# aws/sagemaker-xgboost-container

Measured on NVIDIA H100. Metric: boosting rounds/sec, higher is better.
Workload: dtype int64

## Files before the change

include/b200xgb.h:

```cpp
#ifndef B200XGB_H_
#define B200XGB_H_
#include <stddef.h>
#include <stdint.h>

#ifdef __cplusplus
extern "C" {
#endif

#if defined(__GNUC__)
#define XGB_DLL __attribute__((visibility("default")))
#else
#define XGB_DLL
#endif

typedef void* DMatrixHandle;
typedef void* BoosterHandle;
typedef uint64_t bst_ulong;

XGB_DLL const char* XGBGetLastError(void);
XGB_DLL void XGBoostVersion(int* major, int* minor, int* patch);
XGB_DLL int XGBuildInfo(const char** out);

XGB_DLL int XGDMatrixCreateFromDense(const char* data, const char* config, DMatrixHandle* out);
XGB_DLL int XGDMatrixSetInfoFromInterface(DMatrixHandle handle, const char* field, const char* data);
// ... 33 lines not shown
XGB_DLL int XGBoosterTrainOneIter(BoosterHandle handle, DMatrixHandle dtrain, int iter, const char* grad, const char* hess);
XGB_DLL int XGBoosterBoostOneIter(BoosterHandle handle, DMatrixHandle dtrain, float* grad, float* hess, bst_ulong len);
XGB_DLL int XGBoosterEvalOneIter(BoosterHandle handle, int iter, DMatrixHandle dmats[], const char* evnames[], bst_ulong len,
                         const char** out_result);
XGB_DLL int XGBoosterPredictFromDMatrix(BoosterHandle handle, DMatrixHandle dmat, const char* config,
                                bst_ulong const** out_shape, bst_ulong* out_dim, float const** out_result);
XGB_DLL int XGBoosterPredictFromDense(BoosterHandle handle, const char* values, const char* config, DMatrixHandle m,
                                      bst_ulong const** out_shape, bst_ulong* out_dim, const float** out_result);
XGB_DLL int XGBoosterPredictFromCSR(BoosterHandle handle, const char* indptr, const char* indices, const char* values, bst_ulong ncol,
                                    const char* config, DMatrixHandle m, bst_ulong const** out_shape, bst_ulong* out_dim,
                                    const float** out_result);
XGB_DLL int XGBoosterPredictFromCudaArray(BoosterHandle handle, const char* values, const char* config, DMatrixHandle proxy,
                                          bst_ulong const** out_shape, bst_ulong* out_dim, const float** out_result);
XGB_DLL int XGBoosterSaveModel(BoosterHandle handle, const char* fname);
XGB_DLL int XGBoosterLoadModel(BoosterHandle handle, const char* fname);
XGB_DLL int XGBoosterSaveModelToBuffer(BoosterHandle handle, const char* config, bst_ulong* out_len, const char** out_dptr);
XGB_DLL int XGBoosterLoadModelFromBuffer(BoosterHandle handle, const void* buf, bst_ulong len);
XGB_DLL int XGBoosterSerializeToBuffer(BoosterHandle handle, bst_ulong* out_len, const char** out_dptr);
XGB_DLL int XGBoosterUnserializeFromBuffer(BoosterHandle handle, const void* buf, bst_ulong len);
XGB_DLL int XGBoosterSaveJsonConfig(BoosterHandle handle, bst_ulong* out_len, const char** out_str);
XGB_DLL int XGBoosterLoadJsonConfig(BoosterHandle handle, const char* config);
XGB_DLL int XGBoosterGetNumFeature(BoosterHandle handle, bst_ulong* out);
XGB_DLL int XGBoosterBoostedRounds(BoosterHandle handle, int* out);
XGB_DLL int XGBoosterSlice(BoosterHandle handle, int begin_layer, int end_layer, int step, BoosterHandle* out);
XGB_DLL int XGBoosterGetAttr(BoosterHandle handle, const char* key, const char** out, int* success);
XGB_DLL int XGBoosterSetAttr(BoosterHandle handle, const char* key, const char* value);
XGB_DLL int XGBoosterGetAttrNames(BoosterHandle handle, bst_ulong* out_len, const char*** out);
XGB_DLL int XGBoosterSetStrFeatureInfo(BoosterHandle handle, const char* field, const char** features, bst_ulong size);
XGB_DLL int XGBoosterGetStrFeatureInfo(BoosterHandle handle, const char* field, bst_ulong* len, const char*** out_features);

XGB_DLL int XGCommunicatorInit(const char* config);
XGB_DLL int XGCommunicatorBroadcast(void* send_receive_buffer, size_t size, int root);
XGB_DLL int XGCommunicatorFinalize(void);
XGB_DLL int XGCommunicatorGetRank(void);
XGB_DLL int XGCommunicatorGetWorldSize(void);
XGB_DLL int XGCommunicatorGetUniqueId(const char** out_hex);

XGB_DLL int XGB200DMatrixGetCuts(DMatrixHandle handle, int max_bin, bst_ulong* n_ptrs, const int** ptrs, bst_ulong* n_vals,
                         const float** vals, const float** mins, int* has_missing);
XGB_DLL int XGB200DMatrixSetCuts(DMatrixHandle handle, const int* ptrs, bst_ulong n_ptrs, const float* vals, const float* mins);
XGB_DLL int XGB200DMatrixCreateFromCSV(const char* text, bst_ulong len, char delimiter, int* status, DMatrixHandle* out);
XGB_DLL int XGB200DMatrixCreateFromCSVEx(const char* text, bst_ulong len, char delimiter, int label_column, int weight_column,
                             int* status, DMatrixHandle* out);
XGB_DLL int XGB200DMatrixCreateFromLibsvmText(const char* text, bst_ulong len, int whitespace_mode, float absent, int* status, DMatrixHandle* out);
XGB_DLL int XGB200DMatrixCreateFromRecordIO(const char* buf, bst_ulong len, int* status, DMatrixHandle* out);
XGB_DLL int XGB200CommPeerReduceActive(void);
XGB_DLL int XGB200DMatrixCreateFromColumns(const void* const* cols, const int* col_types, int ncols, bst_ulong nrow, int label_column,
                                   int weight_column, DMatrixHandle* out);
XGB_DLL int XGB200DMatrixGetRaw(DMatrixHandle handle, float* out_row_major);
XGB_DLL int XGB200DeviceMemory(bst_ulong* live, bst_ulong* peak, int reset_peak);
XGB_DLL int XGB200DMatrixGetBins(DMatrixHandle handle, int max_bin, uint8_t* out_row_major);
XGB_DLL int XGB200DMatrixGetBinCopies(DMatrixHandle handle, int max_bin, int* out_aligned_stride, uint8_t* out_aligned, uint8_t* out_col);
XGB_DLL int XGB200DMatrixRankCuts(DMatrixHandle handle, int max_bin, const int64_t* row_bounds, int n_ranges, int* out_ptrs,
                          float* out_vals, float* out_mins);
XGB_DLL int XGB200SegmentedQuantile(const float* values, const int32_t* segments, const float* weights, bst_ulong n, int n_segments,
                                    float alpha, float* out);
XGB_DLL int XGB200GradientBasedSample(const float* gpair, bst_ulong n, float subsample, unsigned seed, uint64_t stream,
                                      float* out_threshold, float* out_gpair);
XGB_DLL int XGB200BoosterModelShape(BoosterHandle handle, bst_ulong* num_trees, bst_ulong* num_nodes, float* base_score, int* num_class);
XGB_DLL int XGB200BoosterExportModel(BoosterHandle handle, int64_t* tree_offset, int32_t* tree_info, int32_t* left, int32_t* right,
                             int32_t* parent, int32_t* split_index, int32_t* split_bin, uint8_t* default_left,
                             float* split_cond, float* base_weight, float* loss_chg, float* sum_hess);
XGB_DLL int XGB200BuildRootHistogram(BoosterHandle handle, DMatrixHandle dmat, const float* gpair, int repeats,
                             int64_t* out_hist, float* scales, float* out_ms);
XGB_DLL int XGB200BuildHistogramEx(BoosterHandle handle, DMatrixHandle dmat, const float* gpair, int repeats, int mode,
                             const unsigned* row_ids, bst_ulong n_ids, int64_t* out_hist, float* scales, float* out_ms,
                             const char** out_kernel);
XGB_DLL int XGB200BoosterEvalRootSplit(BoosterHandle handle, DMatrixHandle dmat, const int64_t* hist, int64_t G, int64_t H, float max_g,
                               float max_h, float lower, float upper, const uint8_t* feat_mask, const char** out_json);
XGB_DLL int XGB200BoosterInplaceDebug(BoosterHandle handle, int64_t chunk_rows, bst_ulong* staged_bytes, bst_ulong* staging_capacity);
XGB_DLL int XGB200BoosterPredictKernelMs(BoosterHandle handle, DMatrixHandle dmat, int repeats, float* out_ms);
XGB_DLL int XGB200BoosterPredictPlan(BoosterHandle handle, DMatrixHandle dmat, int iter_begin, int iter_end, const char** out_json);
XGB_DLL int XGB200BoosterEvalContainerMetrics(BoosterHandle handle, DMatrixHandle dmat, const char** names, bst_ulong len, int output_margin,
                                              long long* out);
XGB_DLL int XGB200BoosterGetCachedMargin(BoosterHandle handle, DMatrixHandle dmat, float* out);
XGB_DLL int XGB200BoosterGetTrainingMargin(BoosterHandle handle, DMatrixHandle dtrain, bst_ulong* out_rows, bst_ulong* out_cols, const float** out);
XGB_DLL int XGB200BoosterGetTreeWeights(BoosterHandle handle, bst_ulong* len, float* out);
XGB_DLL int XGB200BoosterGetRefreshSums(BoosterHandle handle, bst_ulong* len, long long* out);
XGB_DLL int XGB200BoosterComputeGradient(BoosterHandle handle, DMatrixHandle dmat, const float* margin, int round, float* out_gpair);
XGB_DLL int XGB200TimerStart(void);
XGB_DLL int XGB200TimerStop(float* out_ms);
XGB_DLL int XGB200BoosterSetProfile(BoosterHandle handle, int enable);
XGB_DLL int XGB200BoosterGetProfile(BoosterHandle handle, const char** out_json);
XGB_DLL int XGB200LaunchCount(long long* out);
XGB_DLL int XGB200Synchronize(void);
XGB_DLL int XGB200LegacyModelToUBJ(const void* buf, bst_ulong len, bst_ulong* out_len, const char** out);

#ifdef __cplusplus
}
#endif
#endif
```

sagemaker-xgboost-container_b200/backend.py:

```python
import ctypes as C
import json
import os

import numpy as np

_HERE = os.path.dirname(os.path.abspath(__file__))
LIB_PATH = os.path.join(_HERE, "lib", "libb200xgb.so")

c_bst_ulong = C.c_uint64


class XGBoostError(ValueError):
    """Error raised by the native library (same name and base class as xgboost.core.XGBoostError)."""


def _cstr(s):
    return C.c_char_p(s.encode("utf-8"))


def _from_cstr_array(ptr, n):
    return [ptr[i].decode("utf-8") for i in range(n)]


_utf8_and_size = C.pythonapi.PyUnicode_AsUTF8AndSize
# ... 543 lines not shown
    def booster_predict_kernel_ms(self, bh, dh, repeats=5):
        ms = C.c_float()
        self._check(self.lib.XGB200BoosterPredictKernelMs(bh, dh, C.c_int(repeats), C.byref(ms)))
        return float(ms.value)

    def booster_predict_plan(self, bh, dh, iteration_range=(0, 0)):
        out = C.c_char_p()
        self._check(self.lib.XGB200BoosterPredictPlan(bh, dh, C.c_int(iteration_range[0]), C.c_int(iteration_range[1]), C.byref(out)))
        return json.loads(out.value.decode())

    def booster_eval_container_metrics(self, bh, dh, names, output_margin):
        arr = (C.c_char_p * len(names))(*[n.encode("utf-8") for n in names])
        out = np.zeros(8 + 64 * 64, np.int64)
        self._check(self.lib.XGB200BoosterEvalContainerMetrics(bh, dh, arr, c_bst_ulong(len(names)), C.c_int(1 if output_margin else 0),
                                                               out.ctypes.data_as(C.POINTER(C.c_longlong))))
        return out

    @staticmethod
    def _gradient_iface(a):
        if isinstance(a, np.ndarray):
            return {"data": [int(a.ctypes.data), True], "shape": [int(d) for d in a.shape], "typestr": a.dtype.str, "strides": None, "version": 3}
        iface = a.__cuda_array_interface__
        out = {"data": [int(iface["data"][0]), False], "shape": [int(d) for d in iface["shape"]], "typestr": iface["typestr"],
               "strides": [int(d) for d in iface["strides"]], "version": 3}
        if "stream" in iface:
            out["stream"] = None if iface["stream"] is None else int(iface["stream"])
        return out

    def booster_boost(self, bh, dh, it, grad, hess):
        self._check(self.lib.XGBoosterTrainOneIter(bh, dh, C.c_int(it), _cstr(json.dumps(self._gradient_iface(grad))),
                                                   _cstr(json.dumps(self._gradient_iface(hess)))))

    def booster_training_margin(self, bh, dh):
        rows, cols, ptr = c_bst_ulong(), c_bst_ulong(), C.POINTER(C.c_float)()
        self._check(self.lib.XGB200BoosterGetTrainingMargin(bh, dh, C.byref(rows), C.byref(cols), C.byref(ptr)))
        if rows.value * cols.value == 0:
            return np.zeros((rows.value, cols.value), np.float32)
        return np.ctypeslib.as_array(ptr, shape=(rows.value, cols.value)).copy()

    def booster_cached_margin(self, bh, dh, K):
        n = self.dmatrix_num_row(dh)
        out = np.zeros((n, K), np.float32)
        self._check(self.lib.XGB200BoosterGetCachedMargin(bh, dh, out.ctypes.data_as(C.POINTER(C.c_float))))
        return out

    def booster_compute_gradient(self, bh, dh, margin, round=0):
        n = self.dmatrix_num_row(dh)
        margin = np.ascontiguousarray(margin, np.float32).reshape(n, -1)
        out = np.zeros((n, margin.shape[1], 2), np.float32)
        self._check(self.lib.XGB200BoosterComputeGradient(bh, dh, margin.ctypes.data_as(C.POINTER(C.c_float)), C.c_int(int(round)),
                                                          out.ctypes.data_as(C.POINTER(C.c_float))))
        return out

    def booster_tree_weights(self, bh):
        n = c_bst_ulong()
        self._check(self.lib.XGB200BoosterGetTreeWeights(bh, C.byref(n), None))
        out = np.zeros(n.value, np.float32)
        self._check(self.lib.XGB200BoosterGetTreeWeights(bh, C.byref(n), out.ctypes.data_as(C.POINTER(C.c_float))))
        return out

    def booster_refresh_sums(self, bh):
        n = c_bst_ulong()
        self._check(self.lib.XGB200BoosterGetRefreshSums(bh, C.byref(n), None))
        out = np.zeros(n.value, np.int64)
        self._check(self.lib.XGB200BoosterGetRefreshSums(bh, C.byref(n), out.ctypes.data_as(C.POINTER(C.c_longlong))))
        return out.reshape(-1, 2)

    def timer_start(self):
        self._check(self.lib.XGB200TimerStart())

    def timer_stop(self):
        ms = C.c_float()
        self._check(self.lib.XGB200TimerStop(C.byref(ms)))
        return float(ms.value)

    def booster_set_profile(self, bh, enable):
        self._check(self.lib.XGB200BoosterSetProfile(bh, C.c_int(1 if enable else 0)))

    def booster_get_profile(self, bh):
        out = C.c_char_p()
        self._check(self.lib.XGB200BoosterGetProfile(bh, C.byref(out)))
        return json.loads(out.value.decode())

    def launch_count(self):
        out = C.c_longlong()
        self._check(self.lib.XGB200LaunchCount(C.byref(out)))
        return int(out.value)

    def synchronize(self):
        self._check(self.lib.XGB200Synchronize())


_BACKEND = None


def get_backend():
    global _BACKEND
    if _BACKEND is None:
        _BACKEND = CudaBackend()
    return _BACKEND
```

sagemaker-xgboost-container_b200/csrc/booster.cu:

```cuda
#include "booster.h"
#include <algorithm>
#include <atomic>
#include <cctype>
#include <climits>
#include <cmath>
#include <cstring>
#include "comm.h"
#include "multi_target.h"
#include "rng.h"

namespace b200 {

long long g_kernel_launches = 0;

namespace {
struct DeviceCtx {
  cudaStream_t stream = nullptr; int num_sms = 0; bool ok = false; std::string why;
  DeviceCtx() {
    int count = 0;
    cudaError_t e = cudaGetDeviceCount(&count);
    if (e != cudaSuccess || count == 0) { why = std::string("no CUDA device available (") + cudaGetErrorString(e) + ")"; cudaGetLastError(); return; }
    int dev = 0;
    if (const char* lr = getenv("LOCAL_RANK")) { dev = atoi(lr) % count; }
    if (const char* d = getenv("B200XGB_DEVICE")) { dev = atoi(d) % count; }
// ... 2067 lines not shown
    CUDA_OK(cudaMemcpyAsync(d_info.p, info.data(), sizeof(int) * info.size(), cudaMemcpyHostToDevice, s));
  }
  CUDA_OK(cudaMemsetAsync(d_out.p, 0, sizeof(float) * std::max<size_t>(total, 1), s));
  ShapArgs sa{}; sa.X = dm->X.p; sa.n = n; sa.F = F; sa.nodes = d_sn.p; sa.tree_offset = d_off.p; sa.tree_info = d_info.p; sa.tree_begin = tb; sa.tree_end = te; sa.K = K;
  sa.out = d_out.p; sa.base_margin = base_margin(); sa.tree_weight = d_w.p;
  if (!dm->base_margin.empty()) { B200_CHECK(dm->base_margin.size() == (size_t)n * K, "base_margin size does not match rows x groups"); sa.base_margin_rows = dm->d_base_margin.p; }
  launch_shap(sa, max_depth, s);
  out->resize(total);
  if (total) CUDA_OK(cudaMemcpyAsync(out->data(), d_out.p, sizeof(float) * total, cudaMemcpyDeviceToHost, s));
  Comm::get().sync_stream(s);
  if (K > 1) shape->assign({(uint64_t)n, (uint64_t)K, (uint64_t)(F + 1)}); else shape->assign({(uint64_t)n, (uint64_t)(F + 1)});
}

PredictArgs Booster::predict_args(DMatrix* dm, int tree_begin, int tree_end) {
  PredictArgs pa{}; if (dm) { pa.X = dm->X.p; pa.n = dm->n; pa.F = dm->F; pa.has_nan = dm->has_missing ? 1 : 0; }
  pa.nodes = d_nodes.p; pa.tree_offset = d_tree_offset.p; pa.tree_info = d_tree_info.p;
  pa.tree_begin = tree_begin; pa.tree_end = tree_end; pa.K = param_.num_outputs(); pa.margin = nullptr; pa.leaf = nullptr;
  pa.h_tree_offset = h_tree_offset.data(); pa.children_adjacent = children_adjacent_ ? 1 : 0;
  pa.model_F = num_feature_;
  return pa;
}

void Booster::run_predict(DMatrix* dm, PredictArgs pa, cudaStream_t s) {
  if (!dm->quantile) { launch_predict(pa, s); return; }
  if (pa.tree_end <= pa.tree_begin) return;
  int64_t lo = h_tree_offset[pa.tree_begin], hi = h_tree_offset[pa.tree_begin + 1];
  for (int t = pa.tree_begin + 1; t < pa.tree_end; ++t) { lo = std::min(lo, h_tree_offset[t]); hi = std::max(hi, h_tree_offset[t + 1]); }
  bin_nodes_.ensure(std::max<size_t>(d_nodes.n, 1));
  launch_bin_thresholds(d_nodes.p + lo, (size_t)(hi - lo), dm->d_cut_ptrs.p, dm->d_cut_vals.p, dm->d_min_vals.p, dm->F, bin_nodes_.p + lo, s);
  pa.nodes = bin_nodes_.p;
  launch_predict_bins(pa, dm->binned_view(), s);
}

std::string Booster::debug_predict_plan(DMatrix* dm, int iter_begin, int iter_end) {
  configure();
  upload_model();
  if (iter_end == 0) iter_end = layers();
  B200_CHECK(iter_begin >= 0 && iter_begin <= iter_end && iter_end <= layers(), "debug_predict_plan: invalid iteration range");
  const PredictArgs pa = predict_args(dm, iteration_indptr_[iter_begin], iteration_indptr_[iter_end]);
  return predict_plan_json(dm->quantile ? plan_for_bins(pa, dm->binned_view()) : plan_for(pa), pa.tree_begin, pa.tree_end, pa.has_nan != 0);
}

float Booster::debug_predict_kernel_ms(DMatrix* dm, int repeats) {
  configure();
  cudaStream_t s = engine_stream();
  upload_model();
  const int K = param_.num_outputs();
  pred_margin_.ensure((size_t)dm->n * K);
  PredictArgs pa = predict_args(dm, 0, (int)trees_.size());
  pa.margin = pred_margin_.p;
  cudaEvent_t e0, e1; CUDA_OK(cudaEventCreate(&e0)); CUDA_OK(cudaEventCreate(&e1));
  float total = 0.f;
  for (int r = 0; r < std::max(1, repeats); ++r) {
    launch_fill(pred_margin_.p, dm->n * K, base_margin(), s);
    CUDA_OK(cudaEventRecord(e0, s));
    run_predict(dm, pa, s);
    CUDA_OK(cudaEventRecord(e1, s));
    CUDA_OK(cudaEventSynchronize(e1));
    float ms = 0; CUDA_OK(cudaEventElapsedTime(&ms, e0, e1)); total += ms;
  }
  cudaEventDestroy(e0); cudaEventDestroy(e1);
  return total / std::max(1, repeats);
}

int Booster::training_margin(DMatrix* dtrain, std::vector<float>* out) {
  configure();
  if (layers() == 0 && !update_mode_) check_targets(dtrain, true);
  cached_margin(dtrain, out);
  return param_.num_outputs();
}

void Booster::cached_margin(DMatrix* dm, std::vector<float>* out) {
  configure();
  cudaStream_t s = engine_stream();
  PredCache& c = cache_for(dm);
  bring_cache_up_to_date(dm, c);
  out->resize((size_t)dm->n * param_.num_outputs());
  if (!out->empty()) CUDA_OK(cudaMemcpyAsync(out->data(), c.margin.p, sizeof(float) * out->size(), cudaMemcpyDeviceToHost, s));
  Comm::get().sync_stream(s);
}

void Booster::set_profile(bool on) { builder_->set_profile(on); }
std::string Booster::get_profile() { return builder_->profile_json(); }

}
```

sagemaker-xgboost-container_b200/csrc/booster.h:

```cpp
#pragma once
#include <functional>
#include <map>
#include <memory>
#include <string>
#include <vector>
#include "container_metrics.h"
#include "curve.h"
#include "custom_grad.h"
#include "engine.h"
#include "grow.h"
#include "json.h"
#include "misc.h"
#include "rank.h"
#include "refresh.h"
#include "sampling.h"
#include "survival.h"
#include "tree.h"

namespace b200 {

struct ProxyBatch {
  enum Kind { kNone, kHostDense, kDevice, kCSR } kind = kNone;
  int64_t n = 0; int F = 0;
  const float* data = nullptr;
// ... 61 lines not shown
};

void csr_to_dense_device(const unsigned long long* d_ptr, const unsigned* d_idx, const float* d_val, int64_t nrow, int F, float* X, cudaStream_t s);

struct HostTree {
  std::vector<int> left, right, parent, split_index, split_bin;
  std::vector<uint8_t> default_left;
  std::vector<float> split_cond, base_weight, loss_chg, sum_hess;
  int num_nodes() const { return (int)left.size(); }
};

struct UpdateState {
  bool started = false;
  std::vector<HostTree> trees; std::vector<int> tree_info;
  std::vector<int> indptr{0};
  std::vector<int> node_off;
  std::vector<int64_t> block_off;
  DevBuf<unsigned char> in_block;
  DevBuf<DevNode> nodes; DevBuf<int> d_node_off, d_class; DevBuf<int64_t> d_block_off;
  DevBuf<GH64> sums; DevBuf<int> scratch; DevBuf<unsigned char> out_blocks;
  DevBuf<float2> gpair; DevBuf<unsigned> absmax; DevBuf<float> scales;
  int64_t global_n = 0; uint64_t global_n_uid = 0;
  int layers() const { return (int)indptr.size() - 1; }
};

struct PredCache {
  DevBuf<float> margin; int trees_applied = 0; int64_t n = 0; uint64_t model_version = 0;
  std::vector<float> weights;
};

struct DartParam { bool on = false; float rate_drop = 0.0f, skip_drop = 0.0f; int one_drop = 0, sample_type = 0, normalize_type = 0; };

bool looks_like_legacy_binary(const char* buf, size_t len);
JPtr legacy_binary_to_doc(const char* buf, size_t len);
std::pair<const char*, size_t> legacy_serialized_model_section(const char* buf, size_t len);

struct GradInput {
  static constexpr uint64_t kNoStream = ~0ull;
  const void* ptr = nullptr; int64_t n = 0, m = 1, s0 = 0, s1 = 0; bool f64 = false; uint64_t stream = kNoStream;
};

class Booster {
 public:
  Booster();
  ~Booster();
  void set_param(const std::string& k, const std::string& v);
  std::string save_config();
  void load_config(const std::string& json);
  void update_one_iter(int iter, DMatrix* dtrain);
  void boost_one_iter(DMatrix* dtrain, const GradInput& grad, const GradInput& hess);
  std::string eval_one_iter(int iter, const std::vector<DMatrix*>& dms, const std::vector<std::string>& names);
  void eval_container_metrics(DMatrix* dm, const std::vector<std::string>& names, bool output_margin, long long* out);
  void predict(DMatrix* dm, int type, bool training, int iter_begin, int iter_end, bool strict_shape,
               std::vector<float>* out, std::vector<uint64_t>* shape);
  void predict_contribs(DMatrix* dm, int tree_begin, int tree_end, std::vector<float>* out, std::vector<uint64_t>* shape);
  void inplace_predict(const InputDesc& in, bool on_device, uint64_t stream, int type, int iter_begin, int iter_end, bool strict_shape,
                       const std::vector<float>& base_margin_rows, std::vector<float>* out, std::vector<uint64_t>* shape, const float** dev_out);
  void inplace_debug(int64_t chunk_rows, uint64_t* staged_bytes, uint64_t* staging_capacity);
  std::string save_model_buffer(const std::string& format);
  void load_model_buffer(const char* buf, size_t len);
  std::string serialize();
  void unserialize(const char* buf, size_t len);
  std::unique_ptr<Booster> slice(int begin, int end, int step);
  int boosted_rounds();
  int num_features() const { return num_feature_; }
  std::map<std::string, std::string> attrs;
  std::vector<std::string> feature_names, feature_types;

  void sync_model();
  void cached_margin(DMatrix* dm, std::vector<float>* out);
  int training_margin(DMatrix* dtrain, std::vector<float>* out);
  float debug_predict_kernel_ms(DMatrix* dm, int repeats);
  std::string debug_predict_plan(DMatrix* dm, int iter_begin, int iter_end);
  const std::vector<HostTree>& trees() { sync_model(); return trees_; }
  const std::vector<int>& tree_info() const { return tree_info_; }
  const std::vector<float>& tree_weights() const { return weight_drop_; }
  float base_score() const { return base_score_; }
  int num_class() const { return param_.num_class; }
  const TrainParam& param() { configure(); return param_; }
  void set_profile(bool on);
  void debug_gradient(DMatrix* dm, const float* margin, int round, float* out);
  void debug_refresh_sums(std::vector<long long>* out);
  std::string get_profile();
  void debug_build_root_hist(DMatrix* dm, const float* gpair_host, std::vector<long long>* hist_out, float* scales_out,
                             int repeats, float* ms_out, int mode = 0, const unsigned* row_ids = nullptr, int64_t n_ids = 0);
  std::string debug_eval_root(DMatrix* dm, const long long* hist_fm, long long G, long long H, float max_g, float max_h,
                              float lower, float upper, const unsigned char* feat_mask);

 private:
  PredictArgs predict_args(DMatrix* dm, int tree_begin, int tree_end);
  void run_predict(DMatrix* dm, PredictArgs pa, cudaStream_t s);
  void predict_margin(DMatrix* dm, int tb, int te);
  void finish_predict(int64_t n, int type, bool strict_shape, std::vector<float>* out, std::vector<uint64_t>* shape, const float** dev_out);
  struct InplaceState {
    unsigned char* pinned = nullptr;
    DevBuf<unsigned char> stage;
    DevBuf<float> scratch;
    cudaStream_t copy = nullptr; cudaEvent_t copied[2] = {}, consumed[2] = {};
    int64_t debug_chunk_rows = 0; uint64_t staged_bytes = 0;
  } inplace_;
  DevBuf<DevNode> bin_nodes_;
  std::map<std::string, std::string> raw_params_;
  std::vector<std::string> eval_metrics_;
  std::vector<int> monotone_;
  std::vector<std::vector<int>> interaction_;
  bool configured_ = false;
  TrainParam param_;
  std::string objective_name_ = "reg:squarederror";
  bool base_score_set_ = false; float base_score_ = 0.5f; bool base_score_estimated_ = false;
  int num_feature_ = 0;
  int num_target_ = 1;
  std::vector<HostTree> trees_; std::vector<int> tree_info_;
  std::vector<int> iteration_indptr_{0};
  DevBuf<float2> forest_gpair_;
  GbsScratch gbs_;
  std::vector<float> weight_drop_;
  DartParam dart_;
  float dart_new_weight_ = 1.0f;
  DevBuf<float> dart_drop_margin_;
  DevBuf<int> dart_ids_; DevBuf<float> dart_coef_;
  std::vector<PendingTree> pending_;
  std::vector<char> on_device_;
  uint64_t model_version_ = 0;
  DevBuf<DevNode> d_nodes; std::vector<int64_t> h_tree_offset; DevBuf<int64_t> d_tree_offset; DevBuf<int> d_tree_info;
  size_t d_nodes_used = 0; int d_trees_uploaded = 0;
  std::map<uint64_t, PredCache> caches_;
  std::unique_ptr<TreeBuilder> builder_ = std::make_unique<TreeBuilder>();
  DevBuf<double> dsum_;
  CoxScratch cox_scratch_;
  RankScratch rank_scratch_;
  CurveScratch curve_scratch_;
  ContainerScratch container_scratch_;
  bool labels_checked_ = false;
  DevBuf<float> pred_margin_, pred_cls_; DevBuf<int> pred_leaf_;
  bool children_adjacent_ = true;
  bool update_mode_ = false; std::vector<int> update_ops_; std::string update_ops_str_; int refresh_leaf_ = 1;
  std::unique_ptr<UpdateState> update_ = std::make_unique<UpdateState>();
  DevBuf<float> quantile_alpha_dev_; std::vector<float> quantile_alpha_host_;
  DevBuf<unsigned> target_absmax_;
  const CustomGradArgs* custom_ = nullptr;
  DevBuf<unsigned char> custom_staging_; DevBuf<unsigned long long> custom_bad_; DevBuf<unsigned> custom_bad_flag_;
  void train_round(DMatrix* dtrain, const CustomGradArgs* custom);
  GradArray custom_array(const GradInput& in, bool device, size_t staging_offset);
  void launch_custom_gradient_checked(int round, float2* gpair, int64_t gp_stride, unsigned* absmax, float subsample, bool per_target_absmax);

  void configure();
  void check_label_ranges(const DMatrix* dtrain);
  void check_targets(const DMatrix* dm, bool training);
  const RankGroups& rank_groups(DMatrix* dm, const char* what);
  void begin_update();
  void refresh_one_iter(DMatrix* dtrain);
  int layers() const { return (int)iteration_indptr_.size() - 1; }
  float base_margin() const;
  void estimate_base_score(DMatrix* dtrain);
  void upload_model();
  PredCache& cache_for(DMatrix* dm);
  void bring_cache_up_to_date(DMatrix* dm, PredCache& c);
  void append_device_tree(int class_id, size_t device_offset, int max_nodes, PendingTree pt, float weight);
  std::vector<int> dart_drop_set(int round) const;
  float* dart_begin_round(DMatrix* dtrain, PredCache& c, int round);
  DartArgs dart_args(const std::vector<int>& ids, const std::vector<float>& coef_full, const std::vector<float>& coef_drop);
  void dart_margin(DMatrix* dm, const std::vector<int>& ids, const std::vector<float>& coef_full, const std::vector<float>& coef_drop,
                   float* m_full, float* m_drop);
  void reserve_nodes(size_t count, size_t slack);
  TreeBuilder& builder_for(DMatrix* dm);
  TreeInputs tree_inputs(const DMatrix& dm, const std::string& mask, int tree_index, float* margin, int k);
// ... 22 lines not shown
```

sagemaker-xgboost-container_b200/csrc/capi.cc:

```cpp
#include "../../include/b200xgb.h"
#include <cmath>
#include <cstdio>
#include <cstring>
#include <algorithm>
#include <dirent.h>
#include <fstream>
#include <map>
#include <memory>
#include <sstream>
#include <sys/stat.h>
#include <string>
#include <vector>
#include "booster.h"
#include "comm.h"

using namespace b200;

namespace {
thread_local std::string g_last_error;
struct DMatrixBox {
  std::unique_ptr<DMatrix> dm;
  std::unique_ptr<ProxyBatch> proxy;
  std::vector<const char*> str_ptrs; std::vector<std::string> strs;
  std::vector<uint8_t> scratch_u8;
// ... 808 lines not shown
  std::vector<long long> h; float sc[4];
  BST(handle)->debug_build_root_hist(dm, gpair, &h, sc, repeats, out_ms, mode, row_ids, (int64_t)n_ids);
  hist_to_feature_major(dm, h, out_hist);
  if (scales) memcpy(scales, sc, sizeof sc);
  if (out_kernel) *out_kernel = hist_last_kernel();
  API_END();
}
int XGB200BoosterEvalRootSplit(BoosterHandle handle, DMatrixHandle dmat, const int64_t* hist, int64_t G, int64_t H, float max_g, float max_h,
                               float lower, float upper, const uint8_t* feat_mask, const char** out_json) {
  API_BEGIN(); BoosterBox* box = static_cast<BoosterBox*>(handle);
  box->ret_str = BST(handle)->debug_eval_root(DM(dmat), reinterpret_cast<const long long*>(hist), G, H, max_g, max_h, lower, upper, feat_mask);
  *out_json = box->ret_str.c_str(); API_END();
}
int XGB200BoosterPredictKernelMs(BoosterHandle handle, DMatrixHandle dmat, int repeats, float* out_ms) {
  API_BEGIN();
  *out_ms = BST(handle)->debug_predict_kernel_ms(DM(dmat), repeats);
  API_END();
}
int XGB200BoosterPredictPlan(BoosterHandle handle, DMatrixHandle dmat, int iter_begin, int iter_end, const char** out_json) {
  API_BEGIN(); BoosterBox* box = static_cast<BoosterBox*>(handle); box->ret_str = BST(handle)->debug_predict_plan(DM(dmat), iter_begin, iter_end);
  *out_json = box->ret_str.c_str(); API_END();
}
int XGB200BoosterGetTreeWeights(BoosterHandle handle, bst_ulong* len, float* out) {
  API_BEGIN();
  const std::vector<float>& w = BST(handle)->tree_weights();
  if (len) *len = w.size();
  if (out) memcpy(out, w.data(), sizeof(float) * w.size());
  API_END();
}
int XGB200BoosterGetRefreshSums(BoosterHandle handle, bst_ulong* len, long long* out) {
  API_BEGIN();
  std::vector<long long> v;
  BST(handle)->debug_refresh_sums(&v);
  if (len) *len = v.size();
  if (out) memcpy(out, v.data(), sizeof(long long) * v.size());
  API_END();
}
int XGB200BoosterComputeGradient(BoosterHandle handle, DMatrixHandle dmat, const float* margin, int round, float* out_gpair) {
  API_BEGIN();
  B200_CHECK(round >= 0, "XGB200BoosterComputeGradient: round must be >= 0");
  BST(handle)->debug_gradient(DM(dmat), margin, round, out_gpair);
  API_END();
}
int XGB200BoosterEvalContainerMetrics(BoosterHandle handle, DMatrixHandle dmat, const char** names, bst_ulong len, int output_margin,
                                      long long* out) {
  API_BEGIN();
  std::vector<std::string> v;
  for (bst_ulong i = 0; i < len; ++i) v.emplace_back(names[i]);
  BST(handle)->eval_container_metrics(DM(dmat), v, output_margin != 0, out);
  API_END();
}
int XGB200BoosterGetTrainingMargin(BoosterHandle handle, DMatrixHandle dtrain, bst_ulong* out_rows, bst_ulong* out_cols, const float** out) {
  API_BEGIN();
  BoosterBox* box = static_cast<BoosterBox*>(handle);
  const int K = BST(handle)->training_margin(DM(dtrain), &box->ret_vec);
  *out_rows = (bst_ulong)DM(dtrain)->n; *out_cols = (bst_ulong)K; *out = box->ret_vec.data();
  API_END();
}
int XGB200BoosterGetCachedMargin(BoosterHandle handle, DMatrixHandle dmat, float* out) {
  API_BEGIN();
  std::vector<float> v;
  BST(handle)->cached_margin(DM(dmat), &v);
  memcpy(out, v.data(), sizeof(float) * v.size());
  API_END();
}
static cudaEvent_t g_t0 = nullptr, g_t1 = nullptr;
int XGB200TimerStart(void) {
  API_BEGIN();
  if (!g_t0) { CUDA_OK(cudaEventCreate(&g_t0)); CUDA_OK(cudaEventCreate(&g_t1)); }
  CUDA_OK(cudaEventRecord(g_t0, engine_stream()));
  API_END();
}
int XGB200TimerStop(float* out_ms) {
  API_BEGIN();
  if (!g_t0) throw Error("XGB200TimerStop without XGB200TimerStart");
  CUDA_OK(cudaEventRecord(g_t1, engine_stream())); CUDA_OK(cudaEventSynchronize(g_t1));
  CUDA_OK(cudaEventElapsedTime(out_ms, g_t0, g_t1));
  API_END();
}
int XGB200BoosterSetProfile(BoosterHandle handle, int enable) { API_BEGIN(); BST(handle)->set_profile(enable != 0); API_END(); }
int XGB200BoosterGetProfile(BoosterHandle handle, const char** out_json) {
  API_BEGIN(); BoosterBox* box = static_cast<BoosterBox*>(handle); box->ret_str = BST(handle)->get_profile(); *out_json = box->ret_str.c_str(); API_END();
}
int XGB200LaunchCount(long long* out) { API_BEGIN(); *out = g_kernel_launches; API_END(); }
int XGB200Synchronize(void) { API_BEGIN(); CUDA_OK(cudaStreamSynchronize(engine_stream())); API_END(); }
int XGB200DMatrixCreateFromColumns(const void* const* cols, const int* col_types, int ncols, bst_ulong nrow, int label_column, int weight_column, DMatrixHandle* out) {
  API_BEGIN();
  B200_CHECK(out != nullptr && (ncols == 0 || (cols != nullptr && col_types != nullptr)), "XGB200DMatrixCreateFromColumns: NULL argument");
  auto box = new DMatrixBox(); std::unique_ptr<DMatrixBox> guard(box);
  box->dm = DMatrix::from_columns(cols, col_types, ncols, (int64_t)nrow, label_column, weight_column);
  *out = guard.release();
  API_END();
}
int XGB200LegacyModelToUBJ(const void* buf, bst_ulong len, bst_ulong* out_len, const char** out) {
  API_BEGIN();
  B200_CHECK(buf != nullptr && out_len != nullptr && out != nullptr, "XGB200LegacyModelToUBJ: NULL argument");
  const char* p = (const char*)buf; size_t n = (size_t)len;
  auto sect = legacy_serialized_model_section(p, n);
  if (sect.first != nullptr) { p = sect.first; n = sect.second; }
  B200_CHECK(looks_like_legacy_binary(p, n), "XGB200LegacyModelToUBJ: the buffer is not a legacy binary model");
  g_ret_str.clear(); ubj_write(*legacy_binary_to_doc(p, n), &g_ret_str);
  *out_len = g_ret_str.size(); *out = g_ret_str.data();
  API_END();
}

}
```

sagemaker-xgboost-container_b200/csrc/engine.h:

```cpp
#pragma once
#include <cuda_runtime.h>
#include <cstdint>
#include <cstdio>
#include <stdexcept>
#include <string>
#include <vector>

namespace b200 {

struct Error : std::runtime_error { using std::runtime_error::runtime_error; };
#define B200_CHECK(cond, msg) do { if (!(cond)) throw ::b200::Error(std::string(msg)); } while (0)
#define CUDA_OK(expr) do { cudaError_t e_ = (expr); if (e_ != cudaSuccess) throw ::b200::Error( \
    std::string("CUDA error: ") + cudaGetErrorString(e_) + " at " + __FILE__ + ":" + std::to_string(__LINE__)); } while (0)

extern long long g_kernel_launches;

cudaStream_t engine_stream();
int engine_num_sms();

void devmem_note(int64_t delta);
void devmem_query(uint64_t* live, uint64_t* peak, bool reset_peak);

template <typename T> struct DevBuf {
  T* p = nullptr; size_t n = 0;
  DevBuf() = default;
  DevBuf(const DevBuf&) = delete; DevBuf& operator=(const DevBuf&) = delete;
  ~DevBuf() { release(); }
  void release() { if (p) { cudaFree(p); devmem_note(-(int64_t)(n * sizeof(T))); } p = nullptr; n = 0; }
  void alloc(size_t count) { if (count == n && p) return; release();
    if (count) { CUDA_OK(cudaMalloc(&p, count * sizeof(T))); devmem_note((int64_t)(count * sizeof(T))); } n = count; }
  void ensure(size_t count) { if (count > n) alloc(count); }
  void zero(cudaStream_t s) { if (n) CUDA_OK(cudaMemsetAsync(p, 0, n * sizeof(T), s)); }
};

constexpr int kSlots = 32;
constexpr int kBins = 256;
constexpr int kGroupEntries = kBins * kSlots;
constexpr int kMissingBin = 255;
constexpr int kGradBits = 18, kWindowRows = 8064;
constexpr int kGradBitsSmall = 21, kWindowRowsSmall = 1008;
constexpr int64_t kSmallMatrixRows = 1 << 20;
inline int grad_bits_for(int64_t n) { return n <= kSmallMatrixRows ? kGradBitsSmall : kGradBits; }
inline int window_rows_for(int64_t n) { return n <= kSmallMatrixRows ? kWindowRowsSmall : kWindowRows; }
constexpr int kMaxDepth = 16;
constexpr int kMaxTrainFeatures = 65534 * 32;
static_assert(kMaxTrainFeatures < (1 << 23), "cand_key holds 23 bits of feature id");

struct GH64 { long long g, h; };

struct BinnedMatrix {
  const uint8_t* bins = nullptr;
  const uint8_t* bins_tail = nullptr;
  const uint8_t* bins_col = nullptr;
  const uint8_t* bins_gather = nullptr;
  int gather_stride = 0;
  int tail_in_gather = 0;
  int64_t n = 0;
  int F = 0, ngroups = 0, tw = 0, ntail = 0;
  int has_missing = 0;
  int unused = 0;
};

inline void feature_layout(int F, int* ngroups, int* tw, int* ntail) {
  const int a = F / 32, L = F % 32;
  if (a >= 1 && L >= 1 && L <= 8) { *ngroups = a; *ntail = L; *tw = L <= 4 ? 4 : 8; }
  else { *ngroups = a + (L > 0 ? 1 : 0); if (*ngroups == 0) *ngroups = 1; *ntail = 0; *tw = 0; }
}
inline size_t hist_slot_entries(int ngroups, int tw) { return (size_t)ngroups * 256 * 32 + (size_t)256 * tw; }

enum Objective : int { kSquaredError = 0, kBinaryLogistic = 1, kRegLogistic = 2, kLogitRaw = 3, kSoftprob = 4, kSoftmax = 5,
                       kSquaredLogError = 6, kPseudoHuber = 7, kPoisson = 8, kGamma = 9, kTweedie = 10, kHinge = 11,
                       kAft = 12, kCox = 13,
                       kAbsoluteError = 14,
                       kQuantileError = 15,
                       kRankPairwise = 16, kRankNdcg = 17, kRankMap = 18 };
enum Transform : int { kTransformNone = 0, kTransformSigmoid = 1, kTransformExp = 2, kTransformHinge = 3 };
inline bool objective_is_logistic(int o) { return o == kBinaryLogistic || o == kRegLogistic || o == kLogitRaw; }
inline bool objective_is_log_link(int o) { return o == kPoisson || o == kGamma || o == kTweedie; }
inline bool objective_is_survival(int o) { return o == kAft || o == kCox; }
inline bool objective_is_adaptive(int o) { return o == kAbsoluteError || o == kQuantileError; }
inline bool objective_is_rank(int o) { return o == kRankPairwise || o == kRankNdcg || o == kRankMap; }
inline int objective_transform(int o) {
  if (o == kBinaryLogistic || o == kRegLogistic) return kTransformSigmoid;
  if (objective_is_log_link(o) || objective_is_survival(o)) return kTransformExp;
  return o == kHinge ? kTransformHinge : kTransformNone;
}

struct TrainParam {
  int objective = kSquaredError;
  int num_class = 1;
  int max_depth = 6, max_leaves = 0, max_bin = 256;
  int lossguide = 0;
  float eta = 0.3f, lambda = 1.0f, alpha = 0.0f, gamma = 0.0f, min_child_weight = 1.0f, max_delta_step = 0.0f;
  float scale_pos_weight = 1.0f, subsample = 1.0f, colsample_bytree = 1.0f, colsample_bylevel = 1.0f, colsample_bynode = 1.0f;
  unsigned seed = 0;
  int num_parallel_tree = 1;
  int gradient_based = 0;
  float huber_slope = 1.0f, tweedie_variance_power = 1.5f, poisson_max_delta_step = 0.7f;
  int aft_dist = 0; float aft_sigma = 1.0f;
  std::vector<float> quantile_alpha;
  int rank_mean = 0, rank_unbiased = 0, rank_k = 32, rank_exp_gain = 1, rank_normalization = 1, rank_score_normalization = 1; float rank_bias_norm = 2.0f;
// ... 39 lines not shown
```

sagemaker-xgboost-container_b200/csrc/grow.cu:

```cuda
#include "grow.h"
#include <algorithm>
#include <cmath>
#include <cstdlib>
#include <cstring>
#include "comm.h"

namespace b200 {

__global__ void pack_tree_kernel(TreeArrays t, const int* n_nodes, DevNode* out, int cap) {
  const int nn = *n_nodes;
  for (int i = blockIdx.x * blockDim.x + threadIdx.x; i < cap; i += gridDim.x * blockDim.x) {
    DevNode d;
    if (i < nn) { d.cond = t.split_cond[i]; d.left = t.left[i]; d.right = t.right[i]; d.fidx_dl = (unsigned)t.split_index[i] | ((unsigned)t.default_left[i] << 31); }
    else { d.cond = 0.f; d.left = -1; d.right = -1; d.fidx_dl = 0; }
    out[i] = d;
  }
}
__global__ void snapshot_h_kernel(const GH64* slot, long long* cache, size_t entries) {
  for (size_t e = (size_t)blockIdx.x * blockDim.x + threadIdx.x; e < entries; e += (size_t)gridDim.x * blockDim.x) cache[e] = slot[e].h;
}
__global__ void slot_from_cache_kernel(GH64* slot, const long long* cache, size_t entries) {
  for (size_t e = (size_t)blockIdx.x * blockDim.x + threadIdx.x; e < entries; e += (size_t)gridDim.x * blockDim.x) { GH64 v; v.g = 0; v.h = cache[e]; slot[e] = v; }
}
__global__ void gather_u32_kernel(const unsigned* src, const unsigned* idx, unsigned* dst, int64_t n) {
  const int64_t i = (int64_t)blockIdx.x * blockDim.x + threadIdx.x;
  if (i < n) dst[i] = src[idx[i]];
}

void* PinnedPool::take(size_t bytes) {
  bytes = (bytes + 255) & ~(size_t)255;
  while (cur < chunks.size() && off + bytes > chunks[cur].second) { ++cur; off = 0; }
  if (cur >= chunks.size()) { size_t sz = std::max<size_t>(bytes, 4u << 20); char* p = nullptr; CUDA_OK(cudaMallocHost(&p, sz)); chunks.emplace_back(p, sz); off = 0; }
  void* r = chunks[cur].first + off; off += bytes; return r;
}
static bool tail_by_position(const BinnedMatrix& bm) { return bm.tw == 4 && !bm.tail_in_gather; }

size_t TreeBuilder::carve(GrowState& gs, uintptr_t base) const {
  const size_t N = cap_nodes, L = max_level_nodes, nblocks = ngroups + (tw > 0 ? 1 : 0);
  size_t off = 0;
  auto take = [&](auto*& p, size_t bytes) { p = reinterpret_cast<std::remove_reference_t<decltype(p)>>(base + off); off += (bytes + 255) & ~(size_t)255; };
  take(gs.seg_begin, 4 * N); take(gs.seg_count, 4 * N); take(gs.hist_slot, 4 * N); take(gs.node_sum, 16 * N); take(gs.root_gain, 4 * N); take(gs.weight, 4 * N);
  take(gs.best, sizeof(SplitCand) * N); take(gs.best_group, sizeof(SplitCand) * N * nblocks);
  take(gs.level_nodes, 4 * (size_t)(kMaxDepth + 1) * L); take(gs.level_count, 4 * (kMaxDepth + 2));
  take(gs.build_nid, 4 * L); take(gs.build_sub_nid, 4 * L); take(gs.build_parent_slot, 4 * L); take(gs.build_count, 4); take(gs.build_prefix, 4 * (L + 1));
  take(gs.part_action, 4 * L); take(gs.tile_prefix, 4 * (L + 1));
  take(gs.tile_desc, 8 * ((size_t)max_tiles + 1)); gs.part_ctl = (unsigned*)(gs.tile_desc + max_tiles);
  take(gs.n_leaves, 4); take(gs.scales, 16); take(gs.absmax, 8);
  take(gs.depth, 4 * N); take(gs.open, N); take(gs.n_slots, 4); take(gs.lg_done, 4); take(gs.lower, 4 * N); take(gs.upper, 4 * N);
  return off;
}

void TreeBuilder::ensure(const BinnedMatrix& bm, int max_depth_, int K, int lg_iters_, int n_ic_) {
  const bool tail_pos_ = tail_by_position(bm);
  const int64_t stride_ = (bm.n + 63) & ~(int64_t)63;
  if (n == bm.n && F == bm.F && ngroups == bm.ngroups && tw == bm.tw && tail_pos == tail_pos_ && max_depth == max_depth_ && lg_iters == lg_iters_ &&
      n_ic == n_ic_ && gpair.n >= (size_t)stride_ * K + 512) return;
  if (lg_iters_ == 0) B200_CHECK(max_depth_ >= 1 && max_depth_ <= kMaxDepth, "max_depth must be in [1, 16] for the B200 depth-wise hist builder");
  n = bm.n; F = bm.F; ngroups = bm.ngroups; tw = bm.tw; tail_pos = tail_pos_; max_depth = max_depth_; lg_iters = lg_iters_; n_ic = n_ic_;
  gp_stride = stride_; root_h_valid = false;
  cudaStream_t s = engine_stream();
  if (peer_reduce_active()) {
    peer_reduce_close();
    DevBuf<unsigned> bar; bar.alloc(1); bar.zero(s);
    Comm::get().allreduce_max_u32(bar.p, 1, s);
    Comm::get().sync_stream(s);
  }
  for (auto& tg : graphs) tg.destroy();
  size_t pool_slots; int max_nodes;
  if (lg_iters > 0) {
    max_nodes = 2 * lg_iters + 1; max_level_nodes = 2; region = 0;
    pool_slots = (size_t)lg_iters + kLgFirstFreeSlot;
  } else {
    max_nodes = (1 << (max_depth + 1)) - 1; max_level_nodes = 1 << (max_depth - 1); region = max_level_nodes;
    pool_slots = 2 * (size_t)region;
  }
  cap_nodes = (max_nodes + 15) & ~15;
  slot_stride = hist_slot_entries(ngroups, tw);
  const size_t partial_entries = hist_partial_entries(ngroups, tw, engine_num_sms(), max_level_nodes);
  const size_t pool_bytes = pool_slots * slot_stride * sizeof(GH64) + partial_entries * sizeof(int2);
  size_t free_b = 0, total_b = 0; cudaMemGetInfo(&free_b, &total_b);
  B200_CHECK(pool_bytes < free_b / 2 + hist_pool.n * sizeof(GH64) + hist_partials.n * sizeof(int2),
             "histogram pool for this max_depth / max_leaves / feature count does not fit in device memory");
  hist_pool.alloc(pool_slots * slot_stride);
  hist_partials.alloc(partial_entries);
  gpair.alloc((size_t)gp_stride * K + 512); gpair.zero(s); err.alloc(1); tree_index_dev.alloc(1);
  if (!leaf_scale.p) { leaf_scale.alloc(1); set_leaf_scale(1.0f); }
  root_h_cache.alloc(slot_stride);
  const bool routed = routes(lg_iters, max_depth);
  for (int i = 0; i < 2; ++i) { const size_t m = i == 0 || !routed ? (size_t)n : 0; ridx[i].alloc(m); gp[i].alloc(m); tl[i].alloc(tail_pos ? m : 0); }
  route_tiles = routed ? (unsigned)((n + kRouteTile - 1) / kRouteTile) : 0u;
  node_of_row.alloc(routed ? (size_t)n : 0);
  route_counts.alloc(routed && max_depth >= 2 ? ((size_t)1 << (max_depth - 2)) * route_tiles : 0);
  max_tiles = (unsigned)((n + kPartTile - 1) / kPartTile) + max_level_nodes + 1;
  scratch.alloc(3 * (size_t)max_level_nodes + 8);
  state_block.alloc(carve(gs, 0)); state_block.zero(s);
  carve(gs, (uintptr_t)state_block.p);
  tree_block.alloc(tree_block_bytes(cap_nodes));
  const TreeBlock tb = tree_block_layout(tree_block.p, cap_nodes);
  gs.n_nodes = tb.n_nodes; ta = tb.t; packed.alloc(cap_nodes);
  ic_path.alloc(n_ic ? (size_t)cap_nodes * F : 0); ic_allowed.alloc(n_ic ? (size_t)cap_nodes * F : 0);
  ic_sets.alloc((size_t)n_ic * F); ic_sets_host.clear();
  hist_configure();
  global_n = n;
  if (Comm::get().distributed()) {
    peer_reduce_setup({{hist_pool.p, hist_pool.n * sizeof(GH64)}, {state_block.p, state_block.n}}, s);
// ... 8 lines not shown

float* TreeBuilder::ensure_adaptive(int targets) {
  if (adapt.ensure(n, max_leaves(), cap_nodes, targets)) for (auto& tg : graphs) tg.destroy();
  return adapt.resid.p;
}

void TreeBuilder::set_leaf_scale(float v) {
  cudaStream_t s = engine_stream();
  CUDA_OK(cudaMemcpyAsync(leaf_scale.p, &v, sizeof v, cudaMemcpyHostToDevice, s));
  Comm::get().sync_stream(s);
}

const unsigned char* TreeBuilder::upload_mask(const std::string& mask, int tree_index) {
  cudaStream_t s = engine_stream(); feat_mask.ensure(mask.size());
  CUDA_OK(cudaMemcpyAsync(feat_mask.p, mask.data(), mask.size(), cudaMemcpyHostToDevice, s));
  CUDA_OK(cudaMemcpyAsync(tree_index_dev.p, &tree_index, sizeof(int), cudaMemcpyHostToDevice, s));
  Comm::get().sync_stream(s); return feat_mask.p;
}
template <typename T> static T* upload_changed(DevBuf<T>& d, std::vector<T>& host, const std::vector<T>& v) {
  if (v == host && d.n >= v.size()) return d.p;
  cudaStream_t s = engine_stream(); d.ensure(v.size());
  CUDA_OK(cudaMemcpyAsync(d.p, v.data(), sizeof(T) * v.size(), cudaMemcpyHostToDevice, s));
  Comm::get().sync_stream(s); host = v; return d.p;
}

const int* TreeBuilder::upload_monotone(const std::vector<int>& mono, int F_) {
  if (mono.empty()) return nullptr;
  B200_CHECK((int)mono.size() <= F_, "monotone_constraints has more entries than the data has features");
  std::vector<int> mh(mono); mh.resize((size_t)F_, 0);
  return upload_changed(monotone_dev, monotone_host, mh);
}
void TreeBuilder::upload_interaction(const std::vector<std::vector<int>>& ic, int F_) {
  if (ic.empty()) return;
  std::vector<unsigned char> sets(ic.size() * (size_t)F_, 0);
  for (size_t si = 0; si < ic.size(); ++si)
    for (int f : ic[si]) { B200_CHECK(f < F_, "interaction_constraints names feature " + std::to_string(f) + " but the data has " + std::to_string(F_) + " features"); sets[si * F_ + f] = 1; }
  upload_changed(ic_sets, ic_sets_host, sets);
}
HistArgs TreeBuilder::hist_args(const BinnedMatrix& bm, int k) const {
  HistArgs ha{}; ha.bins = bm.bins; ha.bins_tail = bm.bins_tail; ha.n = bm.n; ha.row_stride = bm.ngroups * kSlots; ha.tw = bm.tw;
  ha.bins_gather = bm.bins_gather; ha.gather_stride = bm.gather_stride;
  ha.tail_in_gather = bm.tail_in_gather;
  ha.gpair = gpair.p + (size_t)k * gp_stride;
  ha.build_count = gs.build_count; ha.build_nid = gs.build_nid; ha.build_prefix = gs.build_prefix; ha.seg_begin = gs.seg_begin;
  ha.hist_slot = gs.hist_slot; ha.scales = gs.scales; ha.hist_pool = hist_pool.p; ha.node_sum = gs.node_sum; ha.ngroups = bm.ngroups;
  ha.partials = hist_partials.p; ha.accumulate_sum = 1; ha.window_rows = window_rows_for(global_n);
  return ha;
}

EvalArgs TreeBuilder::eval_args(const TreeInputs& in, int level, const unsigned char* feat_mask) const {
  const BinnedMatrix& bm = in.bm;
  EvalArgs ea{}; ea.hist_pool = hist_pool.p; ea.gs = gs; ea.cut_ptrs = in.cut_ptrs; ea.feat_mask = feat_mask; ea.p = in.p; ea.F = bm.F;
  ea.ngroups = bm.ngroups; ea.tw = bm.tw; ea.ntail = bm.ntail; ea.has_missing = bm.has_missing; ea.level = level; ea.max_level_nodes = max_level_nodes;
  ea.colsample_bynode = in.mask ? in.colsample_bynode : 1.0f; ea.seed = in.seed; ea.tree_index = tree_index_dev.p; ea.monotone = in.monotone;
  ea.node_allowed = in.n_ic > 0 ? ic_allowed.p : nullptr;
  return ea;
}
ApplyArgs TreeBuilder::apply_args(const TreeInputs& in, int level, int next_base, int next_half) const {
  const BinnedMatrix& bm = in.bm;
  ApplyArgs aa{}; aa.gs = gs; aa.tree = ta; aa.cut_ptrs = in.cut_ptrs; aa.cut_vals = in.cut_vals; aa.min_vals = in.min_vals;
  aa.p = in.p; aa.scratch = scratch.p; aa.nblocks = bm.ngroups + (bm.tw > 0 ? 1 : 0); aa.level = level; aa.max_level_nodes = max_level_nodes;
  aa.next_base = next_base; aa.next_half = next_half; aa.monotone = in.monotone;
  if (in.n_ic > 0) { aa.node_path = ic_path.p; aa.node_allowed = ic_allowed.p; aa.ic_sets = ic_sets.p; aa.n_ic_sets = in.n_ic; aa.F = bm.F; }
  return aa;
}
template <class Launch> void TreeBuilder::timed(ProfKind kind, Launch launch) {
  if (!profile) { launch(); return; }
  ProfEvent e; e.kind = kind; e.launches = g_kernel_launches;
  CUDA_OK(cudaEventCreate(&e.a)); CUDA_OK(cudaEventCreate(&e.b));
  CUDA_OK(cudaEventRecord(e.a, engine_stream()));
  launch();
  e.launches = g_kernel_launches - e.launches;
  CUDA_OK(cudaEventRecord(e.b, engine_stream()));
  prof_events.push_back(e);
}

constexpr int kRootRows = -1;
void TreeBuilder::enqueue(const TreeInputs& in) {
  cudaStream_t s = engine_stream();
  const BinnedMatrix& bm = in.bm;
  const int k = in.k, D = in.p.max_depth;
  const bool dist = in.world > 1;
  const int num_sms = engine_num_sms();
  launch_init_tree(gs, ta, (unsigned)bm.n, s);
  if (in.root_mode == 2) { slot_from_cache_kernel<<<num_sms, 256, 0, s>>>(hist_pool.p, root_h_cache.p, slot_stride); ++g_kernel_launches; CUDA_OK(cudaGetLastError()); }
  else CUDA_OK(cudaMemsetAsync(hist_pool.p, 0, slot_stride * sizeof(GH64), s));
  const bool g_only = in.root_mode != 0;
  const int pay = g_only ? 4 : 8;
  const bool carry_tail = tail_by_position(bm);
  const bool routed = routes(in.lg_iters, D);
  if (profile && routed) {
    prof_part_row_bytes[0] = 3;
    prof_part_row_bytes[1] = 4;
    prof_part_row_bytes[2] = pay + 4 + pay + (carry_tail ? 8 : 0);
  } else if (profile) {
    prof_part_row_bytes[0] = pay + (carry_tail ? 4 : 0) + 1;
    prof_part_row_bytes[2] = 4 + pay + (carry_tail ? 4 : 0);
    prof_part_row_bytes[1] = prof_part_row_bytes[2] + 1;
  }
  HistArgs root = hist_args(bm, k);
  if (g_only) { root.gpair = nullptr; root.gpos = g_dense(); }
  root.g_only = in.root_mode == 2 ? 1 : 0; root.rows_counter = profile ? prof_rows.p : nullptr;
  timed(kProfRootHist, [&] { launch_hist_build(root, num_sms, s); });
  if (in.root_mode == 1) { snapshot_h_kernel<<<num_sms, 256, 0, s>>>(hist_pool.p, root_h_cache.p, slot_stride); ++g_kernel_launches; CUDA_OK(cudaGetLastError()); }
  auto collective = [&](std::function<void()> f) {
    if (!dist) return;
    if (!capturing) { f(); return; }
    end_segment(); capturing->colls.push_back(f);
    CUDA_OK(cudaStreamBeginCapture(s, cudaStreamCaptureModeThreadLocal));
  };
  auto allreduce_hist = [&](GH64* p, size_t cnt) {
    if (!dist) return;
    if (peer_allreduce_i64(reinterpret_cast<long long*>(p), cnt, s)) return;
    collective([p, cnt, s]() { Comm::get().allreduce_sum_i64(p, cnt, s); });
  };
  allreduce_hist(hist_pool.p, slot_stride * 2);
  allreduce_hist(gs.node_sum, 2);
  if (in.n_ic > 0) {
    CUDA_OK(cudaMemsetAsync(ic_path.p, 0, (size_t)bm.F, s));
    CUDA_OK(cudaMemsetAsync(ic_allowed.p, 1, (size_t)bm.F, s));
  }
  auto part_args = [&](int level, int cur, int next) {
    const bool root = cur == kRootRows;
    PartArgs pa{}; pa.gs = gs; pa.tree = ta; pa.bins_col = bm.bins_col; pa.n = bm.n;
    pa.ridx_cur = root ? nullptr : ridx[cur].p; pa.ridx_next = ridx[next].p;
    const void* root_gp = g_only ? static_cast<const void*>(g_dense()) : static_cast<const void*>(gpair.p + (size_t)k * gp_stride);
    pa.gp_cur = root ? root_gp : gp[cur].p; pa.gp_next = gp[next].p; pa.g_only = g_only ? 1 : 0;
    pa.tl_cur = !carry_tail ? nullptr : (root ? reinterpret_cast<const unsigned*>(bm.bins_tail) : tl[cur].p); pa.tl_next = carry_tail ? tl[next].p : nullptr;
    pa.has_missing = bm.has_missing; pa.level = level; pa.max_level_nodes = max_level_nodes; pa.rows_counter = profile ? prof_rows.p + 2 : nullptr;
    return pa;
  };
  auto level_hist_args = [&](int set) {
    HistArgs ha = hist_args(bm, k);
    ha.ridx = ridx[set].p; ha.tail_pos = carry_tail ? tl[set].p : nullptr; ha.accumulate_sum = 0;
    ha.gpair = g_only ? nullptr : gp[set].p; ha.gpos = g_only ? reinterpret_cast<const float*>(gp[set].p) : nullptr;
    ha.rows_counter = profile ? prof_rows.p + 1 : nullptr;
    return ha;
  };
  launch_eval(eval_args(in, 0, in.mask), 1, s);
  for (int it = 0; it < in.lg_iters; ++it) {
    launch_apply_lossguide(apply_args(in, 0, 0, 0), it, s);
    const PartArgs pa = part_args(0, it == 0 ? kRootRows : 0, 1);
    timed(kProfPartition, [&] { launch_partition(pa, max_tiles, s); });
    launch_lg_copy_back(pa, ridx[0].p, gp[0].p, tl[0].p, max_tiles, s);
    launch_zero_build_slots(gs, hist_pool.p, slot_stride, 1, s);
    timed(kProfDeepHist, [&] { launch_hist_build(level_hist_args(0), num_sms, s); });
    if (dist) {
      launch_lg_stage(gs, hist_pool.p, slot_stride, 1, s);
      allreduce_hist(hist_pool.p + (size_t)kLgStageSlot * slot_stride, slot_stride * 2);
      launch_lg_stage(gs, hist_pool.p, slot_stride, 0, s);
    }
    launch_subtract(gs, hist_pool.p, slot_stride, 1, s);
    launch_eval(eval_args(in, 1, nullptr), 2, s);
  }
  for (int L = 0; L < D && in.lg_iters == 0; ++L) {
    const bool final_level = (L == D - 1);
    const int next_base = ((L + 1) & 1) * region, next_half = 1 << L;
    launch_apply(apply_args(in, L, next_base, next_half), s);
    if (final_level) break;
    if (routed) {
      RouteArgs ra{}; ra.gs = gs; ra.tree = ta; ra.bins_col = bm.bins_col; ra.n = bm.n; ra.node_of_row = node_of_row.p;
      ra.tile_counts = route_counts.p; ra.ntiles = route_tiles; ra.has_missing = bm.has_missing; ra.level = L;
      if (g_only) ra.g = g_dense(); else ra.gpair = gpair.p + (size_t)k * gp_stride;
      ra.g_only = g_only ? 1 : 0;
      ra.tail_row = carry_tail ? reinterpret_cast<const unsigned*>(bm.bins_tail) : nullptr;
      ra.ridx = ridx[0].p; ra.gp = gp[0].p; ra.tl = carry_tail ? tl[0].p : nullptr; ra.rows_counter = profile ? prof_rows.p + 2 : nullptr;
      timed(kProfPartition, [&] { launch_route(ra, s); });
    } else {
      PartArgs pa = part_args(L, L == 0 ? kRootRows : (L & 1) ^ 1, L & 1);
      pa.build_only = L == D - 2 ? 1 : 0;
      timed(kProfPartition, [&] { launch_partition(pa, max_tiles, s); });
    }
    CUDA_OK(cudaMemsetAsync(hist_pool.p + (size_t)next_base * slot_stride, 0, (size_t)next_half * slot_stride * sizeof(GH64), s));
    timed(kProfDeepHist, [&] { launch_hist_build(level_hist_args(routed ? 0 : L & 1), num_sms, s); });
    allreduce_hist(hist_pool.p + (size_t)next_base * slot_stride, (size_t)next_half * slot_stride * 2);
    launch_subtract(gs, hist_pool.p, slot_stride, next_half, s);
    launch_eval(eval_args(in, L + 1, in.mask ? in.mask + (size_t)(L + 1) * bm.F : nullptr), 1 << (L + 1), s);
  }
  const uint8_t* start = routed && D >= 2 ? node_of_row.p : nullptr;
  if (in.adaptive) {
    launch_locate_leaves(ta, gs.n_nodes, bm.bins_col, bm.n, bm.has_missing, start, g_only ? nullptr : gpair.p + (size_t)k * gp_stride, &adapt, s);
    SelectArgs sa{}; sa.values = in.resid; sa.seg = adapt.seg.p; sa.h = in.adaptive == 2 ? reinterpret_cast<const float*>(gpair.p + (size_t)k * gp_stride) + 1 : nullptr;
    sa.h_stride = 2; sa.scales = gs.scales; sa.n = bm.n; sa.nseg = max_leaves(); sa.alpha = (double)in.alpha;
    if (in.adaptive == 3) { sa.h = in.weight; sa.h_stride = 1; sa.scales = adapt.scales.p; }
    sa.leaf_nid = adapt.leaf_nid.p; sa.split_cond = ta.split_cond; sa.lr = in.p.eta;
    segmented_select(sa, &adapt, [&](unsigned long long* p, size_t cnt) { collective([p, cnt, s]() { Comm::get().allreduce_sum_i64(p, cnt, s); }); },
                     [&](unsigned* p, size_t cnt) { collective([p, cnt, s]() { Comm::get().allreduce_max_u32(p, cnt, s); }); }, s);
  }
  timed(kProfMargin, [&] { launch_update_margin(ta, gs.n_nodes, bm.bins_col, bm.n, bm.has_missing, start, in.margin, in.K, k, leaf_scale.p, s); });
  if (profile) prof_margin_rows += bm.n;
  pack_tree_kernel<<<(cap_nodes + 255) / 256, 256, 0, s>>>(ta, gs.n_nodes, packed.p, cap_nodes); ++g_kernel_launches;
  CUDA_OK(cudaGetLastError());
}
void TreeBuilder::end_segment() {
  cudaGraph_t graph = nullptr; cudaGraphExec_t exec = nullptr;
  CUDA_OK(cudaStreamEndCapture(engine_stream(), &graph));
  cudaError_t e = cudaGraphInstantiate(&exec, graph, 0);
  cudaGraphDestroy(graph);
  CUDA_OK(e);
  capturing->segs.push_back(exec);
}

void TreeBuilder::grow(const TreeInputs& in) {
  cudaStream_t s = engine_stream();
  static const bool no_graph = getenv("B200XGB_NO_GRAPH") != nullptr;
  if ((int)graphs.size() <= in.k) graphs.resize(in.k + 1);
  TreeGraph& tg = graphs[in.k];
  if (profile || no_graph || (in.world > 1 && !tg.eager_done) || in.root_mode == 1) { tg.eager_done = true; enqueue(in); return; }
  if (tg.segs.empty() || memcmp(&tg.key, &in, sizeof in) != 0) {
    tg.destroy();
    const long long launches_before = g_kernel_launches;
    CUDA_OK(cudaStreamBeginCapture(s, cudaStreamCaptureModeThreadLocal));
    capturing = &tg;
    try { enqueue(in); end_segment(); }
    catch (...) { capturing = nullptr; cudaGraph_t graph = nullptr; cudaStreamEndCapture(s, &graph); if (graph) cudaGraphDestroy(graph); tg.destroy(); throw; }
    capturing = nullptr;
    tg.key = in; tg.launches = g_kernel_launches - launches_before;
    g_kernel_launches = launches_before;
  }
  for (size_t i = 0; i < tg.segs.size(); ++i) {
    CUDA_OK(cudaGraphLaunch(tg.segs[i], s));
    if (i < tg.colls.size()) tg.colls[i]();
  }
  g_kernel_launches += tg.launches;
}
PendingTree TreeBuilder::stage_tree() {
  cudaStream_t s = engine_stream();
  PendingTree pt; pt.cap_nodes = (size_t)cap_nodes; pt.staging = pinned.take(tree_block.n);
  if (!free_events.empty()) { pt.ready = free_events.back(); free_events.pop_back(); }
  else CUDA_OK(cudaEventCreateWithFlags(&pt.ready, cudaEventDisableTiming));
  CUDA_OK(cudaMemcpyAsync(pt.staging, tree_block.p, tree_block.n, cudaMemcpyDeviceToHost, s));
  CUDA_OK(cudaEventRecord(pt.ready, s));
  return pt;
}

void TreeBuilder::debug_build_root_hist(const BinnedMatrix& bm, const float* gpair_host, std::vector<long long>* hist_out, float* scales_out,
                                        int repeats, float* ms_out, int mode, const unsigned* row_ids, int64_t n_ids) {
  cudaStream_t s = engine_stream();
  const int64_t rows = row_ids ? n_ids : bm.n;
  B200_CHECK(rows <= bm.n, "debug_build_root_hist: more row ids than rows");
  CUDA_OK(cudaMemcpyAsync(gpair.p, gpair_host, sizeof(float2) * rows, cudaMemcpyHostToDevice, s));
  if (row_ids) CUDA_OK(cudaMemcpyAsync(ridx[0].p, row_ids, sizeof(unsigned) * rows, cudaMemcpyHostToDevice, s));
  float mg = 0.f, mh = 0.f;
  for (int64_t i = 0; i < rows; ++i) { mg = std::max(mg, std::fabs(gpair_host[2 * i])); mh = std::max(mh, gpair_host[2 * i + 1]); }
  unsigned am[2]; memcpy(&am[0], &mg, 4); memcpy(&am[1], &mh, 4);
  CUDA_OK(cudaMemcpyAsync(gs.absmax, am, 8, cudaMemcpyHostToDevice, s));
  launch_scales(gs, grad_bits_for(global_n), s);
  HistArgs ha = hist_args(bm, 0);
  ha.ridx = row_ids ? ridx[0].p : nullptr;
  ha.force_gather = (mode & 3) == 1 ? 1 : 0; ha.g_only = (mode & 3) == 2 ? 1 : 0;
  if ((mode & 8) || ha.g_only) {
    std::vector<float> gh((size_t)rows);
    for (int64_t i = 0; i < rows; ++i) gh[i] = gpair_host[2 * i];
    float* gpos = row_ids ? reinterpret_cast<float*>(gp[0].p) : g_dense();
    if (rows) CUDA_OK(cudaMemcpyAsync(gpos, gh.data(), sizeof(float) * rows, cudaMemcpyHostToDevice, s));
    Comm::get().sync_stream(s);
    ha.gpos = gpos; ha.gpair = nullptr;
  }
  if ((mode & 4) && row_ids && tail_by_position(bm)) {
    gather_u32_kernel<<<(unsigned)((rows + 255) / 256), 256, 0, s>>>(reinterpret_cast<const unsigned*>(bm.bins_tail), ridx[0].p, tl[0].p, rows); ++g_kernel_launches;
    CUDA_OK(cudaGetLastError());
    ha.tail_pos = tl[0].p;
  }
  root_h_valid = false;
  cudaEvent_t e0, e1; CUDA_OK(cudaEventCreate(&e0)); CUDA_OK(cudaEventCreate(&e1));
  float total = 0.f;
  for (int r = 0; r < std::max(1, repeats); ++r) {
    launch_init_tree(gs, ta, (unsigned)rows, s);
    CUDA_OK(cudaMemsetAsync(hist_pool.p, 0, slot_stride * sizeof(GH64), s));
    CUDA_OK(cudaEventRecord(e0, s));
    launch_hist_build(ha, engine_num_sms(), s);
    CUDA_OK(cudaEventRecord(e1, s));
    CUDA_OK(cudaEventSynchronize(e1));
    float ms = 0; CUDA_OK(cudaEventElapsedTime(&ms, e0, e1)); total += ms;
  }
  if (ms_out) *ms_out = total / std::max(1, repeats);
  hist_out->resize(slot_stride * 2);
  CUDA_OK(cudaMemcpyAsync(hist_out->data(), hist_pool.p, sizeof(GH64) * slot_stride, cudaMemcpyDeviceToHost, s));
  CUDA_OK(cudaMemcpyAsync(scales_out, gs.scales, 4 * sizeof(float), cudaMemcpyDeviceToHost, s));
  Comm::get().sync_stream(s);
  cudaEventDestroy(e0); cudaEventDestroy(e1);
}

std::string TreeBuilder::debug_eval_root(const TreeInputs& in, const long long* hist_fm, long long G, long long H, float max_g, float max_h,
                                         float lower, float upper) {
  cudaStream_t s = engine_stream();
  root_h_valid = false;
  const BinnedMatrix& bm = in.bm;
  const int F_ = bm.F;
  std::vector<GH64> slot(slot_stride, GH64{0, 0});
  const size_t W = (size_t)bm.ngroups * kSlots, tail0 = (size_t)bm.ngroups * kGroupEntries;
  for (int f = 0; f < F_; ++f)
    for (int b = 0; b < kBins; ++b) {
      const size_t e = (size_t)f < W ? ((size_t)(f / kSlots) * kBins + b) * kSlots + f % kSlots : tail0 + (size_t)b * bm.tw + (f - W);
      slot[e].g = hist_fm[((size_t)f * kBins + b) * 2]; slot[e].h = hist_fm[((size_t)f * kBins + b) * 2 + 1];
    }
  launch_init_tree(gs, ta, (unsigned)bm.n, s);
  CUDA_OK(cudaMemcpyAsync(hist_pool.p, slot.data(), sizeof(GH64) * slot_stride, cudaMemcpyHostToDevice, s));
  const GH64 tot{G, H};
  CUDA_OK(cudaMemcpyAsync(gs.node_sum, &tot, sizeof tot, cudaMemcpyHostToDevice, s));
  CUDA_OK(cudaMemcpyAsync(gs.lower, &lower, 4, cudaMemcpyHostToDevice, s));
  CUDA_OK(cudaMemcpyAsync(gs.upper, &upper, 4, cudaMemcpyHostToDevice, s));
  unsigned am[2]; memcpy(&am[0], &max_g, 4); memcpy(&am[1], &max_h, 4);
  CUDA_OK(cudaMemcpyAsync(gs.absmax, am, 8, cudaMemcpyHostToDevice, s));
  launch_scales(gs, grad_bits_for(global_n), s);
  launch_eval(eval_args(in, 0, in.mask), 1, s);
  const ApplyArgs aa = apply_args(in, 0, region, 1);
  if (in.lg_iters > 0) launch_apply_lossguide(aa, 0, s); else launch_apply(aa, s);
  const int nblocks = bm.ngroups + (bm.tw > 0 ? 1 : 0);
  std::vector<unsigned char> sb(state_block.n), tb(tree_block.n);
  CUDA_OK(cudaMemcpyAsync(sb.data(), state_block.p, sb.size(), cudaMemcpyDeviceToHost, s));
  CUDA_OK(cudaMemcpyAsync(tb.data(), tree_block.p, tb.size(), cudaMemcpyDeviceToHost, s));
  Comm::get().sync_stream(s);
  GrowState h; carve(h, (uintptr_t)sb.data());
  auto bits = [](float v) { unsigned u; memcpy(&u, &v, 4); return std::to_string(u); };
  auto cand = [&](const SplitCand& c) {
    return "{\"loss_chg\":" + bits(c.loss_chg) + ",\"feature\":" + std::to_string(c.feature) + ",\"bin\":" + std::to_string(c.bin) + ",\"dleft\":" +
           std::to_string(c.dleft) + ",\"ord\":" + std::to_string(c.ord) + ",\"GL\":" + std::to_string(c.GL) + ",\"HL\":" + std::to_string(c.HL) + "}";
  };
  const TreeBlock t = tree_block_layout(tb.data(), cap_nodes);
  const int nn = *t.n_nodes;
  std::string o = "{\"scales\":[";
  for (int i = 0; i < 4; ++i) o += (i ? "," : "") + bits(h.scales[i]);
  o += "],\"root_gain\":" + bits(h.root_gain[0]) + ",\"weight\":" + bits(h.weight[0]) + ",\"best_group\":[";
  for (int i = 0; i < nblocks; ++i) o += (i ? "," : "") + cand(h.best_group[i]);
  o += "],\"best\":" + cand(h.best[0]) + ",\"n_nodes\":" + std::to_string(nn) + ",\"expanded\":" + (nn == 3 ? "true" : "false") + ",\"tree\":{";
  const char* iname[5] = {"left", "right", "parent", "split_index", "split_bin"};
  const int* iarr[5] = {t.t.left, t.t.right, t.t.parent, t.t.split_index, t.t.split_bin};
  const char* fname[4] = {"split_cond", "base_weight", "loss_chg", "sum_hess"};
  const float* farr[4] = {t.t.split_cond, t.t.base_weight, t.t.loss_chg, t.t.sum_hess};
  for (int a = 0; a < 5; ++a) { o += std::string(a ? "," : "") + "\"" + iname[a] + "\":["; for (int i = 0; i < nn; ++i) o += (i ? "," : "") + std::to_string(iarr[a][i]); o += "]"; }
  for (int a = 0; a < 4; ++a) { o += std::string(",\"") + fname[a] + "\":["; for (int i = 0; i < nn; ++i) o += (i ? "," : "") + bits(farr[a][i]); o += "]"; }
  o += ",\"default_left\":["; for (int i = 0; i < nn; ++i) o += (i ? "," : "") + std::to_string((int)t.t.default_left[i]); o += "]}";
  o += ",\"children\":[";
  for (int c = 1; c < nn && c < 3; ++c)
    o += std::string(c > 1 ? "," : "") + "{\"G\":" + std::to_string(h.node_sum[c].g) + ",\"H\":" + std::to_string(h.node_sum[c].h) + ",\"lower\":" + bits(h.lower[c]) + ",\"upper\":" + bits(h.upper[c]) + "}";
  o += "]}";
  return o;
}

void TreeBuilder::set_profile(bool on) {
  profile = on;
  if (on) { prof_rows.alloc(4); prof_rows.zero(engine_stream()); prof_margin_rows = 0; }
  for (auto& e : prof_events) { cudaEventDestroy(e.a); cudaEventDestroy(e.b); }
  prof_events.clear();
}
std::string TreeBuilder::profile_json() {
  cudaStream_t s = engine_stream();
  Comm::get().sync_stream(s);
  double ms[kProfKinds] = {}; long long launches[kProfKinds] = {};
  for (auto& e : prof_events) { float t = 0; CUDA_OK(cudaEventElapsedTime(&t, e.a, e.b)); ms[e.kind] += t; launches[e.kind] += e.launches; }
  unsigned long long rows[4] = {0, 0, 0, 0};
  if (prof_rows.p) CUDA_OK(cudaMemcpy(rows, prof_rows.p, sizeof rows, cudaMemcpyDeviceToHost));
  char buf[1024];
  snprintf(buf, sizeof buf, "{\"root_hist_ms\":%.6f,\"root_hist_launches\":%lld,\"root_hist_rows\":%llu,\"deep_hist_ms\":%.6f,\"deep_hist_launches\":%lld,\"deep_hist_rows\":%llu,"
           "\"part_ms\":%.6f,\"part_launches\":%lld,\"part_rows\":%llu,\"part_rows_written\":%llu,"
           "\"part_row_bytes_in_root\":%d,\"part_row_bytes_in\":%d,\"part_row_bytes_out\":%d,\"margin_ms\":%.6f,\"margin_launches\":%lld,\"margin_rows\":%lld}",
           ms[kProfRootHist], launches[kProfRootHist], rows[0], ms[kProfDeepHist], launches[kProfDeepHist], rows[1],
           ms[kProfPartition], launches[kProfPartition], rows[2], rows[3], prof_part_row_bytes[0], prof_part_row_bytes[1], prof_part_row_bytes[2],
           ms[kProfMargin], launches[kProfMargin], prof_margin_rows);
  return buf;
}

}
```

sagemaker-xgboost-container_b200/csrc/grow.h:

```cpp
#pragma once
#include <functional>
#include <string>
#include <type_traits>
#include <vector>
#include "adaptive.h"
#include "engine.h"
#include "misc.h"
#include "tree.h"

namespace b200 {

struct TreeInputs {
  BinnedMatrix bm;
  const int* cut_ptrs; const float* cut_vals; const float* min_vals;
  float* margin;
  const unsigned char* mask;
  const int* monotone;
  TrainParamDev p;
  float colsample_bynode; unsigned seed;
  int lg_iters, n_ic;
  int K, k, world;
  int root_mode;
  const float* resid; const float* weight;
  int adaptive;
  float alpha;
};
static_assert(std::is_trivially_copyable<TreeInputs>::value, "TreeInputs is compared as bytes");
static_assert(sizeof(BinnedMatrix) == 4 * sizeof(void*) + sizeof(int64_t) + 8 * sizeof(int), "BinnedMatrix has padding bytes");
static_assert(sizeof(TrainParamDev) == 8 * 4, "TrainParamDev has padding bytes");
static_assert(sizeof(TreeInputs) == sizeof(BinnedMatrix) + 8 * sizeof(void*) + sizeof(TrainParamDev) + 10 * 4, "TreeInputs has padding bytes");

inline size_t tree_block_bytes(size_t cap) { return 64 + 9 * 4 * cap + cap; }
struct TreeBlock { int* n_nodes; TreeArrays t; };
__host__ __device__ inline TreeBlock tree_block_layout(void* base, size_t cap) {
  int* ip = (int*)((unsigned char*)base + 64); float* fp = (float*)(ip + 5 * cap);
  return {(int*)base, {ip, ip + cap, ip + 2 * cap, ip + 3 * cap, ip + 4 * cap, (unsigned char*)(fp + 4 * cap), fp, fp + cap, fp + 2 * cap, fp + 3 * cap}};
}

struct PendingTree {
  void* staging = nullptr; size_t cap_nodes = 0; cudaEvent_t ready = nullptr;
};
struct PinnedPool {
  std::vector<std::pair<char*, size_t>> chunks; size_t cur = 0, off = 0;
  ~PinnedPool() { for (auto& c : chunks) cudaFreeHost(c.first); }
  void* take(size_t bytes);
  void reset() { cur = 0; off = 0; }
};

struct TreeGraph {
  std::vector<cudaGraphExec_t> segs; std::vector<std::function<void()>> colls;
  TreeInputs key{}; long long launches = 0;
  bool eager_done = false;
  TreeGraph() = default; TreeGraph(TreeGraph&&) = default;
  ~TreeGraph() { destroy(); }
  void destroy() { for (auto e : segs) if (e) cudaGraphExecDestroy(e); segs.clear(); colls.clear(); }
};

struct TreeBuilder {
  int64_t n = 0; int F = 0, ngroups = 0, tw = 0, max_depth = 0, cap_nodes = 0, max_level_nodes = 0, region = 0; bool tail_pos = false;
  int lg_iters = 0, n_ic = 0;
  size_t slot_stride = 0;
  int64_t gp_stride = 0;
  unsigned max_tiles = 0;
  int64_t global_n = 0;
  DevBuf<long long> root_h_cache; uint64_t root_h_uid = 0, root_h_version = 0; bool root_h_valid = false;
  GrowState gs{}; TreeArrays ta{};
  DevBuf<unsigned char> state_block;
  DevBuf<unsigned char> tree_block;
  DevBuf<GH64> hist_pool; DevBuf<unsigned> ridx[2], scratch;
  DevBuf<int2> hist_partials;
  DevBuf<float2> gpair, gp[2]; DevBuf<unsigned> tl[2]; DevBuf<int> err, tree_index_dev; DevBuf<unsigned char> ic_path, ic_allowed, ic_sets;
  DevBuf<uint8_t> node_of_row; DevBuf<unsigned> route_counts; unsigned route_tiles = 0;
  DevBuf<DevNode> packed;
  DevBuf<float> leaf_scale;
  DevBuf<unsigned char> feat_mask; DevBuf<int> monotone_dev;
  std::vector<unsigned char> ic_sets_host;
  std::vector<int> monotone_host;
  PinnedPool pinned; std::vector<cudaEvent_t> free_events;
  std::vector<TreeGraph> graphs;
  TreeGraph* capturing = nullptr;
  SelectScratch adapt;
  int max_leaves() const { return lg_iters > 0 ? lg_iters + 1 : 1 << max_depth; }
  float* ensure_adaptive(int targets = 1);
  enum ProfKind { kProfRootHist, kProfDeepHist, kProfPartition, kProfMargin, kProfKinds };
  struct ProfEvent { cudaEvent_t a, b; int kind; long long launches; };
  bool profile = false; std::vector<ProfEvent> prof_events;
  DevBuf<unsigned long long> prof_rows;
  long long prof_margin_rows = 0;
  int prof_part_row_bytes[3] = {0, 0, 0};

  ~TreeBuilder() { for (auto e : free_events) cudaEventDestroy(e); for (auto& e : prof_events) { cudaEventDestroy(e.a); cudaEventDestroy(e.b); } }
  void ensure(const BinnedMatrix& bm, int max_depth, int K, int lg_iters, int n_ic);
  static bool routes(int lg_iters, int max_depth) { return lg_iters == 0 && max_depth <= kRouteMaxDepth; }
  const unsigned char* upload_mask(const std::string& mask, int tree_index);
  const int* upload_monotone(const std::vector<int>& mono, int F);
  void upload_interaction(const std::vector<std::vector<int>>& sets, int F);
  void set_leaf_scale(float v);
  void grow(const TreeInputs& in);
  PendingTree stage_tree();
  void set_profile(bool on); std::string profile_json();
  void debug_build_root_hist(const BinnedMatrix& bm, const float* gpair_host, std::vector<long long>* hist_out, float* scales_out,
                             int repeats, float* ms_out, int mode, const unsigned* row_ids, int64_t n_ids);
  std::string debug_eval_root(const TreeInputs& in, const long long* hist_fm, long long G, long long H, float max_g, float max_h,
                              float lower, float upper);

 private:
  size_t carve(GrowState& g, uintptr_t base) const;
  void enqueue(const TreeInputs& in);
  void end_segment();
  HistArgs hist_args(const BinnedMatrix& bm, int k) const;
  float* g_dense() const { return reinterpret_cast<float*>(gpair.p); }
  EvalArgs eval_args(const TreeInputs& in, int level, const unsigned char* feat_mask) const;
  ApplyArgs apply_args(const TreeInputs& in, int level, int next_base, int next_half) const;
  template <class Launch> void timed(ProfKind kind, Launch launch);
};

}
```

sagemaker-xgboost-container_b200/csrc/hist.cu:

```cuda
#include <cuda.h>
#include <cstdlib>
#include <cstring>
#include <map>
#include <mutex>
#include <tuple>
#include <type_traits>
#include "engine.h"
#include "tree.h"

namespace b200 {

constexpr int kSuperRows = 32;
constexpr int kMinRowsPerCta = 4096;
constexpr int kSpillThresholdG = 1 << 25;
constexpr unsigned kSpillThresholdH = 1u << 26;
constexpr int kPlaneBytes = kGroupEntries * 4;
constexpr int kMaxSmem = 232448;
constexpr int kTeamWarps = 4, kTeams = 6, kRootRows = 16 * kTeamWarps;
constexpr int kRootConsumerWarps = kTeamWarps * kTeams;
constexpr int kRootProducerWarps = 3;
constexpr int kRootThreads = (kRootConsumerWarps + kRootProducerWarps) * 32;

template <int K, int N, typename F> __device__ __forceinline__ void static_for(F&& f) {
  if constexpr (K < N) { f(std::integral_constant<int, K>{}); static_for<K + 1, N>(f); }
// ... 174 lines not shown
    red_shared_u32(addr + kHPlane, hq);
  }
}

__device__ __forceinline__ void flush_node_sum(GH64* dst, int g, unsigned h, int lane) {
  long long G = g, H = h;
#pragma unroll
  for (int o = 16; o > 0; o >>= 1) { G += __shfl_xor_sync(0xffffffffu, G, o); H += __shfl_xor_sync(0xffffffffu, H, o); }
  if (lane == 0 && (G != 0 || H != 0)) { red_global_s64(&dst->g, G); red_global_s64(&dst->h, H); }
}

template <int PL>
__device__ __forceinline__ void spill_main(int* smem, int ng_here, GH64* out, bool last, int tid, int nthr) {
  const int vecs = ng_here * PL * (kGroupEntries / 4);
  const int start = (int)(((long long)blockIdx.x * vecs) / gridDim.x);
  for (int i = tid; i < vecs; i += nthr) {
    int v = i + start; if (v >= vecs) v -= vecs;
    int4 x = reinterpret_cast<int4*>(smem)[v];
    if ((x.x | x.y | x.z | x.w) == 0) continue;
    const int plane = v >> 11;
    const int e0 = (v & 2047) << 2;
    const bool is_h = PL == 2 && (plane & 1);
    GH64* o = out + (size_t)(plane / PL) * kGroupEntries + e0;
    int vals[4] = {x.x, x.y, x.z, x.w};
    bool any = false;
#pragma unroll
    for (int k = 0; k < 4; ++k) {
      const int val = vals[k];
      const bool sp = last ? (val != 0) : (is_h ? ((unsigned)val >= kSpillThresholdH) : (val >= kSpillThresholdG || val <= -kSpillThresholdG));
      if (sp) {
        red_global_s64(is_h ? &o[k].h : &o[k].g, is_h ? (long long)(unsigned)val : (long long)val);
        vals[k] = 0; any = true;
      }
    }
    if (any) reinterpret_cast<int4*>(smem)[v] = make_int4(vals[0], vals[1], vals[2], vals[3]);
  }
}

template <int PL>
__device__ __forceinline__ void spill_tail(int* tsm, int tw, int trep, GH64* out_tail, bool last, int tid, int nthr) {
  const int per_plane = 256 * tw * trep;
  const int per_bin = tw * trep;
  for (int idx = tid; idx < PL * per_plane; idx += nthr) {
    const int val = tsm[idx];
    if (val == 0) continue;
    const bool is_h = idx >= per_plane;
    const int e = is_h ? idx - per_plane : idx;
    const int bin = e / per_bin, slot = e & (tw - 1);
    const bool sp = last ? true : (is_h ? ((unsigned)val >= kSpillThresholdH) : (val >= kSpillThresholdG || val <= -kSpillThresholdG));
    if (sp) {
      GH64* o = out_tail + bin * tw + slot;
      red_global_s64(is_h ? &o->h : &o->g, is_h ? (long long)(unsigned)val : (long long)val);
      tsm[idx] = 0;
    }
  }
}

struct RootCfg {
  int S;
  int trep;
  int box_groups;
  unsigned tail_off;
  unsigned ring_off;
  unsigned stage_bytes;
  unsigned total;
  int flags;
};

template <bool GONLY, int G>
__device__ __forceinline__ void root_unit(const LaneConst& lc, const unsigned (&ldsoff)[4], unsigned rowaddr, int gq, unsigned hq) {
  constexpr int PL = GONLY ? 1 : 2;
  unsigned ww[4];
#pragma unroll
  for (int j = 0; j < 4; ++j) ww[j] = lds_u32(rowaddr + (unsigned)(G * 32) + ldsoff[j]);
  accumulate16<GONLY, G * PL * kPlaneBytes>(lc, ww, gq, hq);
}

template <bool GONLY>
__global__ void __launch_bounds__(kRootThreads, 1)
hist_root_kernel(const __grid_constant__ CUtensorMap tm, HistArgs a, RootCfg c) {
  constexpr int PL = GONLY ? 1 : 2;
  constexpr int NCW = kRootConsumerWarps, R = kRootRows;
  extern __shared__ __align__(128) unsigned char smem_raw[];
  const int nb = *a.build_count;
  if (nb <= 0) return;
  const unsigned T = a.build_prefix[nb];
  if (T == 0) return;
  const int lane = threadIdx.x & 31, warp = threadIdx.x >> 5;
  const int g0 = blockIdx.y * a.ng_chunk;
  const int ng_here = min(a.ng_chunk, a.ngroups - g0);
  const bool has_tail = a.tw > 0 && blockIdx.y == gridDim.y - 1;
  if (a.rows_counter && blockIdx.x == 0 && blockIdx.y == 0 && threadIdx.x == 0) atomicAdd(a.rows_counter, (unsigned long long)T);

  const unsigned smem_base = (unsigned)__cvta_generic_to_shared(smem_raw);
  const unsigned ring = (smem_base + c.ring_off + 127u) & ~127u;
  const unsigned bars = ring + (unsigned)c.S * c.stage_bytes;
  const unsigned row_bytes = 32u * (unsigned)c.box_groups;
  const unsigned main_tile_bytes = (unsigned)R * row_bytes;
  constexpr unsigned kGradBytes = GONLY ? 4u : 8u;
  const unsigned gp_off = main_tile_bytes, tail_tile_off = main_tile_bytes + (unsigned)R * kGradBytes;
  const unsigned ntiles = (T + R - 1) / R;
  const unsigned my_ntiles = ntiles > blockIdx.x ? (ntiles - blockIdx.x + gridDim.x - 1) / gridDim.x : 0u;

  {
    const int main4 = ng_here * PL * kPlaneBytes / 16;
    int4* z = reinterpret_cast<int4*>(smem_raw);
    for (int i = threadIdx.x; i < main4; i += blockDim.x) z[i] = make_int4(0, 0, 0, 0);
    if (has_tail) {
      const int tail4 = PL * 256 * a.tw * c.trep * 4 / 16;
      int4* zt = reinterpret_cast<int4*>(smem_raw + c.tail_off);
      for (int i = threadIdx.x; i < tail4; i += blockDim.x) zt[i] = make_int4(0, 0, 0, 0);
    }
    if (threadIdx.x == 0) {
      for (int s = 0; s < c.S; ++s) { mbar_init(bars + 8u * s, 1); mbar_init(bars + 8u * (c.S + s), kTeamWarps); }
      asm volatile("fence.mbarrier_init.release.cluster;" ::: "memory");
    }
  }
  __syncthreads();

  const int nid = a.build_nid[0];
  const size_t slot_entries = (size_t)a.ngroups * kGroupEntries + (size_t)256 * a.tw;
  GH64* out_slot = a.hist_pool + (size_t)a.hist_slot[nid] * slot_entries;
  GH64* out_main = out_slot + (size_t)g0 * kGroupEntries;
  GH64* out_tail = out_slot + (size_t)a.ngroups * kGroupEntries;

  if (warp >= NCW) {
    if (lane == 0) {
      const unsigned P = (c.flags & 8) ? 1u : (unsigned)kRootProducerWarps, pw = (unsigned)(warp - NCW);
      if (pw < P) {
        const unsigned tx = main_tile_bytes + (unsigned)R * kGradBytes + (has_tail ? (unsigned)R * (unsigned)a.tw : 0u);
        unsigned s = pw % (unsigned)c.S, round = pw / (unsigned)c.S;
        for (unsigned i = pw; i < my_ntiles; i += P) {
          if (round > 0) mbar_wait(bars + 8u * (c.S + s), (round - 1u) & 1u);
          const unsigned full = bars + 8u * s, dst = ring + s * c.stage_bytes;
          const unsigned t = blockIdx.x + i * gridDim.x;
          const unsigned row0 = t * (unsigned)R;
          mbar_expect_tx(full, tx);
          if ((c.flags & 1) && gridDim.y == 1) bulk_load_1d(dst, a.bins + (size_t)row0 * a.row_stride, main_tile_bytes, full);
          else tma_load_2d(dst, &tm, g0 * 32, (int)row0, full);
          if (GONLY) bulk_load_1d(dst + gp_off, a.gpos + row0, (unsigned)R * 4u, full);
          else bulk_load_1d(dst + gp_off, a.gpair + row0, (unsigned)R * 8u, full);
          if (has_tail) bulk_load_1d(dst + tail_tile_off, a.bins_tail + (size_t)row0 * a.tw, (unsigned)R * (unsigned)a.tw, full);
          const unsigned tp = t + 8u * gridDim.x;
          if (tp < ntiles && !(c.flags & 4)) tma_prefetch_2d(&tm, g0 * 32, (int)(tp * (unsigned)R));
          s += P; if (s >= (unsigned)c.S) { s -= (unsigned)c.S; ++round; }
        }
      }
    }
    return;
  }

  const int team = warp / kTeamWarps, wit = warp % kTeamWarps;
  const float sg = a.scales[0], sh = a.scales[1];
  const LaneConst lc = make_lane_const(lane, smem_base);
  unsigned ldsoff[4];
#pragma unroll
  for (int j = 0; j < 4; ++j) { ldsoff[j] = 16u * (unsigned)(lane & 1) + 4u * (unsigned)((j + lc.qw) & 3); asm volatile("" : "+r"(ldsoff[j])); }
  TailConst tc;
  tc.tw = a.tw; tc.base_g = smem_base + c.tail_off; tc.hplane_bytes = 256u * (unsigned)a.tw * (unsigned)c.trep * 4u;
  tc.bin_stride = (unsigned)a.tw * (unsigned)c.trep * 4u;
  tc.rep_off = has_tail ? (unsigned)((lane / a.tw) % c.trep) * (unsigned)a.tw * 4u : 0u;
  const unsigned rowl = (unsigned)(wit << 4) + (unsigned)(lane >> 1);
  const unsigned tiles_per_window = (unsigned)a.window_rows / R;
  const unsigned hq_one = (unsigned)__float2int_rn(1.0f * sh);
  auto quant = [&](unsigned tile, unsigned row, bool valid, int& gq, unsigned& hq) {
    gq = 0; hq = 0;
    if constexpr (GONLY) {
      const float g = __uint_as_float(lds_u32(tile + gp_off + row * 4u));
      if (valid) { gq = __float2int_rn(g * sg); hq = hq_one; }
    } else {
      const uint2 gh = lds_v2(tile + gp_off + row * 8u);
      if (valid) { gq = __float2int_rn(__uint_as_float(gh.x) * sg); hq = (unsigned)__float2int_rn(__uint_as_float(gh.y) * sh); }
    }
  };
  long long accG = 0, accH = 0;
  unsigned i = (unsigned)team, s = (unsigned)team, ph = 0;
  for (unsigned wstart = 0;; wstart += tiles_per_window) {
    const unsigned wend = wstart + tiles_per_window < my_ntiles ? wstart + tiles_per_window : my_ntiles;
    while (i < wend) {
      mbar_wait(bars + 8u * s, ph);
      const unsigned tile = ring + s * c.stage_bytes;
      const unsigned row0 = (blockIdx.x + i * gridDim.x) * (unsigned)R;
      if (!(c.flags & 2)) {
        int gq; unsigned hq;
        quant(tile, rowl, row0 + rowl < T, gq, hq);
        if ((lane & 1) == 0) { accG += gq; accH += hq; }
        const unsigned rowaddr = tile + rowl * row_bytes;
        root_unit<GONLY, 0>(lc, ldsoff, rowaddr, gq, hq);
        if (ng_here > 1) root_unit<GONLY, 1>(lc, ldsoff, rowaddr, gq, hq);
        if (ng_here > 2) root_unit<GONLY, 2>(lc, ldsoff, rowaddr, gq, hq);
        if (has_tail) {
          const unsigned tu = ((unsigned)wit + i) & (unsigned)(kTeamWarps - 1);
          if (tu < (unsigned)(R >> 5)) {
            const unsigned trow = (tu << 5) + (unsigned)lane;
            unsigned w0, w1 = 0;
            if (a.tw == 4) w0 = lds_u32(tile + tail_tile_off + trow * 4u);
            else { const uint2 ww = lds_v2(tile + tail_tile_off + trow * 8u); w0 = ww.x; w1 = ww.y; }
            int gqt; unsigned hqt;
            quant(tile, trow, row0 + trow < T, gqt, hqt);
            if (row0 + trow >= T) { w0 = 0; w1 = 0; }
            tail_accumulate<GONLY>(tc, lane, w0, w1, gqt, hqt);
          }
        }
      }
      __syncwarp();
      if (lane == 0) mbar_arrive(bars + 8u * (c.S + s));
      i += kTeams; s += kTeams;
      if (s >= (unsigned)c.S) { s -= (unsigned)c.S; ph ^= 1u; }
    }
    if (wend == my_ntiles) break;
    named_bar_sync(1, NCW * 32);
    spill_main<PL>(reinterpret_cast<int*>(smem_raw), ng_here, out_main, false, threadIdx.x, NCW * 32);
    if (has_tail) spill_tail<PL>(reinterpret_cast<int*>(smem_raw + c.tail_off), a.tw, c.trep, out_tail, false, threadIdx.x, NCW * 32);
    named_bar_sync(1, NCW * 32);
  }
  named_bar_sync(1, NCW * 32);
  spill_main<PL>(reinterpret_cast<int*>(smem_raw), ng_here, out_main, true, threadIdx.x, NCW * 32);
  if (has_tail) spill_tail<PL>(reinterpret_cast<int*>(smem_raw + c.tail_off), a.tw, c.trep, out_tail, true, threadIdx.x, NCW * 32);
  if (a.accumulate_sum && blockIdx.y == 0) {
#pragma unroll
    for (int o = 16; o > 0; o >>= 1) { accG += __shfl_xor_sync(0xffffffffu, accG, o); accH += __shfl_xor_sync(0xffffffffu, accH, o); }
    if (lane == 0 && (accG != 0 || accH != 0)) { red_global_s64(&a.node_sum[nid].g, accG); red_global_s64(&a.node_sum[nid].h, accH); }
  }
}

template <int TW, bool GPAY> struct Stage { unsigned id; typename std::conditional<GPAY, float, float2>::type gr; unsigned t0; };
template <bool GPAY> struct Stage<8, GPAY> { unsigned id; typename std::conditional<GPAY, float, float2>::type gr; unsigned t0, t1; };

__host__ __device__ constexpr int gather_tail_replicas(int ng) { return ng >= 3 ? 4 : 8; }
__host__ __device__ constexpr int gather_tail_bytes(int ng) { return ng >= 3 ? 32768 : 65536; }
__host__ __device__ constexpr int gather_super_rows(int ng) { return 32 / (2 * ng) * (2 * ng); }

__device__ __forceinline__ void gather_split(unsigned T, unsigned C, unsigned sup, unsigned& ceff, unsigned& chunk) {
  ceff = (T + kMinRowsPerCta - 1) / kMinRowsPerCta;
  ceff = ceff < 1 ? 1 : (ceff > C ? C : ceff);
  chunk = (T + ceff - 1) / ceff;
  chunk = (chunk + sup - 1) / sup * sup;
}

template <int TWC, int TREP>
__device__ __forceinline__ void flush_partials(int* smem, int* tsm, int ng_here, bool has_tail, int2* part_main, int2* part_tail, GH64* out_tail,
                                               int tid, int nthr) {
  constexpr int kHalf = kGroupEntries / 2;
#pragma unroll 1
  for (int i = tid; i < ng_here * kHalf; i += nthr) {
    const int k = i / kHalf, e = (i - k * kHalf) * 2;
    int2* G = reinterpret_cast<int2*>(smem + k * 2 * kGroupEntries + e);
    int2* H = G + kHalf;
    const int2 g = *G, h = *H;
    *reinterpret_cast<int4*>(part_main + (size_t)k * kGroupEntries + e) = make_int4(g.x, h.x, g.y, h.y);
    *G = make_int2(0, 0); *H = make_int2(0, 0);
  }
  if (has_tail) {
    constexpr int kTailPlane = 256 * TWC * TREP;
    for (int e = tid; e < 256 * TWC; e += nthr) {
      const int bin = e / TWC, slot = e - bin * TWC;
      long long g = 0, h = 0;
#pragma unroll
      for (int r = 0; r < TREP; ++r) {
        int* t = tsm + (bin * TREP + r) * TWC + slot;
        g += t[0]; h += (unsigned)t[kTailPlane];
        t[0] = 0; t[kTailPlane] = 0;
      }
      if (g != (long long)(int)g) { red_global_s64(&out_tail[e].g, g); g = 0; }
      if (h != (long long)(unsigned)h) { red_global_s64(&out_tail[e].h, h); h = 0; }
      part_tail[e] = make_int2((int)g, (int)(unsigned)h);
    }
  }
}

template <int NG, int TW, int NTHREADS, bool GPAY>
__global__ void __launch_bounds__(NTHREADS, NG == 1 ? (TW ? 1 : 3) : 1) hist_gather_kernel(HistArgs a) {
  constexpr bool TAIL = TW != 0;
  constexpr int NWARPS = NTHREADS / 32;
  constexpr int LPR = 2 * NG, RPI = 32 / LPR, U = 2 * NG;
  constexpr int SUP = RPI * U;
  static_assert(SUP == gather_super_rows(NG), "hist_reduce_kernel splits the rows with gather_super_rows");
  static_assert(kWindowRowsSmall / (SUP * NWARPS) >= 1, "window too small");
  const unsigned iters_per_window = (unsigned)a.window_rows / (SUP * NWARPS);
  extern __shared__ __align__(16) int smem[];
  const int nb = *a.build_count;
  if (nb <= 0) return;
  const unsigned T = a.build_prefix[nb];
  if (T == 0) return;
  if (a.rows_counter && blockIdx.x == 0 && blockIdx.y == 0 && threadIdx.x == 0) atomicAdd(a.rows_counter, (unsigned long long)T);
  unsigned ceff, chunk;
  gather_split(T, gridDim.x, SUP, ceff, chunk);
  if (blockIdx.x >= ceff) return;
  unsigned long long r0l = (unsigned long long)blockIdx.x * chunk;
  if (r0l >= T) return;
  unsigned r0 = (unsigned)r0l;
  unsigned r1 = (unsigned long long)r0 + chunk > T ? T : r0 + chunk;
  const int g0 = blockIdx.y * a.ng_chunk;
  const int ng_here = min(min(a.ng_chunk, NG), a.ngroups - g0);
  const bool has_tail = TAIL && a.tw > 0 && blockIdx.y == gridDim.y - 1;
  const float sg = a.scales[0], sh = a.scales[1];
  const unsigned smem_g = (unsigned)__cvta_generic_to_shared(smem);
  const bool aligned = a.ridx != nullptr && a.bins_gather != nullptr;
  constexpr bool kLineTail = NG == 3 && TW == 8;
  const bool tail_line = kLineTail && aligned && a.tail_in_gather;
  const int64_t row_stride = aligned ? (int64_t)a.gather_stride : (int64_t)a.row_stride;
  const int lane = threadIdx.x & 31, warp = threadIdx.x >> 5;
  const int q = lane / LPR, c = lane - q * LPR;
  const bool lane_on = q < RPI && (c >> 1) < ng_here;
  const int rot = q < RPI ? NG * q + (c >> 1) : 15;
  const LaneConst lc = make_lane_const_rot(rot, c & 1, smem_g + (unsigned)((q < RPI ? (c >> 1) : 0) * 2 * kPlaneBytes));
  const int rot_qw = rot >> 2, rot_qb8 = (rot & 3) * 8;
  const uint8_t* gbins = (aligned ? a.bins_gather : a.bins) + (int64_t)g0 * kSlots + c * 16;
  constexpr int TWC = TAIL ? TW : 4;
  constexpr int trep = gather_tail_replicas(NG) < gather_tail_bytes(NG) / (2 * 256 * 4 * TWC) ? gather_tail_replicas(NG) : gather_tail_bytes(NG) / (2 * 256 * 4 * TWC);
  const unsigned tail_base_rep = smem_g + (unsigned)(NG * 2 * kPlaneBytes) + (unsigned)((lane / TWC) % trep) * (unsigned)TWC * 4u;

  {
    const int words4 = (NG * 2 * kPlaneBytes + (TAIL ? 2 * 256 * TWC * trep * 4 : 0)) / 16;
    for (int i = threadIdx.x; i < words4; i += NTHREADS) reinterpret_cast<int4*>(smem)[i] = make_int4(0, 0, 0, 0);
  }
  __syncthreads();

  int b = 0;
  { int lo = 0, hi = nb; while (lo < hi) { int mid = (lo + hi) >> 1; if (a.build_prefix[mid + 1] > r0) hi = mid; else lo = mid + 1; } b = lo; }

  const size_t slot_entries = (size_t)a.ngroups * kGroupEntries + (size_t)256 * a.tw;
  typedef Stage<TW, GPAY> StageT;
  const unsigned hq_one = (unsigned)__float2int_rn(1.0f * sh);
  while (r0 < r1) {
    const unsigned nbeg = a.build_prefix[b], nend_node = a.build_prefix[b + 1];
    const unsigned nend = nend_node < r1 ? nend_node : r1;
    const int nid = a.build_nid[b];
    const unsigned seg = a.seg_begin[nid];
    GH64* out_slot = a.hist_pool + (size_t)a.hist_slot[nid] * slot_entries;
    GH64* out_main = out_slot + (size_t)g0 * kGroupEntries;
    GH64* out_tail = out_slot + (size_t)a.ngroups * kGroupEntries;
    int accG = 0; unsigned accH = 0;
    const unsigned pa = seg + (r0 - nbeg), pb = seg + (nend - nbeg);
    const unsigned nsuper = (pb - pa + SUP - 1) / SUP;
    const unsigned iters = (nsuper + NWARPS - 1) / NWARPS;

    auto load_ids = [&](unsigned st) -> StageT {
      StageT s_; s_.id = 0xffffffffu; s_.gr = {}; s_.t0 = 0u;
      if constexpr (TW == 8) s_.t1 = 0u;
      unsigned p = pa + st * SUP + lane;
      if (lane < SUP && st < nsuper && p < pb) {
        s_.id = a.ridx ? __ldg(a.ridx + p) : p;
        if constexpr (GPAY) s_.gr = __uint_as_float(ldg_nc_u32(a.gpos + p)); else s_.gr = ldg_nc_f2(a.gpair + p);
        if (TAIL && has_tail && !tail_line) {
          if constexpr (TW == 8) { const uint2 v = ldg_nc_v2(a.bins_tail + (int64_t)s_.id * 8); s_.t0 = v.x; s_.t1 = v.y; }
          else if (a.tail_pos) s_.t0 = ldg_nc_u32(a.tail_pos + p);
          else s_.t0 = ldg_nc_u32(a.bins_tail + (int64_t)s_.id * 4);
        }
      }
      return s_;
    };
    auto load_unit = [&](unsigned ids, int k) -> uint4 {
      const unsigned rid = __shfl_sync(0xffffffffu, ids, q < RPI ? k * RPI + q : 0);
      return (lane_on && rid != 0xffffffffu) ? ldg_nc_v4(gbins + (int64_t)rid * row_stride) : make_uint4(0, 0, 0, 0);
    };
    auto load_line_tail = [&](StageT& s_) {
      if constexpr (TAIL) {
        if (tail_line && has_tail && s_.id != 0xffffffffu) {
          const uint8_t* t = a.bins_gather + (int64_t)s_.id * row_stride + a.ngroups * kSlots;
          if constexpr (TW == 8) { const uint2 v = ldg_nc_v2(t); s_.t0 = v.x; s_.t1 = v.y; } else s_.t0 = ldg_nc_u32(t);
        }
      }
    };
    StageT cur = load_ids(warp);
    StageT nxt = load_ids(warp + NWARPS);
    uint4 w[U];
#pragma unroll
    for (int k = 0; k < U; ++k) w[k] = load_unit(cur.id, k);
    load_line_tail(cur);
    for (unsigned it = 0; it < iters; ++it) {
      const unsigned s = warp + it * NWARPS;
      StageT nn = load_ids(s + 2 * NWARPS);
      const bool active = s < nsuper;
      int gq_l; unsigned hq_l;
      if constexpr (GPAY) { gq_l = __float2int_rn(cur.gr * sg); hq_l = cur.id != 0xffffffffu ? hq_one : 0u; }
      else { gq_l = __float2int_rn(cur.gr.x * sg); hq_l = (unsigned)__float2int_rn(cur.gr.y * sh); }
      accG += gq_l; accH += hq_l;
#pragma unroll
      for (int k = 0; k < U; ++k) {
        if (active) {
          int gq = __shfl_sync(0xffffffffu, gq_l, q < RPI ? k * RPI + q : 0);
          unsigned hq = __shfl_sync(0xffffffffu, hq_l, q < RPI ? k * RPI + q : 0);
          if (!lane_on) { gq = 0; hq = 0; }
          unsigned ww[4];
          rotate_words_bytes(rot_qw, rot_qb8, w[k], ww);
          accumulate16_pairs_prerotated<0>(lc.A, ww, gq, hq);
        }
        w[k] = load_unit(nxt.id, k);
      }
      if constexpr (TAIL) { if (active && has_tail) { unsigned t1 = 0; if constexpr (TW == 8) t1 = cur.t1; tail_accumulate_ct<TWC, trep>(tail_base_rep, lane, cur.t0, t1, gq_l, hq_l); } }
      load_line_tail(nxt);
      cur = nxt; nxt = nn;
      if ((it + 1) % iters_per_window == 0 && it + 1 < iters) {
        if (a.accumulate_sum && blockIdx.y == 0) { flush_node_sum(a.node_sum + nid, accG, accH, lane); accG = 0; accH = 0; }
        __syncthreads();
        spill_main<2>(smem, ng_here, out_main, false, threadIdx.x, NTHREADS);
        if (has_tail) spill_tail<2>(smem + NG * 2 * kGroupEntries, TWC, trep, out_tail, false, threadIdx.x, NTHREADS);
        __syncthreads();
      }
    }
    __syncthreads();
    if (a.partials) {
      int2* part = a.partials + (size_t)(blockIdx.x + b) * slot_entries;
      flush_partials<TWC, trep>(smem, smem + NG * 2 * kGroupEntries, ng_here, has_tail, part + (size_t)g0 * kGroupEntries,
                                part + (size_t)a.ngroups * kGroupEntries, out_tail, threadIdx.x, NTHREADS);
    } else {
      spill_main<2>(smem, ng_here, out_main, true, threadIdx.x, NTHREADS);
      if (has_tail) spill_tail<2>(smem + NG * 2 * kGroupEntries, TWC, trep, out_tail, true, threadIdx.x, NTHREADS);
    }
    __syncthreads();
    if (a.accumulate_sum && blockIdx.y == 0) flush_node_sum(a.node_sum + nid, accG, accH, lane);
    r0 = nend; ++b;
  }
}

__global__ void __launch_bounds__(256) hist_reduce_kernel(HistArgs a, unsigned C, unsigned sup) {
  const int nb = *a.build_count;
  if (nb <= 0) return;
  const unsigned T = a.build_prefix[nb];
  if (T == 0) return;
  unsigned ceff, chunk;
  gather_split(T, C, sup, ceff, chunk);
  const size_t slot_entries = (size_t)a.ngroups * kGroupEntries + (size_t)256 * a.tw;
  const size_t pairs = slot_entries / 2;
  for (size_t item = (size_t)blockIdx.x * blockDim.x + threadIdx.x; item < (size_t)nb * pairs; item += (size_t)gridDim.x * blockDim.x) {
    const int b = (int)(item / pairs);
    const size_t p = item - (size_t)b * pairs;
    const unsigned nbeg = a.build_prefix[b], nend = a.build_prefix[b + 1];
    if (nbeg == nend) continue;
    const unsigned x_lo = nbeg / chunk, nseg = (nend - 1) / chunk - x_lo + 1;
    const int4* src = reinterpret_cast<const int4*>(a.partials + (size_t)(x_lo + b) * slot_entries) + p;
    long long g0 = 0, h0 = 0, g1 = 0, h1 = 0;
    auto add = [&](const int4& v) { g0 += v.x; h0 += (unsigned)v.y; g1 += v.z; h1 += (unsigned)v.w; };
    unsigned s = 0;
    for (; s + 8 <= nseg; s += 8) {
      int4 v[8];
#pragma unroll
      for (int j = 0; j < 8; ++j) v[j] = __ldcs(src + (size_t)(s + j) * pairs);
#pragma unroll
      for (int j = 0; j < 8; ++j) add(v[j]);
    }
    for (; s < nseg; ++s) add(__ldcs(src + (size_t)s * pairs));
    longlong2* o = reinterpret_cast<longlong2*>(a.hist_pool + (size_t)a.hist_slot[a.build_nid[b]] * slot_entries + 2 * p);
    longlong2 e0 = o[0], e1 = o[1];
    e0.x += g0; e0.y += h0; e1.x += g1; e1.y += h1;
    o[0] = e0; o[1] = e1;
  }
}

static thread_local const char* g_last_kernel = "none";
const char* hist_last_kernel() { return g_last_kernel; }

static int chunks_for(int ngroups) { return (ngroups + 2) / 3; }
static int groups_per_chunk(int ngroups) { const int nc = chunks_for(ngroups); return (ngroups + nc - 1) / nc; }
static int gather_grid_x(int ngroups, int tw, int num_sms) {
  const int nchunks = chunks_for(ngroups);
  const int per_sm = groups_per_chunk(ngroups) > 1 ? 1 : (tw ? 1 : 3);
  return (num_sms * per_sm + nchunks - 1) / nchunks;
}
size_t hist_partial_entries(int ngroups, int tw, int num_sms, int max_build) {
  return ((size_t)gather_grid_x(ngroups, tw, num_sms) + (size_t)max_build) * hist_slot_entries(ngroups, tw);
}

static bool root_plan(int ngc, int tw, bool gonly, RootCfg* c) {
  const int PL = gonly ? 1 : 2;
  const unsigned main_b = (unsigned)ngc * PL * kPlaneBytes;
  const unsigned avail = kMaxSmem - 128  - 2 * 8 * 16 ;
  const unsigned stage = (unsigned)kRootRows * (32u * ngc + (gonly ? 4u : 8u) + tw);
  int trep = tw ? 32 / tw : 0;
  unsigned tail_b = (unsigned)PL * 256u * tw * trep * 4u;
  if (tw && main_b + tail_b + kTeams * stage > avail) { trep = 1; tail_b = (unsigned)PL * 256u * tw * 4u; }
  if (main_b + tail_b + kTeams * stage > avail) return false;
  int S = (int)((avail - main_b - tail_b) / stage);
  int smax = 16;
  if (const char* e = getenv("B200XGB_ROOT_S")) smax = atoi(e);
  if (S > smax) S = smax;
  constexpr int kStageQuantum = kTeams % kRootProducerWarps == 0 ? kTeams : kTeams * kRootProducerWarps;
  S -= S % kStageQuantum;
  if (S < kTeams) return false;
  c->S = S; c->trep = trep; c->box_groups = ngc; c->tail_off = main_b; c->ring_off = main_b + tail_b; c->stage_bytes = stage;
  c->total = main_b + tail_b + 128 + (unsigned)S * stage + 2 * 8 * (unsigned)S;
  c->flags = 0;
  if (const char* f = getenv("B200XGB_ROOT_FLAGS")) c->flags = atoi(f);
  return true;
}

typedef CUresult (*EncodeTiledFn)(CUtensorMap*, CUtensorMapDataType, cuuint32_t, void*, const cuuint64_t*, const cuuint64_t*, const cuuint32_t*,
                                  const cuuint32_t*, CUtensorMapInterleave, CUtensorMapSwizzle, CUtensorMapL2promotion, CUtensorMapFloatOOBfill);
static EncodeTiledFn encode_fn() {
  static EncodeTiledFn fn = [] {
    void* p = nullptr; cudaDriverEntryPointQueryResult q;
    if (cudaGetDriverEntryPoint("cuTensorMapEncodeTiled", &p, cudaEnableDefault, &q) != cudaSuccess || q != cudaDriverEntryPointSuccess) { cudaGetLastError(); p = nullptr; }
    return reinterpret_cast<EncodeTiledFn>(p);
  }();
  return fn;
}

static bool get_tensor_map(const uint8_t* bins, int64_t n, int row_stride, int box_groups, int R, CUtensorMap* out) {
  typedef std::tuple<const void*, int64_t, int, int, int> Key;
  static std::map<Key, CUtensorMap> cache; static std::mutex mu;
  std::lock_guard<std::mutex> lk(mu);
  const Key key(bins, n, row_stride, box_groups, R);
  auto it = cache.find(key);
  if (it != cache.end()) { *out = it->second; return true; }
  EncodeTiledFn fn = encode_fn();
  if (!fn) return false;
  CUtensorMap tm;
  const cuuint64_t dims[2] = {(cuuint64_t)row_stride, (cuuint64_t)n};
  const cuuint64_t strides[1] = {(cuuint64_t)row_stride};
  const cuuint32_t box[2] = {(cuuint32_t)(32 * box_groups), (cuuint32_t)R};
  const cuuint32_t estr[2] = {1, 1};
  CUresult r = fn(&tm, CU_TENSOR_MAP_DATA_TYPE_UINT8, 2, const_cast<uint8_t*>(bins), dims, strides, box, estr, CU_TENSOR_MAP_INTERLEAVE_NONE,
                  CU_TENSOR_MAP_SWIZZLE_NONE, CU_TENSOR_MAP_L2_PROMOTION_L2_128B, CU_TENSOR_MAP_FLOAT_OOB_FILL_NONE);
  if (r != CUDA_SUCCESS) return false;
  if (cache.size() > 64) cache.clear();
  cache[key] = tm; *out = tm;
  return true;
}

template <int NG, int TW, int NT> static void set_gather_attr() {
  const int smem = NG * 2 * kPlaneBytes + (TW ? gather_tail_bytes(NG) : 0);
  CUDA_OK(cudaFuncSetAttribute(hist_gather_kernel<NG, TW, NT, false>, cudaFuncAttributeMaxDynamicSharedMemorySize, smem));
  CUDA_OK(cudaFuncSetAttribute(hist_gather_kernel<NG, TW, NT, true>, cudaFuncAttributeMaxDynamicSharedMemorySize, smem));
}

void hist_configure() {
  static bool configured = false;
  if (configured) return;
  set_gather_attr<1, 0, 256>(); set_gather_attr<1, 4, 256>(); set_gather_attr<1, 8, 256>();
  set_gather_attr<2, 0, 768>(); set_gather_attr<2, 4, 768>(); set_gather_attr<2, 8, 768>();
  set_gather_attr<3, 0, 768>(); set_gather_attr<3, 4, 768>(); set_gather_attr<3, 8, 768>();
  CUDA_OK(cudaFuncSetAttribute(hist_root_kernel<false>, cudaFuncAttributeMaxDynamicSharedMemorySize, kMaxSmem));
  CUDA_OK(cudaFuncSetAttribute(hist_root_kernel<true>, cudaFuncAttributeMaxDynamicSharedMemorySize, kMaxSmem));
  configured = true;
}

template <int NG, int NT, bool GPAY>
static void launch_gather_tw(const HistArgs& a, int gx, int nchunks, cudaStream_t stream) {
  const int smem = NG * 2 * kPlaneBytes + (a.tw ? gather_tail_bytes(NG) : 0);
  if (a.tw == 0) hist_gather_kernel<NG, 0, NT, GPAY><<<dim3(gx, nchunks), NT, smem, stream>>>(a);
  else if (a.tw == 4) hist_gather_kernel<NG, 4, NT, GPAY><<<dim3(gx, nchunks), NT, smem, stream>>>(a);
  else hist_gather_kernel<NG, 8, NT, GPAY><<<dim3(gx, nchunks), NT, smem, stream>>>(a);
}
template <int NG, int NT>
static void launch_gather(const HistArgs& a, int gx, int nchunks, cudaStream_t stream) {
  if (a.gpos) launch_gather_tw<NG, NT, true>(a, gx, nchunks, stream); else launch_gather_tw<NG, NT, false>(a, gx, nchunks, stream);
}

void launch_hist_build(const HistArgs& a_in, int num_sms, cudaStream_t stream) {
  HistArgs a = a_in;
  const int nchunks = chunks_for(a.ngroups);
  a.ng_chunk = groups_per_chunk(a.ngroups);
  static const bool no_tma = getenv("B200XGB_NO_TMA") != nullptr;
  const bool gonly = a.g_only != 0;
  B200_CHECK(!gonly || a.gpos != nullptr, "hist: the G-only root pass reads the dense g (gpos)");
  if (a.ridx == nullptr && !no_tma && !a.force_gather && (a.gpos == nullptr || gonly)) {
    RootCfg c; CUtensorMap tm;
    if (root_plan(a.ng_chunk, a.tw, gonly, &c) && get_tensor_map(a.bins, a.n, a.row_stride, c.box_groups, kRootRows, &tm)) {
      const int gx = num_sms / nchunks > 0 ? num_sms / nchunks : 1;
      if (gonly) hist_root_kernel<true><<<dim3(gx, nchunks), kRootThreads, c.total, stream>>>(tm, a, c);
      else hist_root_kernel<false><<<dim3(gx, nchunks), kRootThreads, c.total, stream>>>(tm, a, c);
      g_last_kernel = gonly ? "hist_root_kernel<GONLY>" : "hist_root_kernel<GH>";
      ++g_kernel_launches;
      CUDA_OK(cudaGetLastError());
      return;
    }
  }
  B200_CHECK(!a.g_only || a.ridx == nullptr, "hist: G-only accumulation is a root-pass mode");
  B200_CHECK(!a.g_only, "hist: the G-only root pass needs the TMA kernel (tensor-map creation failed or B200XGB_NO_TMA is set)");
  static const bool red_flush = getenv("B200XGB_HIST_RED_FLUSH") != nullptr;
  if (red_flush) a.partials = nullptr;
  else B200_CHECK(a.partials != nullptr, "hist: the gathered passes need the builder's partial histograms");
  const int ng = a.ng_chunk;
  const int gx = gather_grid_x(a.ngroups, a.tw, num_sms);
  if (ng == 1) launch_gather<1, 256>(a, gx, nchunks, stream);
  else if (ng == 2) launch_gather<2, 768>(a, gx, nchunks, stream);
  else launch_gather<3, 768>(a, gx, nchunks, stream);
  g_last_kernel = "hist_gather_kernel";
  ++g_kernel_launches;
  CUDA_OK(cudaGetLastError());
  if (a.partials) {
    hist_reduce_kernel<<<num_sms * 8, 256, 0, stream>>>(a, (unsigned)gx, (unsigned)gather_super_rows(ng));
    ++g_kernel_launches;
    CUDA_OK(cudaGetLastError());
  }
}

}
```

sagemaker-xgboost-container_b200/csrc/tree.cu:

```cuda
#include <algorithm>
#include <type_traits>
#include "engine.h"
#include "rng.h"
#include "split_math.h"
#include "tree.h"

namespace b200 {


__device__ __forceinline__ void interaction_children(const ApplyArgs& a, int nid, int f, int Lc, int Rc) {
  if (a.node_allowed == nullptr) return;
  const size_t F = (size_t)a.F;
  unsigned char* pl = a.node_path + (size_t)Lc * F; unsigned char* pr = a.node_path + (size_t)Rc * F;
  unsigned char* al = a.node_allowed + (size_t)Lc * F; unsigned char* ar = a.node_allowed + (size_t)Rc * F;
  const unsigned char* pp = a.node_path + (size_t)nid * F;
  for (int j = 0; j < a.F; ++j) { const unsigned char v = (pp[j] || j == f) ? 1 : 0; pl[j] = v; pr[j] = v; al[j] = v; ar[j] = v; }
  for (int s = 0; s < a.n_ic_sets; ++s) {
    const unsigned char* set = a.ic_sets + (size_t)s * F;
    bool relevant = true;
    for (int j = 0; j < a.F && relevant; ++j) if (pl[j] && !set[j]) relevant = false;
    if (relevant) for (int j = 0; j < a.F; ++j) if (set[j]) { al[j] = 1; ar[j] = 1; }
  }
}

__device__ __forceinline__ float clamp_weight(float w, float lo, float hi) { return w < lo ? lo : (w > hi ? hi : w); }
__device__ __forceinline__ float gain_at_weight(const TrainParamDev& p, double G, double H, float w) {
  if (H <= 0.0) return 0.0f;
  return gain_at_weight_f((float)G, (float)H, p.lambda, w);
}
__device__ __forceinline__ bool constrained_split_gain(const TrainParamDev& p, double GL, double HL, double GR, double HR, float lo, float hi, int c, float* gain) {
  const float wl = clamp_weight(calc_weight(p, GL, HL), lo, hi), wr = clamp_weight(calc_weight(p, GR, HR), lo, hi);
  *gain = gain_at_weight(p, GL, HL, wl) + gain_at_weight(p, GR, HR, wr);
  return c == 0 || (c > 0 ? wl <= wr : wl >= wr);
}

__device__ __forceinline__ unsigned long long cand_key(float loss, int f, int ord) {
  if (!(loss > 0.0f) || isinf(loss)) return 0ull;
  return ((unsigned long long)__float_as_uint(loss) << 32) | ((unsigned long long)(0x7FFFFFu - (unsigned)f) << 9) |
         (unsigned long long)(0x1FFu - (unsigned)ord);
}

__global__ void init_tree_kernel(GrowState gs, TreeArrays t, unsigned n) {
  if (threadIdx.x != 0 || blockIdx.x != 0) return;
  *gs.n_nodes = 1; *gs.n_leaves = 1;
  *gs.n_slots = kLgFirstFreeSlot; *gs.lg_done = 0; gs.depth[0] = 0; gs.open[0] = 0;
  gs.lower[0] = -INFINITY; gs.upper[0] = INFINITY;
  for (int d = 0; d < kMaxDepth + 2; ++d) gs.level_count[d] = 0;
  gs.level_count[0] = 1; gs.level_nodes[0] = 0;
  gs.seg_begin[0] = 0; gs.seg_count[0] = n; gs.hist_slot[0] = kLgRootSlot;
  gs.node_sum[0].g = 0; gs.node_sum[0].h = 0;
  *gs.build_count = 1; gs.build_nid[0] = 0; gs.build_sub_nid[0] = -1; gs.build_parent_slot[0] = -1;
  gs.build_prefix[0] = 0; gs.build_prefix[1] = n;
  t.left[0] = -1; t.right[0] = -1; t.parent[0] = 2147483647; t.split_index[0] = 0; t.split_bin[0] = -1;
  t.default_left[0] = 0; t.split_cond[0] = 0.f; t.base_weight[0] = 0.f; t.loss_chg[0] = 0.f; t.sum_hess[0] = 0.f;
}

__global__ void scales_kernel(GrowState gs, int grad_bits) {
  if (threadIdx.x != 0 || blockIdx.x != 0) return;
  float mg = __uint_as_float(gs.absmax[0]), mh = __uint_as_float(gs.absmax[1]);
  int eg = 0, eh = 0;
  if (mg > 0.f && isfinite(mg)) frexpf(mg, &eg);
  if (mh > 0.f && isfinite(mh)) frexpf(mh, &eh);
  float sg = ldexpf(1.0f, grad_bits - eg), sh = ldexpf(1.0f, grad_bits + 1 - eh);
  gs.scales[0] = sg; gs.scales[1] = sh; gs.scales[2] = 1.0f / sg; gs.scales[3] = 1.0f / sh;
}

constexpr int kEvalSegs = 32, kEvalBinsPerSeg = kBins / kEvalSegs;
__global__ void __launch_bounds__(32 * kEvalSegs) eval_kernel(EvalArgs a) {
  const int li = blockIdx.x;
  if (li >= a.gs.level_count[a.level]) return;
  const int nid = a.gs.level_nodes[(size_t)a.level * a.max_level_nodes + li];
  const int group = blockIdx.y;
  const bool is_tail = group == a.ngroups;
  const int nblocks = a.ngroups + (a.tw > 0 ? 1 : 0);
  const int64_t slot_entries = (int64_t)a.ngroups * kGroupEntries + 256 * a.tw;
  const GH64* hist = a.hist_pool + (int64_t)a.gs.hist_slot[nid] * slot_entries + (int64_t)group * kGroupEntries;
  const int stride = is_tail ? a.tw : kSlots;
  const int slot = threadIdx.x & 31, seg = threadIdx.x >> 5;
  const int f = group * kSlots + slot;
  bool active = slot < stride && f < a.F && (a.feat_mask == nullptr || a.feat_mask[f] != 0);
  if (active && a.node_allowed != nullptr) active = a.node_allowed[(size_t)nid * a.F + f] != 0;
  if (a.feat_mask != nullptr && a.colsample_bynode < 1.0f) {
    __shared__ int s_rank[32], s_cnt;
    if (threadIdx.x < 32) s_rank[threadIdx.x] = 0;
    if (threadIdx.x == 0) s_cnt = 0;
    __syncthreads();
    const unsigned long long stream = 0x80000000ull + ((unsigned long long)(unsigned)*a.tree_index << 20) + (unsigned long long)nid;
    const float uf = rng_uniform(a.seed, stream, (unsigned long long)f);
    int rank = 0, cnt = 0;
    for (int g = seg; g < a.F; g += kEvalSegs) {
      if (a.feat_mask[g]) { ++cnt; const float ug = rng_uniform(a.seed, stream, (unsigned long long)g); rank += (ug < uf || (ug == uf && g < f)) ? 1 : 0; }
    }
    if (rank) atomicAdd(&s_rank[slot], rank);
    if (slot == 0 && cnt) atomicAdd(&s_cnt, cnt);
    __syncthreads();
    const int keep = max(1, (int)floorf(a.colsample_bynode * (float)s_cnt));
    active = active && s_rank[slot] < keep;
  }
  const int nbf = active ? a.cut_ptrs[f + 1] - a.cut_ptrs[f] : 0;
  const double isg = (double)a.gs.scales[2], ish = (double)a.gs.scales[3];
  const GH64 tot = a.gs.node_sum[nid];
  const double G = (double)tot.g * isg, H = (double)tot.h * ish;
  const bool mono = a.monotone != nullptr;
  const float w_lo = mono ? a.gs.lower[nid] : 0.f, w_hi = mono ? a.gs.upper[nid] : 0.f;
  const int mono_c = (mono && active) ? a.monotone[f] : 0;
  const float node_w = mono ? clamp_weight(calc_weight(a.p, G, H), w_lo, w_hi) : calc_weight(a.p, G, H);
  const float root_gain = mono ? gain_at_weight(a.p, G, H, node_w) : calc_gain(a.p, G, H);
  if (threadIdx.x == 0 && group == 0) { a.gs.root_gain[nid] = root_gain; a.gs.weight[nid] = node_w; }

  __shared__ long long segG[kEvalSegs][32], segH[kEvalSegs][32];
  __shared__ unsigned long long wkey[kEvalSegs];
  const int b0 = seg * kEvalBinsPerSeg;
  GH64 vals[kEvalBinsPerSeg];
  long long sG = 0, sH = 0;
#pragma unroll
  for (int i = 0; i < kEvalBinsPerSeg; ++i) { int b = b0 + i; GH64 v; v.g = 0; v.h = 0; if (b < nbf) v = hist[b * stride + slot]; vals[i] = v; sG += v.g; sH += v.h; }
  segG[seg][slot] = sG; segH[seg][slot] = sH;
  __syncthreads();
  long long pG = 0, pH = 0, tG = 0, tH = 0;
#pragma unroll 8
  for (int s = 0; s < kEvalSegs; ++s) { long long x = segG[s][slot], y = segH[s][slot]; if (s < seg) { pG += x; pH += y; } tG += x; tH += y; }
  const bool fmiss = a.has_missing && (tG != tot.g || tH != tot.h);

  SplitCand best; best.loss_chg = 0.f; best.feature = 0; best.bin = -1; best.dleft = 0; best.ord = 0; best.GL = 0; best.HL = 0;
  unsigned long long bkey = 0ull;
  const double mcw = (double)a.p.min_child_weight;
  long long cG = pG, cH = pH;
#pragma unroll
  for (int i = 0; i < kEvalBinsPerSeg; ++i) {
    int b = b0 + i;
    if (b < nbf) {
      GH64 v = vals[i]; cG += v.g; cH += v.h;
      double GL = (double)cG * isg, HL = (double)cH * ish;
      double GR = (double)(tot.g - cG) * isg, HR = (double)(tot.h - cH) * ish;
      if (HL >= mcw && HR >= mcw) {
        float lc;
        if (mono) { float gsum; lc = constrained_split_gain(a.p, GL, HL, GR, HR, w_lo, w_hi, mono_c, &gsum) ? gsum - root_gain : 0.0f; }
        else lc = calc_split_gain(a.p, GL, HL, GR, HR) - root_gain;
        unsigned long long k = cand_key(lc, f, b);
        if (k > bkey) { bkey = k; best.loss_chg = lc; best.feature = f; best.bin = b; best.dleft = 0; best.ord = b; best.GL = cG; best.HL = cH; }
      }
    }
  }
  if (fmiss) {
    long long rG = tG - pG, rH = tH - pH;
#pragma unroll
    for (int i = 0; i < kEvalBinsPerSeg; ++i) {
      int b = b0 + i;
      if (b < nbf) {
        long long lG = tot.g - rG, lH = tot.h - rH;
        double GL = (double)lG * isg, HL = (double)lH * ish, GR = (double)rG * isg, HR = (double)rH * ish;
// ... 30 lines not shown
    unsigned v = i < n ? in[i] : 0u, x = v;
#pragma unroll
    for (int o = 1; o < 32; o <<= 1) { unsigned y = __shfl_up_sync(0xffffffffu, x, o); if (lane >= o) x += y; }
    if (lane == 31) s_tmp[warp] = x;
    __syncthreads();
    if (warp == 0) {
      unsigned w = lane < nw ? s_tmp[lane] : 0u, z = w;
#pragma unroll
      for (int o = 1; o < 32; o <<= 1) { unsigned y = __shfl_up_sync(0xffffffffu, z, o); if (lane >= o) z += y; }
      s_tmp[lane] = z - w;
      if (lane == 31) s_tmp[32] = z;
    }
    __syncthreads();
    if (i < n) out[i] = carry + s_tmp[warp] + x - v;
    carry += s_tmp[32];
    __syncthreads();
  }
  return carry;
}

__device__ __forceinline__ SplitCand best_of_blocks(const ApplyArgs& a, int nid) {
  SplitCand best = a.gs.best_group[(size_t)nid * a.nblocks];
  unsigned long long bk = cand_key(best.loss_chg, best.feature, best.ord);
  for (int g = 1; g < a.nblocks; ++g) {
    SplitCand c = a.gs.best_group[(size_t)nid * a.nblocks + g];
    unsigned long long k = cand_key(c.loss_chg, c.feature, c.ord);
    if (k > bk) { bk = k; best = c; }
  }
  a.gs.best[nid] = best;
  return best;
}

__device__ __forceinline__ bool split_is_valid(const TrainParamDev& p, const SplitCand& best, const GH64& tot, int depth) {
  bool ok = best.loss_chg > 1e-6f;
  if (ok && (best.HL == 0 || tot.h - best.HL == 0)) ok = false;
  if (ok && best.loss_chg < p.gamma) ok = false;
  if (ok && p.max_depth > 0 && depth >= p.max_depth) ok = false;
  return ok;
}

__device__ __forceinline__ void finish_root(const ApplyArgs& a, double ish) {
  const GrowState& gs = a.gs; const TreeArrays& t = a.tree;
  t.base_weight[0] = gs.weight[0]; t.sum_hess[0] = (float)((double)gs.node_sum[0].h * ish); t.split_cond[0] = a.p.eta * gs.weight[0];
}

__device__ __forceinline__ void expand_node(const ApplyArgs& a, int nid, const SplitCand& best, const GH64& tot, int Lc, int Rc, double isg, double ish) {
  const GrowState& gs = a.gs; const TreeArrays& t = a.tree;
  const long long GLq = best.GL, HLq = best.HL, GRq = tot.g - best.GL, HRq = tot.h - best.HL;
  const double GL = (double)GLq * isg, HL = (double)HLq * ish, GR = (double)GRq * isg, HR = (double)HRq * ish;
  float wl = calc_weight(a.p, GL, HL), wr = calc_weight(a.p, GR, HR);
  if (a.monotone) {
    const float lo = gs.lower[nid], hi = gs.upper[nid];
    wl = clamp_weight(wl, lo, hi); wr = clamp_weight(wr, lo, hi);
    const float mid = (wl + wr) / 2.0f; const int mc = a.monotone[best.feature];
    gs.lower[Lc] = lo; gs.upper[Lc] = hi; gs.lower[Rc] = lo; gs.upper[Rc] = hi;
    if (mc < 0) { gs.lower[Lc] = mid; gs.upper[Rc] = mid; } else if (mc > 0) { gs.upper[Lc] = mid; gs.lower[Rc] = mid; }
  }
  interaction_children(a, nid, best.feature, Lc, Rc);
  const int cb = a.cut_ptrs[best.feature];
  const float thr = best.dleft ? (best.bin < 0 ? a.min_vals[best.feature] : a.cut_vals[cb + best.bin]) : a.cut_vals[cb + best.bin];
  t.left[nid] = Lc; t.right[nid] = Rc; t.split_index[nid] = best.feature; t.split_cond[nid] = thr;
  t.split_bin[nid] = best.bin; t.default_left[nid] = (unsigned char)best.dleft;
  t.base_weight[nid] = gs.weight[nid]; t.loss_chg[nid] = best.loss_chg; t.sum_hess[nid] = (float)((double)tot.h * ish);
  const int ch[2] = {Lc, Rc}; const float cw[2] = {wl, wr}; const double chh[2] = {HL, HR};
  for (int s = 0; s < 2; ++s) {
    const int c = ch[s];
    t.left[c] = -1; t.right[c] = -1; t.parent[c] = nid; t.split_index[c] = 0; t.split_bin[c] = -1; t.default_left[c] = 0;
    t.split_cond[c] = a.p.eta * cw[s]; t.base_weight[c] = a.p.eta * cw[s]; t.loss_chg[c] = 0.f; t.sum_hess[c] = (float)chh[s];
  }
  gs.node_sum[Lc].g = GLq; gs.node_sum[Lc].h = HLq; gs.node_sum[Rc].g = GRq; gs.node_sum[Rc].h = HRq;
  gs.seg_begin[Lc] = 0; gs.seg_count[Lc] = 0; gs.seg_begin[Rc] = 0; gs.seg_count[Rc] = 0;
}

__device__ __forceinline__ void plan_child_hists(const GrowState& gs, int r, int nid, const SplitCand& best, const GH64& tot, int Lc, int Rc,
                                                 int bld_slot, int sub_slot) {
  const bool fewer_right = tot.h - best.HL < best.HL;
  const int bld = fewer_right ? Rc : Lc, sub = fewer_right ? Lc : Rc;
  gs.hist_slot[bld] = bld_slot; gs.hist_slot[sub] = sub_slot;
  gs.build_nid[r] = bld; gs.build_sub_nid[r] = sub; gs.build_parent_slot[r] = gs.hist_slot[nid];
}

__global__ void __launch_bounds__(256) apply_kernel(ApplyArgs a) {
  __shared__ unsigned s_tmp[33];
  GrowState& gs = a.gs;
  const int L = a.level;
  const int cnt = gs.level_count[L];
  const int* nodes = gs.level_nodes + (size_t)L * a.max_level_nodes;
  unsigned* valid = a.scratch;
  unsigned* rank = a.scratch + a.max_level_nodes;
  unsigned* tiles = a.scratch + 2 * (size_t)a.max_level_nodes;
  const double isg = (double)gs.scales[2], ish = (double)gs.scales[3];
  if (L == 0 && threadIdx.x == 0 && cnt > 0) finish_root(a, ish);
  for (int i = threadIdx.x; i < cnt; i += blockDim.x) {
    const int nid = nodes[i];
    const SplitCand best = best_of_blocks(a, nid);
    valid[i] = split_is_valid(a.p, best, gs.node_sum[nid], L) ? 1u : 0u;
  }
  __syncthreads();
  if (a.p.max_leaves > 0 && threadIdx.x == 0) {
    int leaves = *gs.n_leaves;
    for (int i = 0; i < cnt; ++i) { if (valid[i]) { if (leaves >= a.p.max_leaves) valid[i] = 0; else ++leaves; } }
  }
  __syncthreads();
  const unsigned nvalid = block_exclusive_scan(valid, rank, cnt, s_tmp);
  const int n0 = *gs.n_nodes;
  const bool children_evaluated = (L + 1 < a.p.max_depth) || a.p.max_depth == 0;
  for (int i = threadIdx.x; i < cnt; i += blockDim.x) {
    const int nid = nodes[i];
    tiles[i] = (gs.seg_count[nid] + kPartTile - 1) / kPartTile;
    gs.part_action[i] = (int)valid[i];
    if (!valid[i]) continue;
    const SplitCand best = gs.best[nid];
    const GH64 tot = gs.node_sum[nid];
    const int r = (int)rank[i];
    const int Lc = n0 + 2 * r, Rc = Lc + 1;
    expand_node(a, nid, best, tot, Lc, Rc, isg, ish);
    if (children_evaluated) {
      int* nxt = gs.level_nodes + (size_t)(L + 1) * a.max_level_nodes;
      nxt[2 * r] = Lc; nxt[2 * r + 1] = Rc;
      plan_child_hists(gs, r, nid, best, tot, Lc, Rc, a.next_base + r, a.next_base + a.next_half + r);
    }
  }
  __syncthreads();
  const unsigned total_tiles = block_exclusive_scan(tiles, gs.tile_prefix, cnt, s_tmp);
  if (threadIdx.x == 0) {
    gs.tile_prefix[cnt] = total_tiles;
    *gs.n_nodes = n0 + 2 * (int)nvalid;
    *gs.n_leaves += (int)nvalid;
    gs.level_count[L + 1] = children_evaluated ? 2 * (int)nvalid : 0;
    *gs.build_count = children_evaluated ? (int)nvalid : 0;
  }
}

__global__ void __launch_bounds__(256) apply_lossguide_kernel(ApplyArgs a, int iter) {
  __shared__ unsigned long long s_key[8];
  GrowState& gs = a.gs;
  const double isg = (double)gs.scales[2], ish = (double)gs.scales[3];
  const int src = iter == 0 ? 0 : 1;
  const int cnt = gs.level_count[src];
  const int* nodes = gs.level_nodes + (size_t)src * a.max_level_nodes;
  if (iter == 0 && threadIdx.x == 0 && cnt > 0) finish_root(a, ish);
  for (int i = threadIdx.x; i < cnt; i += blockDim.x) {
    const int nid = nodes[i];
    gs.open[nid] = best_of_blocks(a, nid).loss_chg > 1e-6f ? 1 : 0;
  }
  __syncthreads();
  const int n0 = *gs.n_nodes;
  unsigned long long key = 0ull;
  for (int nid = threadIdx.x; nid < n0; nid += blockDim.x)
    if (gs.open[nid]) { unsigned long long k = ((unsigned long long)__float_as_uint(gs.best[nid].loss_chg) << 32) | (unsigned long long)(0xffffffffu - (unsigned)nid); key = k > key ? k : key; }
#pragma unroll
  for (int o = 16; o > 0; o >>= 1) { unsigned long long x = __shfl_xor_sync(0xffffffffu, key, o); key = x > key ? x : key; }
  if ((threadIdx.x & 31) == 0) s_key[threadIdx.x >> 5] = key;
  __syncthreads();
  if (threadIdx.x != 0) return;
  for (int w = 1; w < 8; ++w) key = s_key[w] > key ? s_key[w] : key;
  bool stop = *gs.lg_done != 0 || key == 0ull;
  int nid = 0; SplitCand best{}; GH64 tot{};
  if (!stop) {
    nid = (int)(0xffffffffu - (unsigned)(key & 0xffffffffull));
    best = gs.best[nid]; tot = gs.node_sum[nid];
    stop = !split_is_valid(a.p, best, tot, gs.depth[nid]) || (a.p.max_leaves > 0 && *gs.n_leaves == a.p.max_leaves);
  }
  if (stop) {
    *gs.lg_done = 1;
    gs.level_count[0] = 0; gs.level_count[1] = 0; *gs.build_count = 0; gs.part_action[0] = 0; gs.tile_prefix[0] = 0; gs.tile_prefix[1] = 0;
// ... 131 lines not shown
    }
    const int lane = threadIdx.x & 31, warp = threadIdx.x >> 5;
    unsigned x = mine;
#pragma unroll
    for (int o = 1; o < 32; o <<= 1) { unsigned y = __shfl_up_sync(0xffffffffu, x, o); if (lane >= o) x += y; }
    if (lane == 31) s_w[warp] = x;
    __syncthreads();
    unsigned woff = 0, tile_left = 0;
    for (int w = 0; w < 8; ++w) { if (w < warp) woff += s_w[w]; tile_left += s_w[w]; }
    unsigned long long* desc = gs.tile_desc + t0;
    if (threadIdx.x == 0) st_relaxed_u64(desc + lt, (lt == 0 ? kDescPrefix : kDescAggregate) | tile_left);
    unsigned lbefore = woff + x - mine;
#pragma unroll
    for (int j = 0; j < 8; ++j) {
      if (fl[j] == 2) continue;
      const unsigned jj = threadIdx.x * 8 + j;
      const unsigned slot = fl[j] ? lbefore++ : tile_left + (jj - lbefore);
      s_rid[slot] = rows[j]; s_gp[slot] = gp[j]; if constexpr (TL) s_tl[slot] = tl[j];
    }
    unsigned lefts_before = 0;
    if (warp == 0 && lt > 0) {
      lefts_before = lookback_lefts(desc, lt);
      if (lane == 0) st_relaxed_u64(desc + lt, kDescPrefix | (lefts_before + tile_left));
    }
    __syncthreads();
    if (threadIdx.x == 0) s_w[0] = lefts_before;
    __syncthreads();
    lefts_before = s_w[0];
    const unsigned rights_before = lt * kPartTile - lefts_before;
    const int Lc = a.tree.left[nid], Rc = a.tree.right[nid];
    bool write_left = true, write_right = true;
    if (a.build_only) { const bool build_right = gs.node_sum[Rc].h < gs.node_sum[Lc].h; write_left = !build_right; write_right = build_right; }
    const unsigned k0 = write_left ? 0u : tile_left, k1 = write_right ? nrows : tile_left;
    const unsigned dl0 = b + lefts_before, dr0 = b + c - 1 - rights_before + tile_left;
    for (unsigned k = k0 + threadIdx.x; k < k1; k += blockDim.x) {
      const unsigned dest = k < tile_left ? dl0 + k : dr0 - k;
      a.ridx_next[dest] = s_rid[k];
      gp_next[dest] = s_gp[k];
      if constexpr (TL) a.tl_next[dest] = s_tl[k];
    }
    if (threadIdx.x == 0) {
      if (lt == gs.tile_prefix[i + 1] - t0 - 1) {
        const unsigned nl = lefts_before + tile_left;
        gs.seg_begin[Lc] = b; gs.seg_count[Lc] = nl; gs.seg_begin[Rc] = b + nl; gs.seg_count[Rc] = c - nl;
      }
      if (a.rows_counter) { atomicAdd(a.rows_counter, (unsigned long long)nrows); atomicAdd(a.rows_counter + 1, (unsigned long long)(k1 - k0)); }
    }
  }
  __syncthreads();
  if (threadIdx.x == 0) { __threadfence(); s_w[0] = atomicAdd(gs.part_ctl + 1, 1u) == gridDim.x - 1 ? 1u : 0u; }
  __syncthreads();
  if (!s_w[0]) return;
  __threadfence();
  const int nb = *gs.build_count;
  for (int r = threadIdx.x; r < nb; r += blockDim.x) gs.build_prefix[r] = __ldcg(gs.seg_count + gs.build_nid[r]);
  __syncthreads();
  const unsigned tot = nb > 0 ? block_exclusive_scan(gs.build_prefix, gs.build_prefix, nb, s_rid ) : 0u;
  if (threadIdx.x == 0) gs.build_prefix[nb > 0 ? nb : 0] = tot;
}

struct PackedNode { unsigned feat; unsigned short bin_dl; unsigned short left; };
constexpr int kPackedNodesSmem = 2048;
static_assert(sizeof(PackedNode) == 8, "PackedNode is 8 B");
__device__ __forceinline__ PackedNode pack_node(const TreeArrays& t, int i) {
  PackedNode p; p.feat = (unsigned)t.split_index[i]; p.bin_dl = (unsigned short)((t.split_bin[i] + 1) | (t.default_left[i] ? 0x8000 : 0));
  const int l = t.left[i]; p.left = l < 0 ? 0xffff : (unsigned short)l;
  return p;
}
__device__ __forceinline__ bool goes_left(const PackedNode& p, int byte, int has_missing) {
  return (has_missing && byte == kMissingBin) ? ((p.bin_dl & 0x8000) != 0) : (byte < (int)(p.bin_dl & 0x7fff));
}

__device__ __forceinline__ void stage_route_tables(const RouteArgs& a, PackedNode* s_node, unsigned char* s_bidx, int nb) {
  const int nn = *a.gs.n_nodes;
  for (int i = threadIdx.x; i < kRouteMaxNodes; i += blockDim.x) {
    if (s_node) { PackedNode p{0u, 0, 0xffff}; if (i < nn) p = pack_node(a.tree, i); s_node[i] = p; }
    s_bidx[i] = 0xff;
  }
  __syncthreads();
  for (int r = threadIdx.x; r < nb; r += blockDim.x) s_bidx[a.gs.build_nid[r]] = (unsigned char)r;
  __syncthreads();
}

constexpr int kRuns = kRouteTile / 1024;
__global__ void __launch_bounds__(256) route_kernel(RouteArgs a) {
  __shared__ PackedNode s_node[kRouteMaxNodes];
  __shared__ unsigned char s_bidx[kRouteMaxNodes];
  __shared__ unsigned s_cnt[kRouteMaxBuild];
  const int nb = *a.gs.build_count;
  if (a.level > 0 && nb == 0) return;
  const int64_t r0 = (int64_t)blockIdx.x * kRouteTile + threadIdx.x * 4;
  const int lane = threadIdx.x & 31;
  unsigned ids[kRuns], out[kRuns];
#pragma unroll
  for (int j = 0; j < kRuns; ++j) {
    const int64_t r = r0 + j * 1024;
    ids[j] = 0u; out[j] = 0u;
    if (a.level > 0) {
      if (r + 4 <= a.n) ids[j] = *reinterpret_cast<const unsigned*>(a.node_of_row + r);
      else for (int e = 0; e < 4; ++e) if (r + e < a.n) ids[j] |= (unsigned)a.node_of_row[r + e] << (8 * e);
    }
  }
  if (threadIdx.x < kRouteMaxBuild) s_cnt[threadIdx.x] = 0;
  stage_route_tables(a, s_node, s_bidx, nb);
  int byte[4 * kRuns];
#pragma unroll
  for (int q = 0; q < 4 * kRuns; ++q) {
    const int64_t r = r0 + (q >> 2) * 1024 + (q & 3);
    const PackedNode p = s_node[(ids[q >> 2] >> (8 * (q & 3))) & 0xffu];
    byte[q] = (r < a.n && p.left != 0xffff) ? a.bins_col[(int64_t)p.feat * a.n + r] : 0;
  }
#pragma unroll
  for (int q = 0; q < 4 * kRuns; ++q) {
    const int64_t r = r0 + (q >> 2) * 1024 + (q & 3);
    const unsigned id = (ids[q >> 2] >> (8 * (q & 3))) & 0xffu;
    const PackedNode p = s_node[id];
    const unsigned child = p.left == 0xffff ? id : (goes_left(p, byte[q], a.has_missing) ? p.left : p.left + 1u);
    out[q >> 2] |= child << (8 * (q & 3));
    const unsigned c = r < a.n ? s_bidx[child] : 0xffu;
    const unsigned m = __match_any_sync(0xffffffffu, c);
    if (c != 0xffu && lane == __ffs(m) - 1) atomicAdd(&s_cnt[c], (unsigned)__popc(m));
  }
#pragma unroll
  for (int j = 0; j < kRuns; ++j) {
    const int64_t r = r0 + j * 1024;
    if (a.level > 0 && out[j] == ids[j]) continue;
    if (r + 4 <= a.n) *reinterpret_cast<unsigned*>(a.node_of_row + r) = out[j];
    else for (int e = 0; e < 4; ++e) if (r + e < a.n) a.node_of_row[r + e] = (uint8_t)(out[j] >> (8 * e));
  }
  __syncthreads();
  for (int c = threadIdx.x; c < nb; c += blockDim.x) a.tile_counts[(size_t)c * a.ntiles + blockIdx.x] = s_cnt[c];
  if (a.rows_counter && threadIdx.x == 0) {
    const int64_t t0 = (int64_t)blockIdx.x * kRouteTile;
    atomicAdd(a.rows_counter, (unsigned long long)(a.n - t0 < (int64_t)kRouteTile ? a.n - t0 : (int64_t)kRouteTile));
  }
}

__global__ void __launch_bounds__(1024) route_scan_kernel(RouteArgs a) {
  __shared__ unsigned s_run[1024], s_tmp[33];
  const int c = blockIdx.x;
  if (c >= *a.gs.build_count) return;
  unsigned* cnt = a.tile_counts + (size_t)c * a.ntiles;
  const unsigned per = (a.ntiles + blockDim.x - 1) / blockDim.x, t0 = threadIdx.x * per, t1 = min(t0 + per, a.ntiles);
  unsigned sum = 0;
#pragma unroll 8
  for (unsigned t = t0; t < t1; ++t) sum += cnt[t];
  s_run[threadIdx.x] = sum;
  __syncthreads();
  const unsigned tot = block_exclusive_scan(s_run, s_run, (int)blockDim.x, s_tmp);
  unsigned run = s_run[threadIdx.x];
#pragma unroll 8
  for (unsigned t = t0; t < t1; ++t) { const unsigned v = cnt[t]; cnt[t] = run; run += v; }
  if (threadIdx.x == 0) a.gs.seg_count[a.gs.build_nid[c]] = tot;
}

constexpr int kWarpRows = kRouteTile / 8, kWarpSteps = kWarpRows / 32;
template <bool GONLY, bool TL>
__global__ void __launch_bounds__(256, 4) scatter_kernel(RouteArgs a) {
  typedef typename std::conditional<GONLY, float, float2>::type Pay;
  __shared__ unsigned char s_bidx[kRouteMaxNodes];
  __shared__ unsigned s_start[kRouteMaxBuild];
  __shared__ unsigned s_local[kRouteMaxBuild + 1];
  __shared__ unsigned s_dst[kRouteMaxBuild];
  __shared__ unsigned s_wofs[8][kRouteMaxBuild];
  __shared__ unsigned s_rid[kRouteTile];
  __shared__ Pay s_gp[kRouteTile];
  __shared__ unsigned s_tl[TL ? kRouteTile : 1];
  __shared__ unsigned char s_ch[kRouteTile];
  const GrowState& gs = a.gs;
  const int nb = *gs.build_count;
  if (nb == 0) { if (blockIdx.x == 0 && threadIdx.x == 0) gs.build_prefix[0] = 0; return; }
  stage_route_tables(a, nullptr, s_bidx, nb);
  if (threadIdx.x < nb) s_start[threadIdx.x] = gs.seg_count[gs.build_nid[threadIdx.x]];
  __syncthreads();
  if (threadIdx.x == 0) {
    unsigned run = 0;
    for (int c = 0; c < nb; ++c) {
      const unsigned t = s_start[c]; s_start[c] = run;
      if (blockIdx.x == 0) { gs.build_prefix[c] = run; gs.seg_begin[gs.build_nid[c]] = run; }
      run += t;
    }
    if (blockIdx.x == 0) gs.build_prefix[nb] = run;
  }
  const int lane = threadIdx.x & 31, warp = threadIdx.x >> 5;
  const unsigned lanes_below = (1u << lane) - 1u;
  for (unsigned tile = blockIdx.x; tile < a.ntiles; tile += gridDim.x) {
    const int64_t rw = (int64_t)tile * kRouteTile + warp * kWarpRows + lane;
    unsigned ck[kWarpSteps];
#pragma unroll
    for (int it = 0; it < kWarpSteps; ++it) { const int64_t r = rw + it * 32; ck[it] = r < a.n ? a.node_of_row[r] : kRouteMaxNodes - 1; }
    const unsigned toff = threadIdx.x < nb ? a.tile_counts[(size_t)threadIdx.x * a.ntiles + tile] : 0u;
    __syncthreads();
    for (int i = threadIdx.x; i < 8 * kRouteMaxBuild; i += blockDim.x) s_wofs[i / kRouteMaxBuild][i % kRouteMaxBuild] = 0;
    __syncthreads();
#pragma unroll
    for (int it = 0; it < kWarpSteps; ++it) {
      const unsigned c = s_bidx[ck[it]];
      const unsigned m = __match_any_sync(0xffffffffu, c);
      const unsigned before = c != 0xffu ? s_wofs[warp][c] : 0u;
      __syncwarp();
      if (c != 0xffu && lane == __ffs(m) - 1) s_wofs[warp][c] = before + __popc(m);
      __syncwarp();
      ck[it] = c << 16 | (before + __popc(m & lanes_below));
    }
    __syncthreads();
    if (threadIdx.x < nb) {
      unsigned t = 0;
      for (int w = 0; w < 8; ++w) t += s_wofs[w][threadIdx.x];
      s_local[threadIdx.x + 1] = t;
    }
    __syncthreads();
    if (threadIdx.x == 0) { s_local[0] = 0; for (int c = 0; c < nb; ++c) s_local[c + 1] += s_local[c]; }
    __syncthreads();
    if (threadIdx.x < nb) {
      const unsigned c = threadIdx.x;
      unsigned run = s_local[c];
      s_dst[c] = s_start[c] + toff - run;
      for (int w = 0; w < 8; ++w) { const unsigned t = s_wofs[w][c]; s_wofs[w][c] = run; run += t; }
    }
    __syncthreads();
#pragma unroll
    for (int h = 0; h < kWarpSteps; h += 8) {
      Pay pv[8]; unsigned tv[8];
#pragma unroll
      for (int j = 0; j < 8; ++j) {
        const unsigned r = (unsigned)(rw + (h + j) * 32);
        pv[j] = Pay{}; tv[j] = 0u;
        if ((ck[h + j] >> 16) != 0xffu) {
          if constexpr (GONLY) pv[j] = __ldg(a.g + r); else pv[j] = __ldg(a.gpair + r);
          if constexpr (TL) tv[j] = __ldg(a.tail_row + r);
        }
      }
#pragma unroll
      for (int j = 0; j < 8; ++j) {
        const unsigned c = ck[h + j] >> 16;
        if (c == 0xffu) continue;
        const unsigned k = s_wofs[warp][c] + (ck[h + j] & 0xffffu);
        s_rid[k] = (unsigned)(rw + (h + j) * 32); s_gp[k] = pv[j]; s_ch[k] = (unsigned char)c;
        if constexpr (TL) s_tl[k] = tv[j];
      }
    }
    __syncthreads();
    const unsigned built = s_local[nb];
    for (unsigned k = threadIdx.x; k < built; k += blockDim.x) {
      const unsigned pos = s_dst[s_ch[k]] + k;
      a.ridx[pos] = s_rid[k]; static_cast<Pay*>(a.gp)[pos] = s_gp[k];
      if constexpr (TL) a.tl[pos] = s_tl[k];
    }
    if (a.rows_counter && threadIdx.x == 0) atomicAdd(a.rows_counter + 1, (unsigned long long)built);
  }
}

__global__ void __launch_bounds__(256) update_margin_kernel(TreeArrays t, const int* n_nodes, const uint8_t* bins_col, int64_t n, int has_missing,
                                                            const uint8_t* node_of_row, float* margin, int K, int k, const float* leaf_scale) {
  __shared__ PackedNode s_nodes[kPackedNodesSmem];
  __shared__ float s_leaf[kPackedNodesSmem];
  const int nn = *n_nodes;
  const bool packed = nn <= kPackedNodesSmem && nn < 0xffff;
  if (packed) {
    for (int i = threadIdx.x; i < nn; i += blockDim.x) { s_nodes[i] = pack_node(t, i); s_leaf[i] = t.split_cond[i]; }
    __syncthreads();
  }
  const int64_t base = (int64_t)blockIdx.x * 1024 + threadIdx.x;
  int nid[4]; bool done[4];
#pragma unroll
  for (int j = 0; j < 4; ++j) {
    const int64_t r = base + j * 256;
    nid[j] = (node_of_row != nullptr && r < n) ? (int)node_of_row[r] : 0;
    done[j] = r >= n || (packed ? (s_nodes[nid[j]].left == 0xffff) : (t.left[nid[j]] == -1));
  }
  bool any = !(done[0] && done[1] && done[2] && done[3]);
  while (any) {
    int byte[4];
#pragma unroll
    for (int j = 0; j < 4; ++j) {
      const int f = packed ? (int)s_nodes[nid[j]].feat : t.split_index[nid[j]];
      byte[j] = done[j] ? 0 : bins_col[(int64_t)f * n + base + j * 256];
    }
    any = false;
#pragma unroll
    for (int j = 0; j < 4; ++j) {
      if (done[j]) continue;
      const int nd = nid[j];
      if (packed) {
        const PackedNode p = s_nodes[nd];
        nid[j] = goes_left(p, byte[j], has_missing) ? p.left : p.left + 1;
        done[j] = s_nodes[nid[j]].left == 0xffff;
      } else {
        const bool left = (has_missing && byte[j] == kMissingBin) ? (t.default_left[nd] != 0) : (byte[j] <= t.split_bin[nd]);
        nid[j] = left ? t.left[nd] : t.right[nd];
        done[j] = t.left[nid[j]] == -1;
      }
      any |= !done[j];
    }
  }
  const float sc = *leaf_scale;
#pragma unroll
  for (int j = 0; j < 4; ++j) { const int64_t r = base + j * 256; if (r < n) margin[r * K + k] = __fadd_rn(margin[r * K + k], __fmul_rn(sc, packed ? s_leaf[nid[j]] : t.split_cond[nid[j]])); }
}

__global__ void __launch_bounds__(256) subtract_kernel(GrowState gs, GH64* pool, size_t stride) {
  const int r = blockIdx.x;
  if (r >= *gs.build_count) return;
  const int bld = gs.build_nid[r], sub = gs.build_sub_nid[r];
  const GH64* hb = pool + (size_t)gs.hist_slot[bld] * stride;
  const GH64* hp = pool + (size_t)gs.build_parent_slot[r] * stride;
  GH64* hs = pool + (size_t)gs.hist_slot[sub] * stride;
  for (size_t e = (size_t)blockIdx.y * blockDim.x + threadIdx.x; e < stride; e += (size_t)gridDim.y * blockDim.x) {
    GH64 p = hp[e], b = hb[e]; GH64 o; o.g = p.g - b.g; o.h = p.h - b.h; hs[e] = o;
  }
}

void launch_init_tree(const GrowState& gs, const TreeArrays& t, unsigned n, cudaStream_t s) {
  init_tree_kernel<<<1, 32, 0, s>>>(gs, t, n); ++g_kernel_launches; CUDA_OK(cudaGetLastError());
}
void launch_scales(const GrowState& gs, int grad_bits, cudaStream_t s) { scales_kernel<<<1, 32, 0, s>>>(gs, grad_bits); ++g_kernel_launches; CUDA_OK(cudaGetLastError()); }
void launch_eval(const EvalArgs& a, int max_nodes_level, cudaStream_t s) {
  dim3 grid(max_nodes_level, a.ngroups + (a.tw > 0 ? 1 : 0)); eval_kernel<<<grid, 32 * kEvalSegs, 0, s>>>(a); ++g_kernel_launches; CUDA_OK(cudaGetLastError());
}
void launch_apply_lossguide(const ApplyArgs& a, int iter, cudaStream_t s) { apply_lossguide_kernel<<<1, 256, 0, s>>>(a, iter); ++g_kernel_launches; CUDA_OK(cudaGetLastError()); }
void launch_lg_copy_back(const PartArgs& a, unsigned* ridx_dst, void* gp_dst, unsigned* tl_dst, unsigned max_tiles, cudaStream_t s) {
  const unsigned grid = max_tiles < 1184u ? max_tiles : 1184u;
  if (a.g_only) lg_copy_back_kernel<float><<<grid, 256, 0, s>>>(a, ridx_dst, static_cast<float*>(gp_dst), tl_dst);
  else lg_copy_back_kernel<float2><<<grid, 256, 0, s>>>(a, ridx_dst, static_cast<float2*>(gp_dst), tl_dst);
  ++g_kernel_launches; CUDA_OK(cudaGetLastError());
}
void launch_zero_build_slots(const GrowState& gs, GH64* pool, size_t slot_entries, int max_build, cudaStream_t s) {
  dim3 grid(max_build, (unsigned)((slot_entries + 1023) / 1024)); zero_build_slots_kernel<<<grid, 256, 0, s>>>(gs, pool, slot_entries); ++g_kernel_launches; CUDA_OK(cudaGetLastError());
}
void launch_lg_stage(const GrowState& gs, GH64* pool, size_t slot_entries, int to_stage, cudaStream_t s) {
  lg_stage_kernel<<<(unsigned)((slot_entries + 1023) / 1024), 256, 0, s>>>(gs, pool, slot_entries, to_stage); ++g_kernel_launches; CUDA_OK(cudaGetLastError());
}
void launch_apply(const ApplyArgs& a, cudaStream_t s) { apply_kernel<<<1, 256, 0, s>>>(a); ++g_kernel_launches; CUDA_OK(cudaGetLastError()); }
void launch_partition(const PartArgs& a, unsigned max_tiles, cudaStream_t s) {
  CUDA_OK(cudaMemsetAsync(a.gs.tile_desc, 0, sizeof(unsigned long long) * ((size_t)max_tiles + 1), s));
  const bool tl = a.tl_cur != nullptr;
  if (a.g_only) { if (tl) part_kernel<true, true><<<max_tiles, 256, 0, s>>>(a); else part_kernel<true, false><<<max_tiles, 256, 0, s>>>(a); }
  else { if (tl) part_kernel<false, true><<<max_tiles, 256, 0, s>>>(a); else part_kernel<false, false><<<max_tiles, 256, 0, s>>>(a); }
  ++g_kernel_launches; CUDA_OK(cudaGetLastError());
}
void launch_route(const RouteArgs& a, cudaStream_t s) {
  if (a.ntiles == 0) return;
  route_kernel<<<a.ntiles, 256, 0, s>>>(a); ++g_kernel_launches; CUDA_OK(cudaGetLastError());
  route_scan_kernel<<<1u << a.level, 1024, 0, s>>>(a); ++g_kernel_launches; CUDA_OK(cudaGetLastError());
  const bool tl = a.tail_row != nullptr;
  const unsigned grid = std::min(a.ntiles, 4u * (unsigned)engine_num_sms());
  if (a.g_only) { if (tl) scatter_kernel<true, true><<<grid, 256, 0, s>>>(a); else scatter_kernel<true, false><<<grid, 256, 0, s>>>(a); }
  else { if (tl) scatter_kernel<false, true><<<grid, 256, 0, s>>>(a); else scatter_kernel<false, false><<<grid, 256, 0, s>>>(a); }
  ++g_kernel_launches; CUDA_OK(cudaGetLastError());
}
void launch_update_margin(const TreeArrays& t, const int* n_nodes, const uint8_t* bins_col, int64_t n, int has_missing, const uint8_t* node_of_row,
                          float* margin, int K, int k, const float* leaf_scale, cudaStream_t s) {
  if (n == 0) return;
  update_margin_kernel<<<(unsigned)((n + 1023) / 1024), 256, 0, s>>>(t, n_nodes, bins_col, n, has_missing, node_of_row, margin, K, k, leaf_scale);
  ++g_kernel_launches; CUDA_OK(cudaGetLastError());
}
void launch_subtract(const GrowState& gs, GH64* pool, size_t slot_entries, int max_build, cudaStream_t s) {
  dim3 grid(max_build, (unsigned)((slot_entries + 1023) / 1024)); subtract_kernel<<<grid, 256, 0, s>>>(gs, pool, slot_entries); ++g_kernel_launches; CUDA_OK(cudaGetLastError());
}

}
```

sagemaker-xgboost-container_b200/csrc/tree.h:

```cpp
#pragma once
#include "engine.h"

namespace b200 {

constexpr unsigned kPartTile = 2048;

struct TrainParamDev {
  float eta, lambda, alpha, gamma, min_child_weight, max_delta_step;
  int max_depth, max_leaves;
};

struct EvalArgs {
  const GH64* hist_pool; GrowState gs; const int* cut_ptrs; const unsigned char* feat_mask;
  TrainParamDev p; int F, ngroups, tw, ntail, has_missing, level, max_level_nodes;
  const int* monotone;
  const unsigned char* node_allowed;
  float colsample_bynode; unsigned seed; const int* tree_index;
};

struct ApplyArgs {
  GrowState gs; TreeArrays tree; const int* cut_ptrs; const float* cut_vals; const float* min_vals;
  TrainParamDev p; unsigned* scratch; int nblocks , level, max_level_nodes, next_base, next_half;
  const int* monotone;
  unsigned char* node_path; unsigned char* node_allowed; const unsigned char* ic_sets; int n_ic_sets, F;
};

struct PartArgs {
  GrowState gs; TreeArrays tree; const uint8_t* bins_col; int64_t n; const unsigned* ridx_cur; unsigned* ridx_next;
  const void* gp_cur; void* gp_next; int g_only;
  const unsigned* tl_cur; unsigned* tl_next;
  int has_missing, level, max_level_nodes;
  int build_only;
  unsigned long long* rows_counter;
};

constexpr int kRouteMaxDepth = 7;
constexpr unsigned kRouteTile = 2048;
constexpr int kRouteMaxNodes = 256;
constexpr int kRouteMaxBuild = 1 << (kRouteMaxDepth - 2);
struct RouteArgs {
  GrowState gs; TreeArrays tree; const uint8_t* bins_col; int64_t n;
  uint8_t* node_of_row;
  unsigned* tile_counts;
  unsigned ntiles; int has_missing, level;
  const float* g; const float2* gpair; int g_only; const unsigned* tail_row;
  unsigned* ridx; void* gp; unsigned* tl;
  unsigned long long* rows_counter;
};

struct HistArgs {
  const uint8_t* bins;
  const uint8_t* bins_tail;
  const unsigned* tail_pos;
  int64_t n;
  int row_stride;
  const uint8_t* bins_gather;
  int gather_stride;
  int tail_in_gather;
  int tw;
  const float2* gpair;
  const float* gpos;
  const unsigned* ridx;
  const int* build_count;
  const int* build_nid;
  const unsigned* build_prefix;
  const unsigned* seg_begin;
  const int* hist_slot;
  const float* scales;
  GH64* hist_pool;
  GH64* node_sum;
  int2* partials;
  int ngroups;
  int ng_chunk;
  int accumulate_sum;
  int g_only;
  int window_rows;
  int force_gather;
  unsigned long long* rows_counter;
};

constexpr int kLgRootSlot = 0, kLgStageSlot = 1, kLgFirstFreeSlot = 2;
void launch_apply_lossguide(const ApplyArgs& a, int iter, cudaStream_t s);
void launch_lg_copy_back(const PartArgs& a, unsigned* ridx_dst, void* gp_dst, unsigned* tl_dst, unsigned max_tiles, cudaStream_t s);
void launch_zero_build_slots(const GrowState& gs, GH64* pool, size_t slot_entries, int max_build, cudaStream_t s);
void launch_lg_stage(const GrowState& gs, GH64* pool, size_t slot_entries, int to_stage, cudaStream_t s);
void launch_hist_build(const HistArgs& a, int num_sms, cudaStream_t stream);
size_t hist_partial_entries(int ngroups, int tw, int num_sms, int max_build);
void hist_configure();
const char* hist_last_kernel();
void launch_init_tree(const GrowState& gs, const TreeArrays& t, unsigned n, cudaStream_t s);
void launch_scales(const GrowState& gs, int grad_bits, cudaStream_t s);
void launch_eval(const EvalArgs& a, int max_nodes_level, cudaStream_t s);
void launch_apply(const ApplyArgs& a, cudaStream_t s);
void launch_partition(const PartArgs& a, unsigned max_tiles, cudaStream_t s);
void launch_route(const RouteArgs& a, cudaStream_t s);
void launch_update_margin(const TreeArrays& t, const int* n_nodes, const uint8_t* bins_col, int64_t n, int has_missing, const uint8_t* node_of_row,
                          float* margin, int K, int k, const float* leaf_scale, cudaStream_t s);
void launch_subtract(const GrowState& gs, GH64* pool, size_t slot_entries, int max_build, cudaStream_t s);

}
```

Measured before the change: 109.0.

## Chain tree-growth kernels with programmatic dependent launch and fold memsets into kernels

Per-round tree-growth kernels now launch through cudaLaunchKernelEx with programmatic stream serialization, and each kernel calls griddepcontrol.wait, so a kernel's launch can overlap the tail of the one before it in the captured graph. Separate memsets (root slot zeroing, interaction-constraint buffers, next-level histogram zeroing on the routed path) are folded into existing kernels to cut node count. The route scan kernel is rewritten to use warp-shuffle scans. The intent is to shrink launch gaps between the many small kernels in each round, at the cost of more complex dependency semantics. Some of the new pieces are only partly visible.

```diff
diff --git a/include/b200xgb.h b/include/b200xgb.h
--- a/include/b200xgb.h
+++ b/include/b200xgb.h
@@ -139,6 +139,7 @@
 XGB_DLL int XGB200TimerStop(float* out_ms);
 XGB_DLL int XGB200BoosterSetProfile(BoosterHandle handle, int enable);
 XGB_DLL int XGB200BoosterGetProfile(BoosterHandle handle, const char** out_json);
+XGB_DLL int XGB200BoosterGraphInfo(BoosterHandle handle, const char** out_json);
 XGB_DLL int XGB200LaunchCount(long long* out);
 XGB_DLL int XGB200Synchronize(void);
 XGB_DLL int XGB200LegacyModelToUBJ(const void* buf, bst_ulong len, bst_ulong* out_len, const char** out);
diff --git a/microbench/tree_timeline.py b/microbench/tree_timeline.py
--- /dev/null
+++ b/microbench/tree_timeline.py
@@ -0,0 +1,150 @@
+#!/usr/bin/env python
+import argparse
+import json
+import os
+import re
+import statistics
+import sys
+import tempfile
+
+HERE = os.path.dirname(os.path.dirname(os.path.abspath(__file__)))
+BIG = ("hist_root_kernel", "hist_gather_kernel", "route_kernel", "scatter_kernel", "update_margin_kernel", "gradient_kernel")
+
+
+def family(name):
+    if not name.startswith("void ") and "(" not in name:
+        return name
+    base = name[5:] if name.startswith("void ") else name
+    base = re.sub(r"\(.*$", "", base)
+    depth, out = 0, []
+    for ch in base:
+        if ch == "<":
+            depth += 1
+        elif ch == ">":
+            depth -= 1
+        elif depth == 0:
+            out.append(ch)
+    return "".join(out).split("::")[-1].strip()
+
+
+def device_events(trace_path):
+    ev = json.load(open(trace_path))["traceEvents"]
+    keep = []
+    for e in ev:
+        if e.get("ph") != "X" or e.get("cat") not in ("kernel", "gpu_memcpy", "gpu_memset"):
+            continue
+        keep.append({"name": e["name"], "family": family(e["name"]), "ts": float(e["ts"]), "dur": float(e["dur"])})
+    keep.sort(key=lambda x: x["ts"])
+    return keep
+
+
+def split_rounds(events):
+    starts = [i for i, e in enumerate(events) if e["family"] == "init_tree_kernel"]
+    return [events[a:b] for a, b in zip(starts, starts[1:])]
+
+
+def analyse(rnd, next_start):
+    rows, gaps, overlap = [], 0.0, 0.0
+    fam = {}
+    level, levels = "root", {}
+    prev_end = None
+    for e in rnd:
+        gap = 0.0 if prev_end is None else e["ts"] - prev_end
+        if e["family"] == "apply_kernel":
+            level = "L%d" % sum(1 for k in levels if k.startswith("L"))
+        lv = levels.setdefault(level, {"small_kernel_us": 0.0, "small_launches": 0, "gap_us": 0.0})
+        if gap > 0:
+            gaps += gap; lv["gap_us"] += gap
+        else:
+            overlap -= gap
+        if e["family"] not in BIG:
+            lv["small_kernel_us"] += e["dur"]; lv["small_launches"] += 1
+        f = fam.setdefault(e["family"], {"count": 0, "us": 0.0})
+        f["count"] += 1; f["us"] += e["dur"]
+        rows.append({"name": e["family"], "start_us": e["ts"] - rnd[0]["ts"], "dur_us": e["dur"], "gap_us": gap})
+        prev_end = e["ts"] + e["dur"] if prev_end is None else max(prev_end, e["ts"] + e["dur"])
+    small = sum(v["us"] for k, v in fam.items() if k not in BIG)
+    return {"span_us": next_start - rnd[0]["ts"], "activities": len(rnd), "gap_sum_us": gaps, "overlap_sum_us": overlap,
+            "small_kernel_us": small, "ceiling_us": gaps + small, "families": fam, "levels": levels, "timeline": rows}
+
+
+def card():
+    try:
+        import pynvml
+        pynvml.nvmlInit()
+        h = pynvml.nvmlDeviceGetHandleByIndex(0)
+        name = pynvml.nvmlDeviceGetName(h)
+        return (name.decode() if isinstance(name, bytes) else name), pynvml.nvmlDeviceGetPowerManagementLimit(h) / 1000.0
+    except Exception:
+        return None, None
+
+
+def main():
+    ap = argparse.ArgumentParser()
+    ap.add_argument("--rows", type=int, default=50_000_000)
+    ap.add_argument("--cols", type=int, default=100)
+    ap.add_argument("--max-depth", type=int, default=6)
+    ap.add_argument("--objective", default="reg:squarederror")
+    ap.add_argument("--warmup", type=int, default=5)
+    ap.add_argument("--timed", type=int, default=20, help="graph-replayed rounds timed with CUDA events, profiler off")
+    ap.add_argument("--rounds", type=int, default=5, help="rounds recorded by the profiler")
+    ap.add_argument("--tree", default=HERE, help="checkout whose package and bench.py are measured")
+    ap.add_argument("--label", default="")
+    ap.add_argument("--out-dir", required=True)
+    a = ap.parse_args()
+    tree = os.path.abspath(a.tree)
+    sys.path.insert(0, tree)
+    import torch
+    import bench
+    import sagemaker_xgboost_container_b200 as xgb
+    assert os.path.dirname(os.path.abspath(bench.__file__)) == tree, bench.__file__
+    if not torch.cuda.is_available():
+        raise SystemExit("tree_timeline: no CUDA device")
+    be = xgb.get_backend()
+    dev = torch.device("cuda", 0)
+    ba = argparse.Namespace(rows=a.rows, cols=a.cols, seed=43, objective=a.objective, num_class=0)
+    X, y = bench.gen_shard(ba, 0, a.rows, dev)
+    d = xgb.DMatrix(X, label=y.cpu().numpy())
+    del X
+    torch.cuda.empty_cache()
+    params = bench.params_of(argparse.Namespace(objective=a.objective, max_depth=a.max_depth, max_bin=256, num_class=0))
+    b = xgb.Booster(params, [d])
+    it = 0
+    for _ in range(a.warmup):
+        b.update(d, it); it += 1
+    be.synchronize()
+    be.timer_start()
+    for _ in range(a.timed):
+        b.update(d, it); it += 1
+    round_ms = be.timer_stop() / a.timed
+    from torch.profiler import ProfilerActivity, profile
+    with profile(activities=[ProfilerActivity.CUDA]) as prof:
+        for _ in range(a.rounds + 1):
+            b.update(d, it); it += 1
+        be.synchronize()
+    os.makedirs(a.out_dir, exist_ok=True)
+    with tempfile.TemporaryDirectory() as td:
+        tp = os.path.join(td, "trace.json")
+        prof.export_chrome_trace(tp)
+        events = device_events(tp)
+    starts = [e["ts"] for e in events if e["family"] == "init_tree_kernel"]
+    rounds = [analyse(r, s) for r, s in zip(split_rounds(events), starts[1:])]
+    if not rounds:
+        raise SystemExit("tree_timeline: the trace holds no complete round (%d device activities)" % len(events))
+    med = sorted(rounds, key=lambda r: r["span_us"])[len(rounds) // 2]
+    name, power = card()
+    label = a.label or os.path.basename(tree.rstrip("/"))
+    out = {"label": label, "tree": tree, "gpu": name, "power_limit_w": power, "rows": a.rows, "cols": a.cols, "objective": a.objective,
+           "max_depth": a.max_depth, "round_ms_event_timed": round_ms, "profiled_rounds": len(rounds),
+           "per_round": [{k: r[k] for k in ("span_us", "activities", "gap_sum_us", "overlap_sum_us", "small_kernel_us", "ceiling_us")} for r in rounds],
+           "median": {k: statistics.median(r[k] for r in rounds) for k in ("span_us", "gap_sum_us", "overlap_sum_us", "small_kernel_us", "ceiling_us")},
+           "median_round": med}
+    path = os.path.join(a.out_dir, "timeline_%s.json" % label)
+    json.dump(out, open(path, "w"), indent=1)
+    summary = {"label": label, "gpu": name, "power_limit_w": power, "round_ms": round_ms, "median": out["median"],
+               "levels": med["levels"], "families": {k: round(v["us"], 2) for k, v in med["families"].items()}}
+    print(json.dumps(summary), flush=True)
+
+
+if __name__ == "__main__":
+    main()
diff --git a/sagemaker-xgboost-container_b200/backend.py b/sagemaker-xgboost-container_b200/backend.py
--- a/sagemaker-xgboost-container_b200/backend.py
+++ b/sagemaker-xgboost-container_b200/backend.py
@@ -649,6 +649,11 @@
         self._check(self.lib.XGB200BoosterGetProfile(bh, C.byref(out)))
         return json.loads(out.value.decode())
 
+    def booster_graph_info(self, bh):
+        out = C.c_char_p()
+        self._check(self.lib.XGB200BoosterGraphInfo(bh, C.byref(out)))
+        return json.loads(out.value.decode())
+
     def launch_count(self):
         out = C.c_longlong()
         self._check(self.lib.XGB200LaunchCount(C.byref(out)))
diff --git a/sagemaker-xgboost-container_b200/csrc/booster.cu b/sagemaker-xgboost-container_b200/csrc/booster.cu
--- a/sagemaker-xgboost-container_b200/csrc/booster.cu
+++ b/sagemaker-xgboost-container_b200/csrc/booster.cu
@@ -2173,5 +2173,6 @@
 
 void Booster::set_profile(bool on) { builder_->set_profile(on); }
 std::string Booster::get_profile() { return builder_->profile_json(); }
-
-}
+std::string Booster::graph_info() const { return builder_->graph_json(); }
+
+}
diff --git a/sagemaker-xgboost-container_b200/csrc/booster.h b/sagemaker-xgboost-container_b200/csrc/booster.h
--- a/sagemaker-xgboost-container_b200/csrc/booster.h
+++ b/sagemaker-xgboost-container_b200/csrc/booster.h
@@ -167,6 +167,7 @@
   void debug_gradient(DMatrix* dm, const float* margin, int round, float* out);
   void debug_refresh_sums(std::vector<long long>* out);
   std::string get_profile();
+  std::string graph_info() const;
   void debug_build_root_hist(DMatrix* dm, const float* gpair_host, std::vector<long long>* hist_out, float* scales_out,
                              int repeats, float* ms_out, int mode = 0, const unsigned* row_ids = nullptr, int64_t n_ids = 0);
   std::string debug_eval_root(DMatrix* dm, const long long* hist_fm, long long G, long long H, float max_g, float max_h,
diff --git a/sagemaker-xgboost-container_b200/csrc/capi.cc b/sagemaker-xgboost-container_b200/csrc/capi.cc
--- a/sagemaker-xgboost-container_b200/csrc/capi.cc
+++ b/sagemaker-xgboost-container_b200/csrc/capi.cc
@@ -914,6 +914,9 @@
 int XGB200BoosterGetProfile(BoosterHandle handle, const char** out_json) {
   API_BEGIN(); BoosterBox* box = static_cast<BoosterBox*>(handle); box->ret_str = BST(handle)->get_profile(); *out_json = box->ret_str.c_str(); API_END();
 }
+int XGB200BoosterGraphInfo(BoosterHandle handle, const char** out_json) {
+  API_BEGIN(); BoosterBox* box = static_cast<BoosterBox*>(handle); box->ret_str = BST(handle)->graph_info(); *out_json = box->ret_str.c_str(); API_END();
+}
 int XGB200LaunchCount(long long* out) { API_BEGIN(); *out = g_kernel_launches; API_END(); }
 int XGB200Synchronize(void) { API_BEGIN(); CUDA_OK(cudaStreamSynchronize(engine_stream())); API_END(); }
 int XGB200DMatrixCreateFromColumns(const void* const* cols, const int* col_types, int ncols, bst_ulong nrow, int label_column, int weight_column, DMatrixHandle* out) {
diff --git a/sagemaker-xgboost-container_b200/csrc/engine.h b/sagemaker-xgboost-container_b200/csrc/engine.h
--- a/sagemaker-xgboost-container_b200/csrc/engine.h
+++ b/sagemaker-xgboost-container_b200/csrc/engine.h
@@ -4,6 +4,7 @@
 #include <cstdio>
 #include <stdexcept>
 #include <string>
+#include <utility>
 #include <vector>
 
 namespace b200 {
@@ -17,6 +18,18 @@
 
 cudaStream_t engine_stream();
 int engine_num_sms();
+
+__device__ __forceinline__ void pdl_wait() { asm volatile("griddepcontrol.wait;" ::: "memory"); }
+
+extern thread_local bool g_chain_launches;
+template <typename... P, typename... A>
+inline void launch_chained(void (*kernel)(P...), dim3 grid, dim3 block, size_t smem, cudaStream_t s, A&&... args) {
+  cudaLaunchAttribute attr;
+  attr.id = cudaLaunchAttributeProgrammaticStreamSerialization; attr.val.programmaticStreamSerializationAllowed = 1;
+  cudaLaunchConfig_t cfg{grid, block, smem, s, &attr, g_chain_launches ? 1u : 0u};
+  CUDA_OK(cudaLaunchKernelEx(&cfg, kernel, std::forward<A>(args)...));
+  ++g_kernel_launches;
+}
 
 void devmem_note(int64_t delta);
 void devmem_query(uint64_t* live, uint64_t* peak, bool reset_peak);
diff --git a/sagemaker-xgboost-container_b200/csrc/grow.cu b/sagemaker-xgboost-container_b200/csrc/grow.cu
--- a/sagemaker-xgboost-container_b200/csrc/grow.cu
+++ b/sagemaker-xgboost-container_b200/csrc/grow.cu
@@ -7,7 +7,15 @@
 
 namespace b200 {
 
+thread_local bool g_chain_launches = false;
+struct ChainScope {
+  explicit ChainScope(bool on) { g_chain_launches = on; }
+  ~ChainScope() { g_chain_launches = false; }
+  void stop() { g_chain_launches = false; }
+};
+
 __global__ void pack_tree_kernel(TreeArrays t, const int* n_nodes, DevNode* out, int cap) {
+  pdl_wait();
   const int nn = *n_nodes;
   for (int i = blockIdx.x * blockDim.x + threadIdx.x; i < cap; i += gridDim.x * blockDim.x) {
     DevNode d;
@@ -19,8 +27,9 @@
 __global__ void snapshot_h_kernel(const GH64* slot, long long* cache, size_t entries) {
   for (size_t e = (size_t)blockIdx.x * blockDim.x + threadIdx.x; e < entries; e += (size_t)gridDim.x * blockDim.x) cache[e] = slot[e].h;
 }
-__global__ void slot_from_cache_kernel(GH64* slot, const long long* cache, size_t entries) {
-  for (size_t e = (size_t)blockIdx.x * blockDim.x + threadIdx.x; e < entries; e += (size_t)gridDim.x * blockDim.x) { GH64 v; v.g = 0; v.h = cache[e]; slot[e] = v; }
+__global__ void root_slot_kernel(GH64* slot, const long long* cache, size_t entries) {
+  pdl_wait();
+  for (size_t e = (size_t)blockIdx.x * blockDim.x + threadIdx.x; e < entries; e += (size_t)gridDim.x * blockDim.x) { GH64 v; v.g = 0; v.h = cache ? cache[e] : 0; slot[e] = v; }
 }
 __global__ void gather_u32_kernel(const unsigned* src, const unsigned* idx, unsigned* dst, int64_t n) {
   const int64_t i = (int64_t)blockIdx.x * blockDim.x + threadIdx.x;
@@ -195,13 +204,13 @@
   const int k = in.k, D = in.p.max_depth;
   const bool dist = in.world > 1;
   const int num_sms = engine_num_sms();
-  launch_init_tree(gs, ta, (unsigned)bm.n, s);
-  if (in.root_mode == 2) { slot_from_cache_kernel<<<num_sms, 256, 0, s>>>(hist_pool.p, root_h_cache.p, slot_stride); ++g_kernel_launches; CUDA_OK(cudaGetLastError()); }
-  else CUDA_OK(cudaMemsetAsync(hist_pool.p, 0, slot_stride * sizeof(GH64), s));
+  const bool routed = routes(in.lg_iters, D);
+  ChainScope chain(routed && !dist && !profile);
+  launch_init_tree(gs, ta, (unsigned)bm.n, s, in.n_ic > 0 ? ic_path.p : nullptr, ic_allowed.p, bm.F);
+  launch_chained(root_slot_kernel, num_sms, 256, 0, s, hist_pool.p, in.root_mode == 2 ? root_h_cache.p : nullptr, slot_stride);
   const bool g_only = in.root_mode != 0;
   const int pay = g_only ? 4 : 8;
   const bool carry_tail = tail_by_position(bm);
-  const bool routed = routes(in.lg_iters, D);
   if (profile && routed) {
     prof_part_row_bytes[0] = 3;
     prof_part_row_bytes[1] = 4;
@@ -229,10 +238,6 @@
   };
   allreduce_hist(hist_pool.p, slot_stride * 2);
   allreduce_hist(gs.node_sum, 2);
-  if (in.n_ic > 0) {
-    CUDA_OK(cudaMemsetAsync(ic_path.p, 0, (size_t)bm.F, s));
-    CUDA_OK(cudaMemsetAsync(ic_allowed.p, 1, (size_t)bm.F, s));
-  }
   auto part_args = [&](int level, int cur, int next) {
     const bool root = cur == kRootRows;
     PartArgs pa{}; pa.gs = gs; pa.tree = ta; pa.bins_col = bm.bins_col; pa.n = bm.n;
@@ -278,13 +283,14 @@
       ra.g_only = g_only ? 1 : 0;
       ra.tail_row = carry_tail ? reinterpret_cast<const unsigned*>(bm.bins_tail) : nullptr;
       ra.ridx = ridx[0].p; ra.gp = gp[0].p; ra.tl = carry_tail ? tl[0].p : nullptr; ra.rows_counter = profile ? prof_rows.p + 2 : nullptr;
+      ra.pool_zero = hist_pool.p + (size_t)next_base * slot_stride; ra.pool_zero_entries = (size_t)next_half * slot_stride;
       timed(kProfPartition, [&] { launch_route(ra, s); });
     } else {
       PartArgs pa = part_args(L, L == 0 ? kRootRows : (L & 1) ^ 1, L & 1);
       pa.build_only = L == D - 2 ? 1 : 0;
       timed(kProfPartition, [&] { launch_partition(pa, max_tiles, s); });
+      CUDA_OK(cudaMemsetAsync(hist_pool.p + (size_t)next_base * slot_stride, 0, (size_t)next_half * slot_stride * sizeof(GH64), s));
     }
-    CUDA_OK(cudaMemsetAsync(hist_pool.p + (size_t)next_base * slot_stride, 0, (size_t)next_half * slot_stride * sizeof(GH64), s));
     timed(kProfDeepHist, [&] { launch_hist_build(level_hist_args(routed ? 0 : L & 1), num_sms, s); });
     allreduce_hist(hist_pool.p + (size_t)next_base * slot_stride, (size_t)next_half * slot_stride * 2);
     launch_subtract(gs, hist_pool.p, slot_stride, next_half, s);
@@ -292,6 +298,7 @@
   }
   const uint8_t* start = routed && D >= 2 ? node_of_row.p : nullptr;
   if (in.adaptive) {
+    chain.stop();
     launch_locate_leaves(ta, gs.n_nodes, bm.bins_col, bm.n, bm.has_missing, start, g_only ? nullptr : gpair.p + (size_t)k * gp_stride, &adapt, s);
     SelectArgs sa{}; sa.values = in.resid; sa.seg = adapt.seg.p; sa.h = in.adaptive == 2 ? reinterpret_cast<const float*>(gpair.p + (size_t)k * gp_stride) + 1 : nullptr;
     sa.h_stride = 2; sa.scales = gs.scales; sa.n = bm.n; sa.nseg = max_leaves(); sa.alpha = (double)in.alpha;
@@ -302,12 +309,20 @@
   }
   timed(kProfMargin, [&] { launch_update_margin(ta, gs.n_nodes, bm.bins_col, bm.n, bm.has_missing, start, in.margin, in.K, k, leaf_scale.p, s); });
   if (profile) prof_margin_rows += bm.n;
-  pack_tree_kernel<<<(cap_nodes + 255) / 256, 256, 0, s>>>(ta, gs.n_nodes, packed.p, cap_nodes); ++g_kernel_launches;
-  CUDA_OK(cudaGetLastError());
+  launch_chained(pack_tree_kernel, (cap_nodes + 255) / 256, 256, 0, s, ta, gs.n_nodes, packed.p, cap_nodes);
 }
 void TreeBuilder::end_segment() {
   cudaGraph_t graph = nullptr; cudaGraphExec_t exec = nullptr;
   CUDA_OK(cudaStreamEndCapture(engine_stream(), &graph));
+  size_t nn = 0, ne = 0;
+  if (cudaGraphGetNodes(graph, nullptr, &nn) == cudaSuccess && cudaGraphGetEdges_v2(graph, nullptr, nullptr, nullptr, &ne) == cudaSuccess) {
+    std::vector<cudaGraphNode_t> nodes(nn), from(ne), to(ne); std::vector<cudaGraphEdgeData> data(ne);
+    if (nn) CUDA_OK(cudaGraphGetNodes(graph, nodes.data(), &nn));
+    if (ne) CUDA_OK(cudaGraphGetEdges_v2(graph, from.data(), to.data(), data.data(), &ne));
+    for (size_t i = 0; i < nn; ++i) { cudaGraphNodeType t; CUDA_OK(cudaGraphNodeGetType(nodes[i], &t)); capturing->kernel_nodes += t == cudaGraphNodeTypeKernel; }
+    capturing->edges += (long long)ne;
+    for (size_t i = 0; i < ne; ++i) capturing->programmatic_edges += data[i].type == cudaGraphDependencyTypeProgrammatic;
+  }
   cudaError_t e = cudaGraphInstantiate(&exec, graph, 0);
   cudaGraphDestroy(graph);
   CUDA_OK(e);
@@ -452,6 +467,16 @@
   return o;
 }
 
+std::string TreeBuilder::graph_json() const {
+  std::string o = "[";
+  for (size_t k = 0; k < graphs.size(); ++k) {
+    const TreeGraph& g = graphs[k];
+    o += (k ? ",{" : "{") + std::string("\"segments\":") + std::to_string(g.segs.size()) + ",\"kernel_nodes\":" + std::to_string(g.kernel_nodes) +
+         ",\"edges\":" + std::to_string(g.edges) + ",\"programmatic_edges\":" + std::to_string(g.programmatic_edges) + "}";
+  }
+  return o + "]";
+}
+
 void TreeBuilder::set_profile(bool on) {
   profile = on;
   if (on) { prof_rows.alloc(4); prof_rows.zero(engine_stream()); prof_margin_rows = 0; }
diff --git a/sagemaker-xgboost-container_b200/csrc/grow.h b/sagemaker-xgboost-container_b200/csrc/grow.h
--- a/sagemaker-xgboost-container_b200/csrc/grow.h
+++ b/sagemaker-xgboost-container_b200/csrc/grow.h
@@ -51,9 +51,10 @@
   std::vector<cudaGraphExec_t> segs; std::vector<std::function<void()>> colls;
   TreeInputs key{}; long long launches = 0;
   bool eager_done = false;
+  long long kernel_nodes = 0, edges = 0, programmatic_edges = 0;
   TreeGraph() = default; TreeGraph(TreeGraph&&) = default;
   ~TreeGraph() { destroy(); }
-  void destroy() { for (auto e : segs) if (e) cudaGraphExecDestroy(e); segs.clear(); colls.clear(); }
+  void destroy() { for (auto e : segs) if (e) cudaGraphExecDestroy(e); segs.clear(); colls.clear(); kernel_nodes = edges = programmatic_edges = 0; }
 };
 
 struct TreeBuilder {
@@ -99,6 +100,7 @@
   void grow(const TreeInputs& in);
   PendingTree stage_tree();
   void set_profile(bool on); std::string profile_json();
+  std::string graph_json() const;
   void debug_build_root_hist(const BinnedMatrix& bm, const float* gpair_host, std::vector<long long>* hist_out, float* scales_out,
                              int repeats, float* ms_out, int mode, const unsigned* row_ids, int64_t n_ids);
   std::string debug_eval_root(const TreeInputs& in, const long long* hist_fm, long long G, long long H, float max_g, float max_h,
diff --git a/sagemaker-xgboost-container_b200/csrc/hist.cu b/sagemaker-xgboost-container_b200/csrc/hist.cu
--- a/sagemaker-xgboost-container_b200/csrc/hist.cu
+++ b/sagemaker-xgboost-container_b200/csrc/hist.cu
@@ -280,25 +280,14 @@
   constexpr int PL = GONLY ? 1 : 2;
   constexpr int NCW = kRootConsumerWarps, R = kRootRows;
   extern __shared__ __align__(128) unsigned char smem_raw[];
-  const int nb = *a.build_count;
-  if (nb <= 0) return;
-  const unsigned T = a.build_prefix[nb];
-  if (T == 0) return;
   const int lane = threadIdx.x & 31, warp = threadIdx.x >> 5;
   const int g0 = blockIdx.y * a.ng_chunk;
   const int ng_here = min(a.ng_chunk, a.ngroups - g0);
   const bool has_tail = a.tw > 0 && blockIdx.y == gridDim.y - 1;
-  if (a.rows_counter && blockIdx.x == 0 && blockIdx.y == 0 && threadIdx.x == 0) atomicAdd(a.rows_counter, (unsigned long long)T);
 
   const unsigned smem_base = (unsigned)__cvta_generic_to_shared(smem_raw);
   const unsigned ring = (smem_base + c.ring_off + 127u) & ~127u;
   const unsigned bars = ring + (unsigned)c.S * c.stage_bytes;
-  const unsigned row_bytes = 32u * (unsigned)c.box_groups;
-  const unsigned main_tile_bytes = (unsigned)R * row_bytes;
-  constexpr unsigned kGradBytes = GONLY ? 4u : 8u;
-  const unsigned gp_off = main_tile_bytes, tail_tile_off = main_tile_bytes + (unsigned)R * kGradBytes;
-  const unsigned ntiles = (T + R - 1) / R;
-  const unsigned my_ntiles = ntiles > blockIdx.x ? (ntiles - blockIdx.x + gridDim.x - 1) / gridDim.x : 0u;
 
   {
     const int main4 = ng_here * PL * kPlaneBytes / 16;
@@ -315,6 +304,18 @@
     }
   }
   __syncthreads();
+  pdl_wait();
+  const int nb = *a.build_count;
+  if (nb <= 0) return;
+  const unsigned T = a.build_prefix[nb];
+  if (T == 0) return;
+  if (a.rows_counter && blockIdx.x == 0 && blockIdx.y == 0 && threadIdx.x == 0) atomicAdd(a.rows_counter, (unsigned long long)T);
+  const unsigned row_bytes = 32u * (unsigned)c.box_groups;
+  const unsigned main_tile_bytes = (unsigned)R * row_bytes;
+  constexpr unsigned kGradBytes = GONLY ? 4u : 8u;
+  const unsigned gp_off = main_tile_bytes, tail_tile_off = main_tile_bytes + (unsigned)R * kGradBytes;
+  const unsigned ntiles = (T + R - 1) / R;
+  const unsigned my_ntiles = ntiles > blockIdx.x ? (ntiles - blockIdx.x + gridDim.x - 1) / gridDim.x : 0u;
 
   const int nid = a.build_nid[0];
   const size_t slot_entries = (size_t)a.ngroups * kGroupEntries + (size_t)256 * a.tw;
@@ -477,6 +478,14 @@
   static_assert(kWindowRowsSmall / (SUP * NWARPS) >= 1, "window too small");
   const unsigned iters_per_window = (unsigned)a.window_rows / (SUP * NWARPS);
   extern __shared__ __align__(16) int smem[];
+  constexpr int TWC = TAIL ? TW : 4;
+  constexpr int trep = gather_tail_replicas(NG) < gather_tail_bytes(NG) / (2 * 256 * 4 * TWC) ? gather_tail_replicas(NG) : gather_tail_bytes(NG) / (2 * 256 * 4 * TWC);
+  {
+    const int words4 = (NG * 2 * kPlaneBytes + (TAIL ? 2 * 256 * TWC * trep * 4 : 0)) / 16;
+    for (int i = threadIdx.x; i < words4; i += NTHREADS) reinterpret_cast<int4*>(smem)[i] = make_int4(0, 0, 0, 0);
+  }
+  __syncthreads();
+  pdl_wait();
   const int nb = *a.build_count;
   if (nb <= 0) return;
   const unsigned T = a.build_prefix[nb];
@@ -505,15 +514,7 @@
   const LaneConst lc = make_lane_const_rot(rot, c & 1, smem_g + (unsigned)((q < RPI ? (c >> 1) : 0) * 2 * kPlaneBytes));
   const int rot_qw = rot >> 2, rot_qb8 = (rot & 3) * 8;
   const uint8_t* gbins = (aligned ? a.bins_gather : a.bins) + (int64_t)g0 * kSlots + c * 16;
-  constexpr int TWC = TAIL ? TW : 4;
-  constexpr int trep = gather_tail_replicas(NG) < gather_tail_bytes(NG) / (2 * 256 * 4 * TWC) ? gather_tail_replicas(NG) : gather_tail_bytes(NG) / (2 * 256 * 4 * TWC);
   const unsigned tail_base_rep = smem_g + (unsigned)(NG * 2 * kPlaneBytes) + (unsigned)((lane / TWC) % trep) * (unsigned)TWC * 4u;
-
-  {
-    const int words4 = (NG * 2 * kPlaneBytes + (TAIL ? 2 * 256 * TWC * trep * 4 : 0)) / 16;
-    for (int i = threadIdx.x; i < words4; i += NTHREADS) reinterpret_cast<int4*>(smem)[i] = make_int4(0, 0, 0, 0);
-  }
-  __syncthreads();
 
   int b = 0;
   { int lo = 0, hi = nb; while (lo < hi) { int mid = (lo + hi) >> 1; if (a.build_prefix[mid + 1] > r0) hi = mid; else lo = mid + 1; } b = lo; }
@@ -614,6 +615,7 @@
 }
 
 __global__ void __launch_bounds__(256) hist_reduce_kernel(HistArgs a, unsigned C, unsigned sup) {
+  pdl_wait();
   const int nb = *a.build_count;
   if (nb <= 0) return;
   const unsigned T = a.build_prefix[nb];
@@ -737,9 +739,8 @@
 template <int NG, int NT, bool GPAY>
 static void launch_gather_tw(const HistArgs& a, int gx, int nchunks, cudaStream_t stream) {
   const int smem = NG * 2 * kPlaneBytes + (a.tw ? gather_tail_bytes(NG) : 0);
-  if (a.tw == 0) hist_gather_kernel<NG, 0, NT, GPAY><<<dim3(gx, nchunks), NT, smem, stream>>>(a);
-  else if (a.tw == 4) hist_gather_kernel<NG, 4, NT, GPAY><<<dim3(gx, nchunks), NT, smem, stream>>>(a);
-  else hist_gather_kernel<NG, 8, NT, GPAY><<<dim3(gx, nchunks), NT, smem, stream>>>(a);
+  void (*k)(HistArgs) = a.tw == 0 ? hist_gather_kernel<NG, 0, NT, GPAY> : a.tw == 4 ? hist_gather_kernel<NG, 4, NT, GPAY> : hist_gather_kernel<NG, 8, NT, GPAY>;
+  launch_chained(k, dim3(gx, nchunks), NT, smem, stream, a);
 }
 template <int NG, int NT>
 static void launch_gather(const HistArgs& a, int gx, int nchunks, cudaStream_t stream) {
@@ -757,11 +758,8 @@
     RootCfg c; CUtensorMap tm;
     if (root_plan(a.ng_chunk, a.tw, gonly, &c) && get_tensor_map(a.bins, a.n, a.row_stride, c.box_groups, kRootRows, &tm)) {
       const int gx = num_sms / nchunks > 0 ? num_sms / nchunks : 1;
-      if (gonly) hist_root_kernel<true><<<dim3(gx, nchunks), kRootThreads, c.total, stream>>>(tm, a, c);
-      else hist_root_kernel<false><<<dim3(gx, nchunks), kRootThreads, c.total, stream>>>(tm, a, c);
+      launch_chained(gonly ? hist_root_kernel<true> : hist_root_kernel<false>, dim3(gx, nchunks), kRootThreads, c.total, stream, tm, a, c);
       g_last_kernel = gonly ? "hist_root_kernel<GONLY>" : "hist_root_kernel<GH>";
-      ++g_kernel_launches;
-      CUDA_OK(cudaGetLastError());
       return;
     }
   }
@@ -776,13 +774,7 @@
   else if (ng == 2) launch_gather<2, 768>(a, gx, nchunks, stream);
   else launch_gather<3, 768>(a, gx, nchunks, stream);
   g_last_kernel = "hist_gather_kernel";
-  ++g_kernel_launches;
-  CUDA_OK(cudaGetLastError());
-  if (a.partials) {
-    hist_reduce_kernel<<<num_sms * 8, 256, 0, stream>>>(a, (unsigned)gx, (unsigned)gather_super_rows(ng));
-    ++g_kernel_launches;
-    CUDA_OK(cudaGetLastError());
-  }
-}
-
-}
+  if (a.partials) launch_chained(hist_reduce_kernel, num_sms * 8, 256, 0, stream, a, (unsigned)gx, (unsigned)gather_super_rows(ng));
+}
+
+}
diff --git a/sagemaker-xgboost-container_b200/csrc/tree.cu b/sagemaker-xgboost-container_b200/csrc/tree.cu
--- a/sagemaker-xgboost-container_b200/csrc/tree.cu
+++ b/sagemaker-xgboost-container_b200/csrc/tree.cu
@@ -40,7 +40,9 @@
          (unsigned long long)(0x1FFu - (unsigned)ord);
 }
 
-__global__ void init_tree_kernel(GrowState gs, TreeArrays t, unsigned n) {
+__global__ void init_tree_kernel(GrowState gs, TreeArrays t, unsigned n, unsigned char* ic_path, unsigned char* ic_allowed, int F) {
+  pdl_wait();
+  if (ic_path) for (int f = threadIdx.x; f < F; f += blockDim.x) { ic_path[f] = 0; ic_allowed[f] = 1; }
   if (threadIdx.x != 0 || blockIdx.x != 0) return;
   *gs.n_nodes = 1; *gs.n_leaves = 1;
   *gs.n_slots = kLgFirstFreeSlot; *gs.lg_done = 0; gs.depth[0] = 0; gs.open[0] = 0;
@@ -67,6 +69,7 @@
 
 constexpr int kEvalSegs = 32, kEvalBinsPerSeg = kBins / kEvalSegs;
 __global__ void __launch_bounds__(32 * kEvalSegs) eval_kernel(EvalArgs a) {
+  pdl_wait();
   const int li = blockIdx.x;
   if (li >= a.gs.level_count[a.level]) return;
   const int nid = a.gs.level_nodes[(size_t)a.level * a.max_level_nodes + li];
@@ -263,6 +266,7 @@
 
 __global__ void __launch_bounds__(256) apply_kernel(ApplyArgs a) {
   __shared__ unsigned s_tmp[33];
+  pdl_wait();
   GrowState& gs = a.gs;
   const int L = a.level;
   const int cnt = gs.level_count[L];
@@ -560,13 +564,18 @@
   __syncthreads();
 }
 
+__device__ __forceinline__ void route_zero_pool(const RouteArgs& a) {
+  for (size_t e = (size_t)blockIdx.x * blockDim.x + threadIdx.x; e < a.pool_zero_entries; e += (size_t)gridDim.x * blockDim.x) a.pool_zero[e] = GH64{0, 0};
+}
+
 constexpr int kRuns = kRouteTile / 1024;
 __global__ void __launch_bounds__(256) route_kernel(RouteArgs a) {
   __shared__ PackedNode s_node[kRouteMaxNodes];
   __shared__ unsigned char s_bidx[kRouteMaxNodes];
   __shared__ unsigned s_cnt[kRouteMaxBuild];
+  pdl_wait();
   const int nb = *a.gs.build_count;
-  if (a.level > 0 && nb == 0) return;
+  if (a.level > 0 && nb == 0) { route_zero_pool(a); return; }
   const int64_t r0 = (int64_t)blockIdx.x * kRouteTile + threadIdx.x * 4;
   const int lane = threadIdx.x & 31;
   unsigned ids[kRuns], out[kRuns];
@@ -612,24 +621,56 @@
     const int64_t t0 = (int64_t)blockIdx.x * kRouteTile;
     atomicAdd(a.rows_counter, (unsigned long long)(a.n - t0 < (int64_t)kRouteTile ? a.n - t0 : (int64_t)kRouteTile));
   }
-}
-
+  route_zero_pool(a);
+}
+
+constexpr int kScanChunks = 8;
 __global__ void __launch_bounds__(1024) route_scan_kernel(RouteArgs a) {
-  __shared__ unsigned s_run[1024], s_tmp[33];
+  __shared__ unsigned s_warp[32], s_tot;
+  pdl_wait();
   const int c = blockIdx.x;
   if (c >= *a.gs.build_count) return;
   unsigned* cnt = a.tile_counts + (size_t)c * a.ntiles;
-  const unsigned per = (a.ntiles + blockDim.x - 1) / blockDim.x, t0 = threadIdx.x * per, t1 = min(t0 + per, a.ntiles);
+  const int lane = threadIdx.x & 31, warp = threadIdx.x >> 5, nw = blockDim.x >> 5;
+  constexpr unsigned kStep = 32u * kScanChunks;
+  const unsigned per = ((a.ntiles + nw - 1) / nw + kStep - 1) / kStep * kStep;
+  const unsigned t0 = min((unsigned)warp * per, a.ntiles), t1 = min(t0 + per, a.ntiles);
   unsigned sum = 0;
-#pragma unroll 8
-  for (unsigned t = t0; t < t1; ++t) sum += cnt[t];
-  s_run[threadIdx.x] = sum;
-  __syncthreads();
-  const unsigned tot = block_exclusive_scan(s_run, s_run, (int)blockDim.x, s_tmp);
-  unsigned run = s_run[threadIdx.x];
-#pragma unroll 8
-  for (unsigned t = t0; t < t1; ++t) { const unsigned v = cnt[t]; cnt[t] = run; run += v; }
-  if (threadIdx.x == 0) a.gs.seg_count[a.gs.build_nid[c]] = tot;
+  for (unsigned base = t0; base < t1; base += kStep) {
+    unsigned v[kScanChunks];
+#pragma unroll
+    for (int j = 0; j < kScanChunks; ++j) { const unsigned t = base + 32u * j + lane; v[j] = t < t1 ? cnt[t] : 0u; }
+#pragma unroll
+    for (int j = 0; j < kScanChunks; ++j) sum += v[j];
+  }
+  sum = __reduce_add_sync(0xffffffffu, sum);
+  if (lane == 0) s_warp[warp] = sum;
+  __syncthreads();
+  if (warp == 0) {
+    const unsigned w = lane < nw ? s_warp[lane] : 0u;
+    unsigned x = w;
+#pragma unroll
+    for (int o = 1; o < 32; o <<= 1) { const unsigned y = __shfl_up_sync(0xffffffffu, x, o); if (lane >= o) x += y; }
+    s_warp[lane] = x - w;
+    if (lane == 31) s_tot = x;
+  }
+  __syncthreads();
+  unsigned run = s_warp[warp];
+  for (unsigned base = t0; base < t1; base += kStep) {
+    unsigned v[kScanChunks];
+#pragma unroll
+    for (int j = 0; j < kScanChunks; ++j) { const unsigned t = base + 32u * j + lane; v[j] = t < t1 ? cnt[t] : 0u; }
+#pragma unroll
+    for (int j = 0; j < kScanChunks; ++j) {
+      unsigned x = v[j];
+#pragma unroll
+      for (int o = 1; o < 32; o <<= 1) { const unsigned y = __shfl_up_sync(0xffffffffu, x, o); if (lane >= o) x += y; }
+      const unsigned t = base + 32u * j + lane;
+      if (t < t1) cnt[t] = run + x - v[j];
+      run += __shfl_sync(0xffffffffu, x, 31);
+    }
+  }
+  if (threadIdx.x == 0) a.gs.seg_count[a.gs.build_nid[c]] = s_tot;
 }
 
 constexpr int kWarpRows = kRouteTile / 8, kWarpSteps = kWarpRows / 32;
@@ -646,6 +687,7 @@
   __shared__ unsigned s_tl[TL ? kRouteTile : 1];
   __shared__ unsigned char s_ch[kRouteTile];
   const GrowState& gs = a.gs;
+  pdl_wait();
   const int nb = *gs.build_count;
   if (nb == 0) { if (blockIdx.x == 0 && threadIdx.x == 0) gs.build_prefix[0] = 0; return; }
   stage_route_tables(a, nullptr, s_bidx, nb);
@@ -733,6 +775,7 @@
                                                             const uint8_t* node_of_row, float* margin, int K, int k, const float* leaf_scale) {
   __shared__ PackedNode s_nodes[kPackedNodesSmem];
   __shared__ float s_leaf[kPackedNodesSmem];
+  pdl_wait();
   const int nn = *n_nodes;
   const bool packed = nn <= kPackedNodesSmem && nn < 0xffff;
   if (packed) {
@@ -778,6 +821,7 @@
 }
 
 __global__ void __launch_bounds__(256) subtract_kernel(GrowState gs, GH64* pool, size_t stride) {
+  pdl_wait();
   const int r = blockIdx.x;
   if (r >= *gs.build_count) return;
   const int bld = gs.build_nid[r], sub = gs.build_sub_nid[r];
@@ -789,12 +833,12 @@
   }
 }
 
-void launch_init_tree(const GrowState& gs, const TreeArrays& t, unsigned n, cudaStream_t s) {
-  init_tree_kernel<<<1, 32, 0, s>>>(gs, t, n); ++g_kernel_launches; CUDA_OK(cudaGetLastError());
+void launch_init_tree(const GrowState& gs, const TreeArrays& t, unsigned n, cudaStream_t s, unsigned char* ic_path, unsigned char* ic_allowed, int F) {
+  launch_chained(init_tree_kernel, 1, ic_path ? 256 : 32, 0, s, gs, t, n, ic_path, ic_allowed, F);
 }
 void launch_scales(const GrowState& gs, int grad_bits, cudaStream_t s) { scales_kernel<<<1, 32, 0, s>>>(gs, grad_bits); ++g_kernel_launches; CUDA_OK(cudaGetLastError()); }
 void launch_eval(const EvalArgs& a, int max_nodes_level, cudaStream_t s) {
-  dim3 grid(max_nodes_level, a.ngroups + (a.tw > 0 ? 1 : 0)); eval_kernel<<<grid, 32 * kEvalSegs, 0, s>>>(a); ++g_kernel_launches; CUDA_OK(cudaGetLastError());
+  launch_chained(eval_kernel, dim3(max_nodes_level, a.ngroups + (a.tw > 0 ? 1 : 0)), 32 * kEvalSegs, 0, s, a);
 }
 void launch_apply_lossguide(const ApplyArgs& a, int iter, cudaStream_t s) { apply_lossguide_kernel<<<1, 256, 0, s>>>(a, iter); ++g_kernel_launches; CUDA_OK(cudaGetLastError()); }
 void launch_lg_copy_back(const PartArgs& a, unsigned* ridx_dst, void* gp_dst, unsigned* tl_dst, unsigned max_tiles, cudaStream_t s) {
@@ -809,7 +853,7 @@
 void launch_lg_stage(const GrowState& gs, GH64* pool, size_t slot_entries, int to_stage, cudaStream_t s) {
   lg_stage_kernel<<<(unsigned)((slot_entries + 1023) / 1024), 256, 0, s>>>(gs, pool, slot_entries, to_stage); ++g_kernel_launches; CUDA_OK(cudaGetLastError());
 }
-void launch_apply(const ApplyArgs& a, cudaStream_t s) { apply_kernel<<<1, 256, 0, s>>>(a); ++g_kernel_launches; CUDA_OK(cudaGetLastError()); }
+void launch_apply(const ApplyArgs& a, cudaStream_t s) { launch_chained(apply_kernel, 1, 256, 0, s, a); }
 void launch_partition(const PartArgs& a, unsigned max_tiles, cudaStream_t s) {
   CUDA_OK(cudaMemsetAsync(a.gs.tile_desc, 0, sizeof(unsigned long long) * ((size_t)max_tiles + 1), s));
   const bool tl = a.tl_cur != nullptr;
@@ -819,22 +863,20 @@
 }
 void launch_route(const RouteArgs& a, cudaStream_t s) {
   if (a.ntiles == 0) return;
-  route_kernel<<<a.ntiles, 256, 0, s>>>(a); ++g_kernel_launches; CUDA_OK(cudaGetLastError());
-  route_scan_kernel<<<1u << a.level, 1024, 0, s>>>(a); ++g_kernel_launches; CUDA_OK(cudaGetLastError());
+  launch_chained(route_kernel, a.ntiles, 256, 0, s, a);
+  launch_chained(route_scan_kernel, 1u << a.level, 1024, 0, s, a);
   const bool tl = a.tail_row != nullptr;
   const unsigned grid = std::min(a.ntiles, 4u * (unsigned)engine_num_sms());
-  if (a.g_only) { if (tl) scatter_kernel<true, true><<<grid, 256, 0, s>>>(a); else scatter_kernel<true, false><<<grid, 256, 0, s>>>(a); }
-  else { if (tl) scatter_kernel<false, true><<<grid, 256, 0, s>>>(a); else scatter_kernel<false, false><<<grid, 256, 0, s>>>(a); }
-  ++g_kernel_launches; CUDA_OK(cudaGetLastError());
+  void (*scatter)(RouteArgs) = a.g_only ? (tl ? scatter_kernel<true, true> : scatter_kernel<true, false>) : (tl ? scatter_kernel<false, true> : scatter_kernel<false, false>);
+  launch_chained(scatter, grid, 256, 0, s, a);
 }
 void launch_update_margin(const TreeArrays& t, const int* n_nodes, const uint8_t* bins_col, int64_t n, int has_missing, const uint8_t* node_of_row,
                           float* margin, int K, int k, const float* leaf_scale, cudaStream_t s) {
   if (n == 0) return;
-  update_margin_kernel<<<(unsigned)((n + 1023) / 1024), 256, 0, s>>>(t, n_nodes, bins_col, n, has_missing, node_of_row, margin, K, k, leaf_scale);
-  ++g_kernel_launches; CUDA_OK(cudaGetLastError());
+  launch_chained(update_margin_kernel, (unsigned)((n + 1023) / 1024), 256, 0, s, t, n_nodes, bins_col, n, has_missing, node_of_row, margin, K, k, leaf_scale);
 }
 void launch_subtract(const GrowState& gs, GH64* pool, size_t slot_entries, int max_build, cudaStream_t s) {
-  dim3 grid(max_build, (unsigned)((slot_entries + 1023) / 1024)); subtract_kernel<<<grid, 256, 0, s>>>(gs, pool, slot_entries); ++g_kernel_launches; CUDA_OK(cudaGetLastError());
-}
-
-}
+  launch_chained(subtract_kernel, dim3(max_build, (unsigned)((slot_entries + 1023) / 1024)), 256, 0, s, gs, pool, slot_entries);
+}
+
+}
diff --git a/sagemaker-xgboost-container_b200/csrc/tree.h b/sagemaker-xgboost-container_b200/csrc/tree.h
--- a/sagemaker-xgboost-container_b200/csrc/tree.h
+++ b/sagemaker-xgboost-container_b200/csrc/tree.h
@@ -46,6 +46,7 @@
   const float* g; const float2* gpair; int g_only; const unsigned* tail_row;
   unsigned* ridx; void* gp; unsigned* tl;
   unsigned long long* rows_counter;
+  GH64* pool_zero; size_t pool_zero_entries;
 };
 
 struct HistArgs {
@@ -88,7 +89,8 @@
 size_t hist_partial_entries(int ngroups, int tw, int num_sms, int max_build);
 void hist_configure();
 const char* hist_last_kernel();
-void launch_init_tree(const GrowState& gs, const TreeArrays& t, unsigned n, cudaStream_t s);
+void launch_init_tree(const GrowState& gs, const TreeArrays& t, unsigned n, cudaStream_t s, unsigned char* ic_path = nullptr,
+                      unsigned char* ic_allowed = nullptr, int F = 0);
 void launch_scales(const GrowState& gs, int grad_bits, cudaStream_t s);
 void launch_eval(const EvalArgs& a, int max_nodes_level, cudaStream_t s);
 void launch_apply(const ApplyArgs& a, cudaStream_t s);
```

After: 110.5, median of 6. 1.01x the previous value.
